# ctpeterson/qex

Hardware: AMD Instinct MI355X
Metric: staggered Dslash GFLOP/s + CG iters/s, 32^4 SU(3) fp64, 1/2/4/8 MI355X (higher is better)
Workload: dtype f64

## Files before the change

### include/qexhip.h

```cpp
#ifndef QEXHIP_H
#define QEXHIP_H

#include <stddef.h>

#ifdef __cplusplus
extern "C" {
#endif

typedef struct qexhip_ctx *qexhip_handle;

#define QEXHIP_OK 0
#define QEXHIP_ERR_ARG (-1)
#define QEXHIP_ERR_HIP (-2)
#define QEXHIP_ERR_STATE (-3)
#define QEXHIP_ERR_COMM (-4)
#define QEXHIP_ERR_IO (-5)

#define QEXHIP_EVEN 0
#define QEXHIP_ODD 1
#define QEXHIP_ALL 2

int qexhip_init(qexhip_handle *h, int device, const int latLocal[4],
                const int rankGeom[4], const int rankCoord[4]);
int qexhip_finalize(qexhip_handle h);
int qexhip_device_count(int *n);
const char *qexhip_last_error(void);
int qexhip_sync(qexhip_handle h);
int qexhip_device_info(qexhip_handle h, char *buf, int buflen);

#define QEXHIP_UNIQUE_ID_BYTES 128
int qexhip_comm_unique_id(char id[QEXHIP_UNIQUE_ID_BYTES]);
int qexhip_comm_init(qexhip_handle h, const char id[QEXHIP_UNIQUE_ID_BYTES], int nranks, int rank);
int qexhip_comm_info(qexhip_handle h, int *nranks, int *rank, int *device, char *busid, int buslen);
int qexhip_comm_transport(qexhip_handle h, char *name, int len, long stats[4]);
int qexhip_comm_count(qexhip_handle h, int *ncomms);
int qexhip_stag_sweep_info(qexhip_handle h, int out[8]);
int qexhip_stag_sweep_tuning(qexhip_handle h, double out[8]);
int qexhip_comm_force_halo(qexhip_handle h, int on);

int qexhip_layout_default_inner(const int localGeom[4], int V, int innerGeom[4]);
int qexhip_layout_simd_map(const int localGeom[4], const int innerGeom[4], int *v1_of_simd);
int qexhip_layout_vec_simd_to_v1(const int localGeom[4], const int innerGeom[4], const double *simd, double *v1);
int qexhip_layout_vec_v1_to_simd(const int localGeom[4], const int innerGeom[4], const double *v1, double *simd);
int qexhip_layout_gauge_simd_to_v1(const int localGeom[4], const int innerGeom[4], const double *const g[4], double *v1);
int qexhip_layout_gauge_v1_to_simd(const int localGeom[4], const int innerGeom[4], const double *v1, double *const g[4]);

int qexhip_stag_set_links(qexhip_handle h, const double *fat, const double *lng);

int qexhip_stag_dslash(qexhip_handle h, double *r, const double *x, int parity, double a, double b);

int qexhip_stag_D(qexhip_handle h, double *r, const double *x, double m, double sc);

int qexhip_stag_stagD(qexhip_handle h, double *r, const double *x, int parity, double m, double sc, double a);

int qexhip_stag_D_acc(qexhip_handle h, double *r, const double *x, double m, double sc, double a);

int qexhip_stag_op_xx(qexhip_handle h, double *r, const double *x, double m2, int par_even);

int qexhip_stag_eo_reconstruct(qexhip_handle h, double *r, const double *b, double m);

int qexhip_stag_eo_reduce(qexhip_handle h, double *r, const double *b, double m);

int qexhip_stag_outer(qexhip_handle h, double *f, const double *x, double scale_even, double scale_odd,
                      int accumulate);

int qexhip_stag_solve_xx(qexhip_handle h, double *x, const double *b, double mass, double r2req,
                         int maxits, int par_even, int *iters, double *r2_over_b2,
                         double *hist, int histcap);

int qexhip_stag_solve(qexhip_handle h, double *x, const double *b, double mass, double r2req,
                      int maxits, int *iters, double *r2_final);

int qexhip_stag_solve_prev(qexhip_handle h, double *x, const double *b, double mass, double r2req,
                           int maxits, int use_prev, int *iters, double *r2_final);

int qexhip_stag_solve_xx_sloppy(qexhip_handle h, double *x, const double *b, double mass, double r2req, int maxits,
                                int par_even, int sloppy, int *iters, double *r2_over_b2, int *nupdates);
int qexhip_stag_solve_sloppy(qexhip_handle h, double *x, const double *b, double mass, double r2req, int maxits,
                             int use_prev, int sloppy, int *iters, double *r2_final, int *nupdates);

int qexhip_stag_solve_xx_multi(qexhip_handle h, double *const *xs, const double *b,
                               const double *shifts, int nmass, double r2req, int maxits,
                               int par_even, int *iters, double *hist, int histcap);
int qexhip_stag_solve_multi(qexhip_handle h, double *const *xs, const double *b,
                            const double *masses, int nmass, double r2req, int maxits,
                            int *iters, double *r2_final);

int qexhip_norm2(qexhip_handle h, const double *x, int parity, double *out);
int qexhip_redot(qexhip_handle h, const double *x, const double *y, int parity, double *out);
int qexhip_dot(qexhip_handle h, const double *x, const double *y, int parity, double out[2]);
int qexhip_axpy(qexhip_handle h, double a, const double *x, double *y, int parity);
int qexhip_xpay(qexhip_handle h, const double *x, double a, double *y, int parity);

int qexhip_field_new(qexhip_handle h, int *id);
int qexhip_field_free(qexhip_handle h, int id);
int qexhip_field_upload(qexhip_handle h, int id, const double *host);
int qexhip_field_download(qexhip_handle h, int id, double *host);
int qexhip_field_zero(qexhip_handle h, int id);
int qexhip_dev_dslash(qexhip_handle h, int r_id, int x_id, int parity, double a, double b);
int qexhip_dev_op_xx(qexhip_handle h, int r_id, int x_id, double m2, int par_even);
int qexhip_dev_solve_xx(qexhip_handle h, int x_id, int b_id, double mass, double r2req,
                        int maxits, int par_even, int *iters, double *r2_over_b2,
                        double *hist, int histcap);
int qexhip_dev_solve_xx_sloppy(qexhip_handle h, int x_id, int b_id, double mass, double r2req, int maxits, int par_even,
                               int sloppy, int *iters, double *r2_over_b2, int *nupdates);
int qexhip_dev_op_xx_sloppy(qexhip_handle h, int r_id, int x_id, double m2, int par_even);
int qexhip_stag_links_info_f32(qexhip_handle h, int *format, double *max_dev);
int qexhip_dev_solve_xx_continue(qexhip_handle h, int x_id, double r2req, int maxits, int *iters, double *r2_over_b2,
                                 double *hist, int histcap);
int qexhip_dev_solve_xx_multi(qexhip_handle h, const int *x_ids, int b_id, const double *shifts, int nmass,
                              double r2req, int maxits, int par_even, int *iters, double *hist, int histcap);

int qexhip_release_workspace(qexhip_handle h);
int qexhip_dev_norm2(qexhip_handle h, int x_id, int parity, double *out);
int qexhip_dev_redot(qexhip_handle h, int x_id, int y_id, int parity, double *out);
int qexhip_dev_dot(qexhip_handle h, int x_id, int y_id, int parity, double out[2]);
int qexhip_dev_D(qexhip_handle h, int r_id, int x_id, double m, double sc);
int qexhip_dev_zero(qexhip_handle h, int id, int parity);
int qexhip_dev_solve_batch(qexhip_handle h, int n, const int *x_ids, const int *b_ids, const double *mass,
                           const double *r2req, int maxits, int *iters, double *r2);
int qexhip_dev_solve_batch_sloppy(qexhip_handle h, int n, const int *x_ids, const int *b_ids, const double *mass,
                                  const double *r2req, int maxits, int sloppy, int *iters, double *r2_final, int *nupdates);

int qexhip_dev_meson_corners(qexhip_handle h, int n, const int *x_ids, const int *y_ids, int t0, double *out);
int qexhip_dev_sym_shift(qexhip_handle h, int r_id, int x_id, int mu);
int qexhip_dev_norm2slice(qexhip_handle h, int id, int dir, double *out);

int qexhip_gauge_set(qexhip_handle h, const double *g);
int qexhip_gauge_get(qexhip_handle h, double *g);
int qexhip_plaq(qexhip_handle h, double out[6]);
int qexhip_gauge_force(qexhip_handle h, double *f, double cplaq);
int qexhip_wflow(qexhip_handle h, int nsteps, double eps);
int qexhip_gauge_force_general(qexhip_handle h, double *f, double cplaq, double c2, int kind);
int qexhip_wflow_general(qexhip_handle h, int nsteps, double eps, double cplaq, double c2, int kind);
int qexhip_flow_EQ(qexhip_handle h, int loop, double out[3]);
int qexhip_flow_measure(qexhip_handle h, double plaq[6], double EQ[3]);
int qexhip_gauge_action(qexhip_handle h, double cplaq, double crect, double cadjplaq, double *out);
int qexhip_gauge_update(qexhip_handle h, const double *p, double t);
int qexhip_gauge_reunit(qexhip_handle h);
int qexhip_wline(qexhip_handle h, const int *path, int n, double out[2]);
int qexhip_polyakov_loops(qexhip_handle h, double out[8]);
int qexhip_plaq_s4(qexhip_handle h, double out[8]);

int qexhip_fat7(qexhip_handle h, const double *g, const double coef[5], double *fl, double *ll, double naik);
int qexhip_hisq_smear(qexhip_handle h, const double *g, double *fl, double *ll);
int qexhip_nhyp_smear(qexhip_handle h, const double *g, double *fl, double alpha1, double alpha2, double alpha3);
int qexhip_fat7_deriv(qexhip_handle h, const double *g, const double *dfl, const double coef[5], const double *dll, double naik, double *d);
int qexhip_hisq_force(qexhip_handle h, const double *g, const double *dsdsu, const double *dsdsul, double *f);
int qexhip_hisq_prepare(qexhip_handle h, const double *g, double *fl, double *ll);
int qexhip_hisq_closure_force(qexhip_handle h, const double *dsdsu, const double *dsdsul, double *f);
int qexhip_hisq_release(qexhip_handle h);
int qexhip_hisq_fermion_force(qexhip_handle h, double *f, const double *const *psi, const double *scale, int n);

int qexhip_stag_solve_xx_batch(qexhip_handle h, int n, double *const *x, const double *const *b, const double *mass,
                               const double *r2req, int maxits, int par_even, int *iters, double *r2_over_b2);
int qexhip_stag_solve_batch(qexhip_handle h, int n, double *const *x, const double *const *b, const double *mass,
                            const double *r2req, int maxits, int *iters, double *r2_over_b2);

int qexhip_stag_solve_xx_batch_sloppy(qexhip_handle h, int n, double *const *x, const double *const *b, const double *mass,
                                      const double *r2req, int maxits, int par_even, int sloppy, int *iters, double *r2_over_b2,
                                      int *nupdates);
int qexhip_stag_solve_batch_sloppy(qexhip_handle h, int n, double *const *x, const double *const *b, const double *mass,
                                   const double *r2req, int maxits, int sloppy, int *iters, double *r2_final, int *nupdates);

int qexhip_stag_links_info(qexhip_handle h, int *nlinks, int *compressed, double *max_dev);
int qexhip_stag_links_storage(qexhip_handle h, int *bytes_per_link, long long *escaped);
int qexhip_link_residual_host(const double *links, int n, unsigned char *escaped, double *row2);
int qexhip_set_option(qexhip_handle h, const char *name, int value);

int qexhip_stag_set_links_hisq(qexhip_handle h, const double *g);
int qexhip_stag_set_links_nhyp(qexhip_handle h, const double *g, double alpha1, double alpha2, double alpha3,
                               const int antiperiodic[4], const int phases[4]);

int qexhip_nhyp_prepare(qexhip_handle h, const double *g, double alpha1, double alpha2, double alpha3, double *fl);
int qexhip_nhyp_force(qexhip_handle h, double *f, const double *chain);
int qexhip_nhyp_release(qexhip_handle h);
int qexhip_nhyp_gauge_force(qexhip_handle h, double *f, double cplaq, double crect, double cadjplaq);
int qexhip_nhyp_fforce(qexhip_handle h, double *f, int n, const double *const *phi, const double *mass, const double *scale,
                       const double *r2req, int maxits, const int antiperiodic[4], const int phases[4], int *iters);
int qexhip_nhyp_fermion_force(qexhip_handle h, double *f, const double *const *psi, const double *scale, int n,
                              const int antiperiodic[4], const int phases[4]);
int qexhip_nhyp_fforce_dev(qexhip_handle h, double *f, int n, const int *phi_ids, const double *mass, const double *scale,
                           const double *r2req, int maxits, const int antiperiodic[4], const int phases[4], int *iters);

typedef struct qexhip_rng qexhip_rng;
int qexhip_rng_new(qexhip_rng **rng, int kind, unsigned long long seed, const int lat[4], const int glat[4], int t_offset);
int qexhip_rng_free(qexhip_rng *rng);
int qexhip_rng_uniform(qexhip_rng *rng, int ncomp, double *v);
int qexhip_rng_gaussian_vector(qexhip_rng *rng, double *v);
int qexhip_rng_u1_vector(qexhip_rng *rng, double *v);
int qexhip_rng_random_tah(qexhip_rng *rng, double *p);
int qexhip_rng_gauge_random(qexhip_rng *rng, double *g);
int qexhip_rng_gauge_warm(qexhip_rng *rng, double s, double *g);
int qexhip_rng_state_words(qexhip_rng *rng);
int qexhip_rng_get_state(qexhip_rng *rng, unsigned *out);
int qexhip_rng_set_state(qexhip_rng *rng, const unsigned *in);

int qexhip_rng_dev_gaussian_vector(qexhip_handle h, qexhip_rng *rng, int field_id);
int qexhip_rng_dev_u1_vector(qexhip_handle h, qexhip_rng *rng, int field_id);
int qexhip_md_refresh_momenta(qexhip_handle h, qexhip_rng *rng);

int qexhip_md_begin(qexhip_handle h, const double *g, const double *p);
int qexhip_md_end(qexhip_handle h, double *g, double *p);
int qexhip_md_momentum_norm2(qexhip_handle h, double *p2);
int qexhip_md_update_links(qexhip_handle h, double t);
int qexhip_md_gauge_force(qexhip_handle h, double cplaq, double crect, double cadj);
int qexhip_md_kick(qexhip_handle h, int source, double t);
int qexhip_md_shift_links(qexhip_handle h, int source, double t);
int qexhip_md_save_links(qexhip_handle h);
int qexhip_md_restore_links(qexhip_handle h);

int qexhip_io_gauge_info(const char *path, int lat[4], char *precision, int *checksums_present);
int qexhip_io_read_gauge(const char *path, const int lat[4], double *g, unsigned *suma, unsigned *sumb);
int qexhip_io_read_gauge_slab(const char *path, const int lat[4], int t0, int nt, double *g);
int qexhip_io_write_gauge(const char *path, const int lat[4], const double *g, char precision, const char *file_md,
                          const char *record_md);
int qexhip_io_write_field(const char *path, const int lat[4], const void *data, int site_bytes, int word_bytes, const char *datatype,
                          char precision, int colors, int datacount, const char *file_md, const char *record_md);
int qexhip_io_read_field(const char *path, const int lat[4], void *data, int site_bytes, int word_bytes, char datatype[64]);
int qexhip_io_metadata(const char *path, char *file_md, int file_cap, char *record_md, int record_cap, int *file_len,
                       int *record_len);
int qexhip_io_crc32(const void *data, size_t nbytes, unsigned *crc);

int qexhip_timers_enable(qexhip_handle h, int on);
int qexhip_timers_reset(qexhip_handle h);
int qexhip_timers_get(qexhip_handle h, const char *name, long *count, double *total_ms);

int qexhip_debug_geom(const int latLocal[4], int depth, int halo, int out[8]);
int qexhip_debug_nbr_pos(const int latLocal[4], int depth, int halo, int c, int parity, int mu, int hop);
int qexhip_debug_site_coord(const int latLocal[4], int c, int parity, int x[4]);
int qexhip_debug_tile_order(const int latLocal[4], int mu, int nu, int *out, int cap);

#ifdef __cplusplus
}
#endif
#endif
```

### qex_amd/__init__.py

```python
from ._lib import QexHipError, LIB_PATH, lib
from .layout import Layout
from .gauge import setBC, stagPhase, rephase, unit, synthetic_random_su3, synthetic_gaussian_vector
from .staggered import (
    Context, device_count, Staggered, SolverParams, newStag, newStag3, link_residual_host, plaq, gaugeForce, gaugeFlow, gaugeSet, gaugeFlowResident, flowEQ, flowMeasure, gaugeAction, gaugeUpdate, reunit, wline, ploops, s4_gauge, ResidentMD, HisqCoefs, HypCoefs, makeImpLinks, fat7lDeriv, EVEN, ODD, ALL,
    SloppyNone, SloppySingle, SloppyHalf,
)
from .io import loadGauge, loadGaugeSlab, saveGauge, getFileLattice, gaugeFileInfo, writeField, readField, fileMetadata
from .rng import RngField, RngMilc6, MRG32k3a
from .mesons import stagLocalMesons, stagMesons, norm2slice, sft, printLocalMesons, pointSource, wallSource, localMesonTables
```

### qex_amd/_lib.py

```python
import ctypes as C
import os

_HERE = os.path.dirname(os.path.abspath(__file__))
LIB_PATH = os.environ.get("QEXHIP_LIB", os.path.join(_HERE, "libqexhip.so"))
_lib = None

_vp, _ci, _cd = C.c_void_p, C.c_int, C.c_double
_pi, _pd = C.POINTER(C.c_int), C.POINTER(C.c_double)
SYMBOLS = [
    ("qexhip_init", _ci, [C.POINTER(_vp), _ci, _pi, _pi, _pi]),
    ("qexhip_finalize", _ci, [_vp]),
    ("qexhip_device_count", _ci, [_pi]),
    ("qexhip_last_error", C.c_char_p, []),
    ("qexhip_sync", _ci, [_vp]),
    ("qexhip_device_info", _ci, [_vp, C.c_char_p, _ci]),
    ("qexhip_layout_default_inner", _ci, [_pi, _ci, _pi]),
    ("qexhip_layout_simd_map", _ci, [_pi, _pi, _pi]),
    ("qexhip_layout_vec_simd_to_v1", _ci, [_pi, _pi, _vp, _vp]),
    ("qexhip_layout_vec_v1_to_simd", _ci, [_pi, _pi, _vp, _vp]),
    ("qexhip_layout_gauge_simd_to_v1", _ci, [_pi, _pi, C.POINTER(C.c_void_p), _vp]),
    ("qexhip_layout_gauge_v1_to_simd", _ci, [_pi, _pi, _vp, C.POINTER(C.c_void_p)]),
    ("qexhip_comm_unique_id", _ci, [C.c_char_p]),
    ("qexhip_comm_init", _ci, [_vp, C.c_char_p, _ci, _ci]),
    ("qexhip_comm_force_halo", _ci, [_vp, _ci]),
    ("qexhip_comm_info", _ci, [_vp, _pi, _pi, _pi, C.c_char_p, _ci]),
    ("qexhip_comm_count", _ci, [_vp, _pi]),
    ("qexhip_comm_transport", _ci, [_vp, C.c_char_p, _ci, C.POINTER(C.c_long)]),
    ("qexhip_stag_sweep_info", _ci, [_vp, _pi]),
    ("qexhip_stag_sweep_tuning", _ci, [_vp, _pd]),
    ("qexhip_dot", _ci, [_vp, _vp, _vp, _ci, _pd]),
    ("qexhip_dev_dot", _ci, [_vp, _ci, _ci, _ci, _pd]),
    ("qexhip_stag_set_links", _ci, [_vp, _vp, _vp]),
    ("qexhip_stag_dslash", _ci, [_vp, _vp, _vp, _ci, _cd, _cd]),
    ("qexhip_stag_D", _ci, [_vp, _vp, _vp, _cd, _cd]),
    ("qexhip_stag_D_acc", _ci, [_vp, _vp, _vp, _cd, _cd, _cd]),
    ("qexhip_stag_op_xx", _ci, [_vp, _vp, _vp, _cd, _ci]),
    ("qexhip_stag_eo_reconstruct", _ci, [_vp, _vp, _vp, _cd]),
    ("qexhip_stag_eo_reduce", _ci, [_vp, _vp, _vp, _cd]),
    ("qexhip_stag_stagD", _ci, [_vp, _vp, _vp, _ci, _cd, _cd, _cd]),
    ("qexhip_stag_outer", _ci, [_vp, _vp, _vp, _cd, _cd, _ci]),
    ("qexhip_stag_solve_xx", _ci, [_vp, _vp, _vp, _cd, _cd, _ci, _ci, _pi, _pd, _vp, _ci]),
    ("qexhip_stag_solve", _ci, [_vp, _vp, _vp, _cd, _cd, _ci, _pi, _pd]),
    ("qexhip_stag_solve_xx_sloppy", _ci, [_vp, _vp, _vp, _cd, _cd, _ci, _ci, _ci, _pi, _pd, _pi]),
    ("qexhip_stag_solve_sloppy", _ci, [_vp, _vp, _vp, _cd, _cd, _ci, _ci, _ci, _pi, _pd, _pi]),
    ("qexhip_dev_solve_xx_sloppy", _ci, [_vp, _ci, _ci, _cd, _cd, _ci, _ci, _ci, _pi, _pd, _pi]),
    ("qexhip_dev_op_xx_sloppy", _ci, [_vp, _ci, _ci, _cd, _ci]),
    ("qexhip_stag_links_info_f32", _ci, [_vp, _pi, _pd]),
    ("qexhip_stag_solve_prev", _ci, [_vp, _vp, _vp, _cd, _cd, _ci, _ci, _pi, _pd]),
    ("qexhip_stag_solve_xx_multi", _ci, [_vp, _vp, _vp, _vp, _ci, _cd, _ci, _ci, _pi, _vp, _ci]),
    ("qexhip_stag_solve_multi", _ci, [_vp, _vp, _vp, _vp, _ci, _cd, _ci, _pi, _pd]),
    ("qexhip_norm2", _ci, [_vp, _vp, _ci, _pd]),
    ("qexhip_redot", _ci, [_vp, _vp, _vp, _ci, _pd]),
    ("qexhip_axpy", _ci, [_vp, _cd, _vp, _vp, _ci]),
    ("qexhip_xpay", _ci, [_vp, _vp, _cd, _vp, _ci]),
    ("qexhip_field_new", _ci, [_vp, _pi]),
    ("qexhip_field_free", _ci, [_vp, _ci]),
    ("qexhip_field_upload", _ci, [_vp, _ci, _vp]),
    ("qexhip_field_download", _ci, [_vp, _ci, _vp]),
    ("qexhip_field_zero", _ci, [_vp, _ci]),
    ("qexhip_dev_dslash", _ci, [_vp, _ci, _ci, _ci, _cd, _cd]),
    ("qexhip_dev_op_xx", _ci, [_vp, _ci, _ci, _cd, _ci]),
    ("qexhip_dev_solve_xx", _ci, [_vp, _ci, _ci, _cd, _cd, _ci, _ci, _pi, _pd, _vp, _ci]),
    ("qexhip_dev_solve_xx_continue", _ci, [_vp, _ci, _cd, _ci, _pi, _pd, _vp, _ci]),
    ("qexhip_dev_solve_xx_multi", _ci, [_vp, _pi, _ci, _pd, _ci, _cd, _ci, _ci, _pi, _vp, _ci]),
    ("qexhip_release_workspace", _ci, [_vp]),
    ("qexhip_dev_norm2", _ci, [_vp, _ci, _ci, _pd]),
    ("qexhip_dev_redot", _ci, [_vp, _ci, _ci, _ci, _pd]),
    ("qexhip_dev_D", _ci, [_vp, _ci, _ci, _cd, _cd]),
    ("qexhip_gauge_set", _ci, [_vp, _vp]),
    ("qexhip_gauge_get", _ci, [_vp, _vp]),
    ("qexhip_plaq", _ci, [_vp, _vp]),
    ("qexhip_gauge_force", _ci, [_vp, _vp, _cd]),
    ("qexhip_wflow", _ci, [_vp, _ci, _cd]),
    ("qexhip_flow_EQ", _ci, [_vp, _ci, _vp]),
    ("qexhip_flow_measure", _ci, [_vp, _vp, _vp]),
    ("qexhip_gauge_force_general", _ci, [_vp, _vp, _cd, _cd, _ci]),
    ("qexhip_wflow_general", _ci, [_vp, _ci, _cd, _cd, _cd, _ci]),
    ("qexhip_fat7", _ci, [_vp, _vp, _pd, _vp, _vp, _cd]),
    ("qexhip_hisq_smear", _ci, [_vp, _vp, _vp, _vp]),
    ("qexhip_nhyp_smear", _ci, [_vp, _vp, _vp, _cd, _cd, _cd]),
    ("qexhip_stag_solve_xx_batch", _ci, [_vp, _ci, _vp, _vp, _vp, _vp, _ci, _ci, _pi, _vp]),
    ("qexhip_stag_solve_batch", _ci, [_vp, _ci, _vp, _vp, _vp, _vp, _ci, _pi, _vp]),
    ("qexhip_stag_solve_xx_batch_sloppy", _ci, [_vp, _ci, _vp, _vp, _vp, _vp, _ci, _ci, _ci, _pi, _vp, _pi]),
    ("qexhip_stag_solve_batch_sloppy", _ci, [_vp, _ci, _vp, _vp, _vp, _vp, _ci, _ci, _pi, _vp, _pi]),
    ("qexhip_stag_links_info", _ci, [_vp, _pi, _pi, _vp]),
    ("qexhip_stag_links_storage", _ci, [_vp, _pi, C.POINTER(C.c_longlong)]),
    ("qexhip_link_residual_host", _ci, [_vp, _ci, _vp, _vp]),
    ("qexhip_set_option", _ci, [_vp, C.c_char_p, _ci]),
    ("qexhip_fat7_deriv", _ci, [_vp, _vp, _vp, _vp, _vp, _cd, _vp]),
    ("qexhip_hisq_force", _ci, [_vp, _vp, _vp, _vp, _vp]),
    ("qexhip_hisq_prepare", _ci, [_vp, _vp, _vp, _vp]),
    ("qexhip_hisq_closure_force", _ci, [_vp, _vp, _vp, _vp]),
    ("qexhip_hisq_release", _ci, [_vp]),
    ("qexhip_hisq_fermion_force", _ci, [_vp, _vp, _vp, _vp, _ci]),
    ("qexhip_stag_set_links_hisq", _ci, [_vp, _vp]),
    ("qexhip_stag_set_links_nhyp", _ci, [_vp, _vp, _cd, _cd, _cd, _pi, _pi]),
    ("qexhip_nhyp_prepare", _ci, [_vp, _vp, _cd, _cd, _cd, _vp]),
    ("qexhip_nhyp_force", _ci, [_vp, _vp, _vp]),
    ("qexhip_nhyp_release", _ci, [_vp]),
    ("qexhip_nhyp_fforce", _ci, [_vp, _vp, _ci, _vp, _vp, _vp, _vp, _ci, _pi, _pi, _pi]),
    ("qexhip_nhyp_gauge_force", _ci, [_vp, _vp, _cd, _cd, _cd]),
    ("qexhip_nhyp_fermion_force", _ci, [_vp, _vp, _vp, _vp, _ci, _pi, _pi]),
    ("qexhip_gauge_action", _ci, [_vp, _cd, _cd, _cd, _vp]),
    ("qexhip_gauge_update", _ci, [_vp, _vp, _cd]),
    ("qexhip_gauge_reunit", _ci, [_vp]),
    ("qexhip_wline", _ci, [_vp, _pi, _ci, _vp]),
    ("qexhip_polyakov_loops", _ci, [_vp, _vp]),
    ("qexhip_plaq_s4", _ci, [_vp, _vp]),
    ("qexhip_rng_new", _ci, [_vp, _ci, C.c_ulonglong, _pi, _pi, _ci]),
    ("qexhip_rng_free", _ci, [_vp]),
    ("qexhip_rng_uniform", _ci, [_vp, _ci, _vp]),
    ("qexhip_rng_gaussian_vector", _ci, [_vp, _vp]),
    ("qexhip_rng_u1_vector", _ci, [_vp, _vp]),
    ("qexhip_rng_random_tah", _ci, [_vp, _vp]),
    ("qexhip_rng_gauge_random", _ci, [_vp, _vp]),
    ("qexhip_rng_gauge_warm", _ci, [_vp, _cd, _vp]),
    ("qexhip_rng_dev_gaussian_vector", _ci, [_vp, _vp, _ci]),
    ("qexhip_rng_dev_u1_vector", _ci, [_vp, _vp, _ci]),
    ("qexhip_md_refresh_momenta", _ci, [_vp, _vp]),
    ("qexhip_dev_zero", _ci, [_vp, _ci, _ci]),
    ("qexhip_dev_solve_batch", _ci, [_vp, _ci, _pi, _pi, _pd, _pd, _ci, _pi, _pd]),
    ("qexhip_dev_solve_batch_sloppy", _ci, [_vp, _ci, _pi, _pi, _pd, _pd, _ci, _ci, _pi, _pd, _pi]),
    ("qexhip_dev_meson_corners", _ci, [_vp, _ci, _pi, _pi, _ci, _vp]),
    ("qexhip_dev_sym_shift", _ci, [_vp, _ci, _ci, _ci]),
    ("qexhip_dev_norm2slice", _ci, [_vp, _ci, _ci, _vp]),
    ("qexhip_nhyp_fforce_dev", _ci, [_vp, _vp, _ci, _pi, _pd, _pd, _pd, _ci, _pi, _pi, _pi]),
    ("qexhip_rng_state_words", _ci, [_vp]),
    ("qexhip_rng_get_state", _ci, [_vp, _vp]),
    ("qexhip_rng_set_state", _ci, [_vp, _vp]),
    ("qexhip_io_write_field", _ci, [C.c_char_p, _pi, _vp, _ci, _ci, C.c_char_p, C.c_char, _ci, _ci, C.c_char_p, C.c_char_p]),
    ("qexhip_io_read_field", _ci, [C.c_char_p, _pi, _vp, _ci, _ci, C.c_char_p]),
    ("qexhip_md_begin", _ci, [_vp, _vp, _vp]),
    ("qexhip_md_end", _ci, [_vp, _vp, _vp]),
    ("qexhip_md_momentum_norm2", _ci, [_vp, _pd]),
    ("qexhip_md_update_links", _ci, [_vp, _cd]),
    ("qexhip_md_gauge_force", _ci, [_vp, _cd, _cd, _cd]),
    ("qexhip_md_kick", _ci, [_vp, _ci, _cd]),
    ("qexhip_md_shift_links", _ci, [_vp, _ci, _cd]),
    ("qexhip_md_save_links", _ci, [_vp]),
    ("qexhip_md_restore_links", _ci, [_vp]),
    ("qexhip_io_metadata", _ci, [C.c_char_p, C.c_char_p, _ci, C.c_char_p, _ci, _pi, _pi]),
    ("qexhip_io_crc32", _ci, [C.c_char_p, C.c_size_t, C.POINTER(C.c_uint)]),
    ("qexhip_io_gauge_info", _ci, [C.c_char_p, _pi, C.c_char_p, _pi]),
    ("qexhip_io_read_gauge", _ci, [C.c_char_p, _pi, _vp, _vp, _vp]),
    ("qexhip_io_read_gauge_slab", _ci, [C.c_char_p, _pi, _ci, _ci, _vp]),
    ("qexhip_io_write_gauge", _ci, [C.c_char_p, _pi, _vp, C.c_char, C.c_char_p, C.c_char_p]),
    ("qexhip_timers_enable", _ci, [_vp, _ci]),
    ("qexhip_timers_reset", _ci, [_vp]),
    ("qexhip_timers_get", _ci, [_vp, C.c_char_p, C.POINTER(C.c_long), _pd]),
    ("qexhip_debug_geom", _ci, [_pi, _ci, _ci, _pi]),
    ("qexhip_debug_nbr_pos", _ci, [_pi, _ci, _ci, _ci, _ci, _ci, _ci]),
    ("qexhip_debug_site_coord", _ci, [_pi, _ci, _ci, _pi]),
    ("qexhip_debug_tile_order", _ci, [_pi, _ci, _ci, _pi, _ci]),
]


class QexHipError(RuntimeError):
    pass


def lib():
    global _lib
    if _lib is None:
        if not os.path.exists(LIB_PATH):
            raise QexHipError(
                f"{LIB_PATH} not found: build it with `make -C {_HERE}` "
                "(__graft_entry__.build()).  qex_amd has no CPU fallback."
            )
        L = C.CDLL(LIB_PATH, mode=C.RTLD_LOCAL | getattr(os, "RTLD_DEEPBIND", 0))
        for name, res, args in SYMBOLS:
            f = getattr(L, name)
            f.restype = res
            f.argtypes = args
        _lib = L
    return _lib


_tune = None


def tune_lib():
    global _tune
    if _tune is None:
        lib()
        path = os.path.join(os.path.dirname(LIB_PATH), "libqexhip_tune.so")
        if not os.path.exists(path):
            raise QexHipError(f"{path} not found: build it with `make -C {_HERE} libqexhip_tune.so`")
        T = C.CDLL(path, mode=C.RTLD_LOCAL | getattr(os, "RTLD_DEEPBIND", 0))
        pd = C.POINTER(C.c_double)
        T.qexhip_tune_dslash.argtypes = [_vp, _ci, _ci, _ci, pd]
        T.qexhip_tune_dslash_norm2.argtypes = [_vp, pd]
        T.qexhip_tune_stream.argtypes = [_vp, _ci, C.c_size_t, _ci, _ci, pd]
        T.qexhip_tune_fma64.argtypes = [_vp, _ci, _ci, _ci, _ci, pd]
        T.qexhip_tune_gather.argtypes = [_vp, _ci, _ci, _ci, _ci, pd]
        T.qexhip_tune_gather_rows.argtypes = [_vp, _ci, _ci, _ci, _ci, _ci, pd]
        _tune = T
    return _tune


def check(rc):
    if rc != 0:
        msg = lib().qexhip_last_error()
        raise QexHipError(f"libqexhip error {rc}: {msg.decode() if msg else ''}")
```

### qex_amd/csrc/api.cpp

```cpp
#include "qexhip_internal.h"
#include <string>
#include "../../include/qexhip.h"
#include <algorithm>
#include <cstdarg>
#include <cstdlib>
#include <cstring>
#include <vector>

static thread_local char g_err[1024] = "";

void qexhip_set_error(const char *fmt, ...) {
  va_list ap;
  va_start(ap, fmt);
  vsnprintf(g_err, sizeof(g_err), fmt, ap);
  va_end(ap);
}
extern "C" const char *qexhip_last_error(void) { return g_err; }

static bool timer_class_on(const qexhip_ctx *c, const char *name) {
  if (!c->timers_on) return false;
  if (c->timers_on == 2) return strncmp(name, "dslash", 6) == 0;
  if (c->timers_on == 3) return strncmp(name, "dslash", 6) == 0 || strcmp(name, "exchange") == 0 || strcmp(name, "allreduce") == 0;
  return true;
}
// ... 581 lines not shown
  if (!c) return QEXHIP_ERR_ARG;
  CHK(sloppy_check(c, 1));
  HIPCHK(hipSetDevice(c->device));
  DevField *fr, *fx;
  CHK(find_field(c, r_id, &fr));
  CHK(find_field(c, x_id, &fx));
  DevFieldF *xi, *ro;
  CHK(f32_field(c, F32_IN, &xi));
  CHK(f32_field(c, F32_AP, &ro));
  const int px = par_even ? 0 : 1;
  CHK(f32_from_f64(c, *xi, *fx, px, 1.0));
  CHK(f32_op_xx(c, *ro, *xi, m2, par_even, 0, nullptr, nullptr));
  return f32_to_f64(c, *fr, *ro, px, 1.0, 0);
}
extern "C" int qexhip_stag_links_info_f32(qexhip_handle c, int *format, double *max_dev) {
  if (!c) return QEXHIP_ERR_ARG;
  HIPCHK(hipSetDevice(c->device));
  return f32_links(c, format, max_dev);
}

extern "C" int qexhip_dev_solve_xx_continue(qexhip_handle c, int x_id, double r2req, int maxits, int *iters, double *r2_over_b2,
                                            double *hist, int histcap) {
  if (!c) return QEXHIP_ERR_ARG;
  HIPCHK(hipSetDevice(c->device));
  DevField *fx;
  CHK(find_field(c, x_id, &fx));
  return solve_xx_continue_dev(c, *fx, r2req, maxits, iters, r2_over_b2, hist, histcap);
}

extern "C" int qexhip_dev_solve_xx_multi(qexhip_handle c, const int *x_ids, int b_id, const double *shifts, int nmass,
                                         double r2req, int maxits, int par_even, int *iters, double *hist, int histcap) {
  if (!c || !x_ids || !shifts || nmass < 1 || nmass > 32) return QEXHIP_ERR_ARG;
  DevField *fb;
  CHK(find_field(c, b_id, &fb));
  std::vector<DevField *> xp(nmass);
  for (int k = 0; k < nmass; k++) {
    CHK(find_field(c, x_ids[k], &xp[k]));
    if (x_ids[k] == b_id) { qexhip_set_error("dev_solve_xx_multi: x_ids[%d] is the source field", k); return QEXHIP_ERR_ARG; }
    for (int j = 0; j < k; j++)
      if (x_ids[j] == x_ids[k]) { qexhip_set_error("dev_solve_xx_multi: x_ids[%d] == x_ids[%d]", j, k); return QEXHIP_ERR_ARG; }
  }
  return solve_xx_multi_dev(c, xp, *fb, shifts, nmass, r2req, maxits, par_even, iters, hist, histcap);
}

extern "C" int qexhip_release_workspace(qexhip_handle c) {
  if (!c) return QEXHIP_ERR_ARG;
  HIPCHK(hipSetDevice(c->device));
  HIPCHK(hipStreamSynchronize(c->stream));
  for (auto it = c->fields.begin(); it != c->fields.end();) {
    if (it->first <= -1000) {
      HIPCHK(hipFree(it->second.d));
      it = c->fields.erase(it);
    } else {
      ++it;
    }
  }
  gauge_release_scratch(c);
  f32_state_free(c);
  batch_f32_state_free(c);
  return 0;
}

extern "C" int qexhip_dev_norm2(qexhip_handle c, int x_id, int parity, double *out) {
  if (!c || !out || parity < 0 || parity > 2) return QEXHIP_ERR_ARG;
  HIPCHK(hipSetDevice(c->device));
  DevField *fx;
  CHK(find_field(c, x_id, &fx));
  CHK(blas_norm2(c, *fx, parity, &c->dscal[8]));
  return read_scalars(c, &c->dscal[8], 1, out);
}
extern "C" int qexhip_dev_redot(qexhip_handle c, int x_id, int y_id, int parity, double *out) {
  if (!c || !out || parity < 0 || parity > 2) return QEXHIP_ERR_ARG;
  HIPCHK(hipSetDevice(c->device));
  DevField *fx, *fy;
  CHK(find_field(c, x_id, &fx));
  CHK(find_field(c, y_id, &fy));
  CHK(blas_redot(c, *fx, *fy, parity, &c->dscal[8]));
  return read_scalars(c, &c->dscal[8], 1, out);
}
extern "C" int qexhip_dev_dot(qexhip_handle c, int x_id, int y_id, int parity, double out[2]) {
  if (!c || !out || parity < 0 || parity > 2) return QEXHIP_ERR_ARG;
  HIPCHK(hipSetDevice(c->device));
  DevField *fx, *fy;
  CHK(find_field(c, x_id, &fx));
  CHK(find_field(c, y_id, &fy));
  CHK(blas_cdot(c, *fx, *fy, parity, &c->dscal[8]));
  return read_scalars(c, &c->dscal[8], 2, out);
}
extern "C" int qexhip_dev_D(qexhip_handle c, int r_id, int x_id, double m, double sc) {
  if (!c || r_id == x_id) return QEXHIP_ERR_ARG;
  HIPCHK(hipSetDevice(c->device));
  DevField *fr, *fx;
  CHK(find_field(c, r_id, &fr));
  CHK(find_field(c, x_id, &fx));
  return op_D(c, *fr, *fx, m, sc);
}

extern "C" int qexhip_dev_meson_corners(qexhip_handle c, int n, const int *x_ids, const int *y_ids, int t0, double *out) {
  if (!c) return QEXHIP_ERR_ARG;
  if (!x_ids || !y_ids || !out) { qexhip_set_error("dev_meson_corners: null argument"); return QEXHIP_ERR_ARG; }
  if (n < 1 || n > 4) { qexhip_set_error("dev_meson_corners: n = %d, must be 1..4", n); return QEXHIP_ERR_ARG; }
  const int ntg = c->g.X[3] * c->rankGeom[3];
  if (t0 < 0 || t0 >= ntg) { qexhip_set_error("dev_meson_corners: t0 = %d outside [0, %d)", t0, ntg); return QEXHIP_ERR_ARG; }
  HIPCHK(hipSetDevice(c->device));
  DevField *xs[4], *ys[4];
  for (int k = 0; k < n; k++) {
    CHK(find_field(c, x_ids[k], &xs[k]));
    CHK(find_field(c, y_ids[k], &ys[k]));
  }
  return meson_corners(c, n, xs, ys, t0, out);
}
extern "C" int qexhip_dev_sym_shift(qexhip_handle c, int r_id, int x_id, int mu) {
  if (!c) return QEXHIP_ERR_ARG;
  if (mu < 0 || mu > 2) { qexhip_set_error("dev_sym_shift: mu = %d, only the spatial directions 0..2 are shifted", mu); return QEXHIP_ERR_ARG; }
  if (r_id == x_id) { qexhip_set_error("dev_sym_shift: r_id == x_id"); return QEXHIP_ERR_ARG; }
  if (!c->W) { qexhip_set_error("dev_sym_shift: no links set (qexhip_stag_set_links first)"); return QEXHIP_ERR_ARG; }
  HIPCHK(hipSetDevice(c->device));
  DevField *fr, *fx;
  CHK(find_field(c, r_id, &fr));
  CHK(find_field(c, x_id, &fx));
  return sym_shift(c, *fr, *fx, mu);
}
extern "C" int qexhip_dev_norm2slice(qexhip_handle c, int id, int dir, double *out) {
  if (!c) return QEXHIP_ERR_ARG;
  if (!out) { qexhip_set_error("dev_norm2slice: null argument"); return QEXHIP_ERR_ARG; }
  if (dir < 0 || dir > 3) { qexhip_set_error("dev_norm2slice: dir = %d, must be 0..3", dir); return QEXHIP_ERR_ARG; }
  HIPCHK(hipSetDevice(c->device));
  DevField *f;
  CHK(find_field(c, id, &f));
  return norm2slice(c, *f, dir, out);
}

extern "C" int qexhip_fat7(qexhip_handle c, const double *g, const double coef[5], double *fl, double *ll, double naik) {
  if (!c || !g || !coef || !fl) return QEXHIP_ERR_ARG;
  HIPCHK(hipSetDevice(c->device));
  return smear_fat7_host(c, g, coef, fl, ll, naik);
}
extern "C" int qexhip_hisq_smear(qexhip_handle c, const double *g, double *fl, double *ll) {
  if (!c || !g || !fl || !ll) return QEXHIP_ERR_ARG;
  HIPCHK(hipSetDevice(c->device));
  return smear_hisq_host(c, g, fl, ll);
}
extern "C" int qexhip_nhyp_smear(qexhip_handle c, const double *g, double *fl, double a1, double a2, double a3) {
  if (!c || !g || !fl) return QEXHIP_ERR_ARG;
  HIPCHK(hipSetDevice(c->device));
  return smear_nhyp_host(c, g, fl, a1, a2, a3);
}

extern "C" int qexhip_set_option(qexhip_handle c, const char *name, int value) {
  if (!c || !name) return QEXHIP_ERR_ARG;
  const std::string n(name);
  if (n == "recon") c->opt_recon = value;
  else if (n == "lossless") c->opt_lossless = value;
  else if (n == "overlap") c->opt_overlap = value;
  else if (n == "transport") {
    if (comm_ready(c)) { qexhip_set_error("option transport must be set before qexhip_comm_init"); return QEXHIP_ERR_STATE; }
    if (value < 0 || value > 3) { qexhip_set_error("option transport: 0 auto, 1 rccl, 2 peer, 3 rccl + mailbox sums"); return QEXHIP_ERR_ARG; }
    c->opt_transport = value;
  }
  else if (n == "batch_multi") c->opt_batch_multi = value;
  else if (n == "multi_reduce") c->opt_multi_reduce = value;
  else if (n == "flow_exp") c->opt_flow_exp = value;
  else if (n == "smear_ca") c->opt_smear_ca = value;
  else if (n == "chain_overlap") c->opt_chain_overlap = value;
  else if (n == "hop_split") {
    if (value != -1 && value != 0 && value != 2) { qexhip_set_error("option hop_split: -1 measured, 0 split by sites, 2 fused (the two-launch form 1 left the library in round 6)"); return QEXHIP_ERR_ARG; }
    c->opt_hop_split = value;
  }
  else if (n == "fused_spin_us") c->opt_fused_spin_us = value;
  else if (n == "emu_exchange_us") c->emu_exchange_us = value;
  else if (n == "emu_allreduce_us") c->emu_allreduce_us = value;
  else if (n == "emu_link_gbs") c->emu_link_gbs = value;
  else if (n == "obs_clover") c->opt_obs_clover = value;
  else if (n == "force_pair") c->opt_force_pair = value;
  else if (n == "sloppy_check") {
    if (value < 1) { qexhip_set_error("option sloppy_check: >= 1 fp32 iterations"); return QEXHIP_ERR_ARG; }
    c->opt_sloppy_check = value;
  }
  else { qexhip_set_error("unknown option"); return QEXHIP_ERR_ARG; }
  return 0;
}
extern "C" int qexhip_stag_solve_xx_batch(qexhip_handle c, int n, double *const *x, const double *const *b, const double *mass,
                                          const double *r2req, int maxits, int par_even, int *iters, double *r2_over_b2) {
  if (!c || !x || !b || !mass || !r2req) return QEXHIP_ERR_ARG;
  HIPCHK(hipSetDevice(c->device));
  return solve_batch_host(c, n, x, b, mass, r2req, maxits, par_even ? 1 : 0, iters, r2_over_b2);
}
extern "C" int qexhip_stag_solve_batch(qexhip_handle c, int n, double *const *x, const double *const *b, const double *mass,
                                       const double *r2req, int maxits, int *iters, double *r2_over_b2) {
  if (!c || !x || !b || !mass || !r2req) return QEXHIP_ERR_ARG;
  HIPCHK(hipSetDevice(c->device));
  return solve_batch_host(c, n, x, b, mass, r2req, maxits, -1, iters, r2_over_b2);
}
extern "C" int qexhip_stag_solve_xx_batch_sloppy(qexhip_handle c, int n, double *const *x, const double *const *b, const double *mass,
                                                 const double *r2req, int maxits, int par_even, int sloppy, int *iters,
                                                 double *r2_over_b2, int *nupdates) {
  if (!c || !x || !b || !mass || !r2req) return QEXHIP_ERR_ARG;
  CHK(sloppy_check(c, sloppy));
  if (n < 1 || n > 4) { qexhip_set_error("batch solve: 1 <= n <= 4"); return QEXHIP_ERR_ARG; }
  if (nupdates) for (int j = 0; j < n; j++) nupdates[j] = 0;
  if (!sloppy) return qexhip_stag_solve_xx_batch(c, n, x, b, mass, r2req, maxits, par_even, iters, r2_over_b2);
  HIPCHK(hipSetDevice(c->device));
  return solve_batch_sloppy_host(c, n, x, b, mass, r2req, maxits, par_even ? 1 : 0, sloppy, iters, r2_over_b2, nupdates);
}
extern "C" int qexhip_stag_solve_batch_sloppy(qexhip_handle c, int n, double *const *x, const double *const *b, const double *mass,
                                              const double *r2req, int maxits, int sloppy, int *iters, double *r2_final, int *nupdates) {
  if (!c || !x || !b || !mass || !r2req) return QEXHIP_ERR_ARG;
  CHK(sloppy_check(c, sloppy));
  if (n < 1 || n > 4) { qexhip_set_error("batch solve: 1 <= n <= 4"); return QEXHIP_ERR_ARG; }
  if (nupdates) for (int j = 0; j < n; j++) nupdates[j] = 0;
  if (!sloppy) return qexhip_stag_solve_batch(c, n, x, b, mass, r2req, maxits, iters, r2_final);
  HIPCHK(hipSetDevice(c->device));
  return solve_batch_sloppy_host(c, n, x, b, mass, r2req, maxits, -1, sloppy, iters, r2_final, nupdates);
}
extern "C" int qexhip_stag_links_info(qexhip_handle c, int *nlinks, int *compressed, double *max_dev) {
  if (!c) return QEXHIP_ERR_ARG;
  if (nlinks) *nlinks = c->W ? c->ndir : 0;
  if (compressed) *compressed = c->recon;
  if (max_dev) *max_dev = c->recon_dev;
  return 0;
}
extern "C" int qexhip_stag_links_storage(qexhip_handle c, int *bytes_per_link, long long *escaped) {
  if (!c) return QEXHIP_ERR_ARG;
  if (bytes_per_link) *bytes_per_link = !c->W ? 0 : (c->lres ? 108 : (c->recon == 1 ? 96 : (c->recon == 2 ? 112 : 144)));
  if (escaped) *escaped = c->lres_esc;
  return 0;
}
extern "C" int qexhip_link_residual_host(const double *links, int n, unsigned char *escaped, double *row2) {
  if (!links || n < 0) return QEXHIP_ERR_ARG;
  return link_residual_host((const double2 *)links, n, escaped, (double2 *)row2);
}
extern "C" int qexhip_hisq_prepare(qexhip_handle c, const double *g, double *fl, double *ll) {
  if (!c || !g) return QEXHIP_ERR_ARG;
  HIPCHK(hipSetDevice(c->device));
  return hisq_prepare(c, g, fl, ll);
}
extern "C" int qexhip_hisq_closure_force(qexhip_handle c, const double *dsdsu, const double *dsdsul, double *f) {
  if (!c || !dsdsu || !dsdsul || !f) return QEXHIP_ERR_ARG;
  HIPCHK(hipSetDevice(c->device));
  return hisq_closure_force(c, dsdsu, dsdsul, f);
}
extern "C" int qexhip_hisq_fermion_force(qexhip_handle c, double *f, const double *const *psi, const double *scale, int n) {
  if (!c || !f || !psi || !scale) return QEXHIP_ERR_ARG;
  HIPCHK(hipSetDevice(c->device));
  return hisq_fermion_force(c, f, psi, scale, n);
}
extern "C" int qexhip_hisq_release(qexhip_handle c) {
  if (!c) return QEXHIP_ERR_ARG;
  HIPCHK(hipSetDevice(c->device));
  hisq_state_free(c);
  return 0;
}
extern "C" int qexhip_hisq_force(qexhip_handle c, const double *g, const double *dsdsu, const double *dsdsul, double *f) {
  if (!c || !g || !dsdsu || !dsdsul || !f) return QEXHIP_ERR_ARG;
  HIPCHK(hipSetDevice(c->device));
  return smear_hisq_force_host(c, g, dsdsu, dsdsul, f);
}
extern "C" int qexhip_fat7_deriv(qexhip_handle c, const double *g, const double *dfl, const double coef[5], const double *dll,
                                 double naik, double *d) {
  if (!c || !g || !dfl || !coef || !d) return QEXHIP_ERR_ARG;
  HIPCHK(hipSetDevice(c->device));
  return smear_fat7_deriv_host(c, g, dfl, coef, dll, naik, d);
}
extern "C" int qexhip_stag_set_links_hisq(qexhip_handle c, const double *g) {
  if (!c) return QEXHIP_ERR_ARG;
  HIPCHK(hipSetDevice(c->device));
  return smear_set_links_hisq(c, g);
}
extern "C" int qexhip_stag_set_links_nhyp(qexhip_handle c, const double *g, double a1, double a2, double a3,
                                          const int antiperiodic[4], const int phases[4]) {
  if (!c) return QEXHIP_ERR_ARG;
  HIPCHK(hipSetDevice(c->device));
  static const int defph[4] = {8, 9, 11, 0};
  int mask = 0;
  for (int mu = 0; mu < 4; mu++) if (antiperiodic ? antiperiodic[mu] : (mu == 3)) mask |= 1 << mu;
  return smear_set_links_nhyp(c, g, a1, a2, a3, mask, phases ? phases : defph);
}

extern "C" int qexhip_nhyp_prepare(qexhip_handle c, const double *g, double a1, double a2, double a3, double *fl) {
  if (!c) return QEXHIP_ERR_ARG;
  HIPCHK(hipSetDevice(c->device));
  return nhyp_prepare(c, g, a1, a2, a3, fl);
}
extern "C" int qexhip_nhyp_force(qexhip_handle c, double *f, const double *chain) {
  if (!c || !f || !chain) return QEXHIP_ERR_ARG;
  HIPCHK(hipSetDevice(c->device));
  return nhyp_force_host(c, f, chain);
}
extern "C" int qexhip_nhyp_gauge_force(qexhip_handle c, double *f, double cplaq, double crect, double cadj) {
  if (!c) return QEXHIP_ERR_ARG;
  if (crect != 0.0 && cadj != 0.0) { qexhip_set_error("rect and adjplaq together are not a QEX action"); return QEXHIP_ERR_ARG; }
  HIPCHK(hipSetDevice(c->device));
  return nhyp_gauge_force(c, f, cplaq, cadj != 0.0 ? cadj : crect, cadj != 0.0 ? 1 : 0);
}
extern "C" int qexhip_nhyp_fermion_force(qexhip_handle c, double *f, const double *const *psi, const double *scale, int n,
                                         const int antiperiodic[4], const int phases[4]) {
  if (!c || !psi || !scale) return QEXHIP_ERR_ARG;
  HIPCHK(hipSetDevice(c->device));
  static const int defph[4] = {8, 9, 11, 0};
  int mask = 0;
  for (int mu = 0; mu < 4; mu++) if (antiperiodic ? antiperiodic[mu] : (mu == 3)) mask |= 1 << mu;
  return nhyp_fermion_force(c, f, psi, scale, n, mask, phases ? phases : defph);
}
extern "C" int qexhip_nhyp_fforce(qexhip_handle c, double *f, int n, const double *const *phi, const double *mass,
                                  const double *scale, const double *r2req, int maxits, const int antiperiodic[4],
                                  const int phases[4], int *iters) {
  if (!c || !phi || !mass || !scale || !r2req) return QEXHIP_ERR_ARG;
  HIPCHK(hipSetDevice(c->device));
  static const int defph[4] = {8, 9, 11, 0};
  int mask = 0;
  for (int mu = 0; mu < 4; mu++) if (antiperiodic ? antiperiodic[mu] : (mu == 3)) mask |= 1 << mu;
  return nhyp_fforce(c, f, n, phi, mass, scale, r2req, maxits, mask, phases ? phases : defph, iters);
}
extern "C" int qexhip_nhyp_fforce_dev(qexhip_handle c, double *f, int n, const int *phi_ids, const double *mass,
                                      const double *scale, const double *r2req, int maxits, const int antiperiodic[4],
                                      const int phases[4], int *iters) {
  if (!c || !phi_ids || !mass || !scale || !r2req || n < 1 || n > 64) return QEXHIP_ERR_ARG;
  HIPCHK(hipSetDevice(c->device));
  static const int defph[4] = {8, 9, 11, 0};
  int mask = 0;
  for (int mu = 0; mu < 4; mu++) if (antiperiodic ? antiperiodic[mu] : (mu == 3)) mask |= 1 << mu;
  std::vector<DevField *> pf(n);
  for (int k = 0; k < n; k++) CHK(find_field(c, phi_ids[k], &pf[k]));
  return nhyp_fforce(c, f, n, nullptr, mass, scale, r2req, maxits, mask, phases ? phases : defph, iters, pf.data());
}
struct qexhip_rng;
extern "C" int qexhip_rng_dev_gaussian_vector(qexhip_handle c, qexhip_rng *rng, int field_id) {
  if (!c || !rng) return QEXHIP_ERR_ARG;
  DevField *f;
  CHK(find_field(c, field_id, &f));
  return rng_dev_generate(c, rng, 0, f, nullptr);
}
extern "C" int qexhip_rng_dev_u1_vector(qexhip_handle c, qexhip_rng *rng, int field_id) {
  if (!c || !rng) return QEXHIP_ERR_ARG;
  DevField *f;
  CHK(find_field(c, field_id, &f));
  return rng_dev_generate(c, rng, 1, f, nullptr);
}
extern "C" int qexhip_md_refresh_momenta(qexhip_handle c, qexhip_rng *rng) {
  if (!c || !rng) return QEXHIP_ERR_ARG;
  HIPCHK(hipSetDevice(c->device));
  double2 *M = nullptr;
  CHK(md_momenta_dev(c, &M));
  return rng_dev_generate(c, rng, 2, nullptr, M);
}
extern "C" int qexhip_dev_zero(qexhip_handle c, int id, int parity) {
  if (!c || parity < 0 || parity > 2) return QEXHIP_ERR_ARG;
  HIPCHK(hipSetDevice(c->device));
  DevField *f;
  CHK(find_field(c, id, &f));
  return blas_zero(c, *f, parity);
}
static int batch_alias_check(int n, const int *x_ids, const int *b_ids) {
  for (int i = 0; i < n; i++)
    for (int j = 0; j < n; j++)
      if (x_ids[i] == b_ids[j] || (i != j && x_ids[i] == x_ids[j])) {
        qexhip_set_error("dev_solve_batch: solution field %d (system %d) aliases %s of system %d", x_ids[i], i,
                         x_ids[i] == b_ids[j] ? "the source" : "the solution", j);
        return QEXHIP_ERR_ARG;
      }
  return 0;
}
extern "C" int qexhip_dev_solve_batch(qexhip_handle c, int n, const int *x_ids, const int *b_ids, const double *mass,
                                      const double *r2req, int maxits, int *iters, double *r2) {
  if (!c || !x_ids || !b_ids || !mass || !r2req || n < 1 || n > 64) return QEXHIP_ERR_ARG;
  HIPCHK(hipSetDevice(c->device));
  CHK(batch_alias_check(n, x_ids, b_ids));
  for (int k0 = 0; k0 < n; k0 += 4) {
    const int k = std::min(4, n - k0);
    DevField *xs[4], *bs[4];
    for (int j = 0; j < k; j++) {
      CHK(find_field(c, x_ids[k0 + j], &xs[j]));
      CHK(find_field(c, b_ids[k0 + j], &bs[j]));
    }
    CHK(solve_full_batch_dev(c, k, xs, bs, mass + k0, r2req + k0, maxits, iters ? iters + k0 : nullptr, r2 ? r2 + k0 : nullptr));
  }
  return 0;
}
extern "C" int qexhip_dev_solve_batch_sloppy(qexhip_handle c, int n, const int *x_ids, const int *b_ids, const double *mass,
                                             const double *r2req, int maxits, int sloppy, int *iters, double *r2, int *nupdates) {
  if (!c || !x_ids || !b_ids || !mass || !r2req) return QEXHIP_ERR_ARG;
  CHK(sloppy_check(c, sloppy));
  if (n < 1 || n > 4) { qexhip_set_error("batch solve: 1 <= n <= 4"); return QEXHIP_ERR_ARG; }
  if (nupdates) for (int j = 0; j < n; j++) nupdates[j] = 0;
// ... 91 lines not shown
```

### qex_amd/csrc/blas.hip

```cpp
#include "qexhip_internal.h"
#include "reduce.h"
#include "cg_device.h"
#include <cstring>
#include "peer_device.h"

static inline int grid_for(size_t n2) {
  size_t nb = (n2 + 255) / 256;
  if (nb > 2048) nb = 2048;
  if (nb < 1) nb = 1;
  return (int)nb;
}
static inline size_t body2(const qexhip_ctx *c) { return (size_t)c->g.ntile * 192; }

#define FOR_PAR(par, p) for (int p = ((par) == 2 ? 0 : (par)); p <= ((par) == 2 ? 1 : (par)); p++)

__global__ void __launch_bounds__(256) k_zero(double2 *y, size_t n) {
  for (size_t i = blockIdx.x * 256 + threadIdx.x; i < n; i += (size_t)gridDim.x * 256) y[i] = make_double2(0, 0);
}
__global__ void __launch_bounds__(256) k_copy(double2 *y, const double2 *x, size_t n) {
  for (size_t i = blockIdx.x * 256 + threadIdx.x; i < n; i += (size_t)gridDim.x * 256) y[i] = x[i];
}
__global__ void __launch_bounds__(256) k_axpy(double a, const double2 *x, double2 *y, size_t n) {
  for (size_t i = blockIdx.x * 256 + threadIdx.x; i < n; i += (size_t)gridDim.x * 256) {
    double2 xv = x[i], yv = y[i];
// ... 17 lines not shown
}
__global__ void __launch_bounds__(256) k_axpby(double a, const double2 *x, double b, const double2 *y, double2 *z, size_t n) {
  for (size_t i = blockIdx.x * 256 + threadIdx.x; i < n; i += (size_t)gridDim.x * 256) {
    double2 xv = x[i], yv = y[i];
    z[i] = make_double2(a * xv.x + b * yv.x, a * xv.y + b * yv.y);
  }
}
__global__ void __launch_bounds__(256) k_redot(const double2 *x, const double2 *y, size_t n, double *partials) {
  double acc = 0;
  for (size_t i = blockIdx.x * 256 + threadIdx.x; i < n; i += (size_t)gridDim.x * 256) {
    double2 xv = x[i], yv = y[i];
    acc = fma(xv.x, yv.x, fma(xv.y, yv.y, acc));
  }
  double r = block_sum_256(acc);
  if (threadIdx.x == 0) partials[blockIdx.x] = r;
}
__global__ void __launch_bounds__(256) k_reduce_final(const double *partials, int n, double *out, const int *done) {
  if (done && *done) return;
  double acc = 0;
  for (int i = threadIdx.x; i < n; i += 256) acc += partials[i];
  double r = block_sum_256(acc);
  if (threadIdx.x == 0) *out = r;
}

__global__ void k_delay(long long ticks) {
  const long long t0 = wall_clock64();
  for (int i = 0; i < (1 << 22); i++) {
    if (wall_clock64() - t0 >= ticks) break;
    __builtin_amdgcn_s_sleep(32);
  }
}
int blas_delay(hipStream_t st, int us) {
  if (us <= 0) return 0;
  k_delay<<<1, 1, 0, st>>>((long long)us * 100);
  HIPCHK(hipGetLastError());
  return 0;
}

int blas_grid(const qexhip_ctx *c, int) { return grid_for(body2(c)); }

int blas_zero(qexhip_ctx *c, DevField &f, int parity) {
  size_t n = body2(c);
  FOR_PAR(parity, p) k_zero<<<grid_for(n), 256, 0, c->stream>>>(f.par(p), n);
  HIPCHK(hipGetLastError());
  return 0;
}
int blas_copy(qexhip_ctx *c, DevField &dst, const DevField &src, int parity) {
  size_t n = body2(c);
  FOR_PAR(parity, p) k_copy<<<grid_for(n), 256, 0, c->stream>>>(dst.par(p), src.par(p), n);
  HIPCHK(hipGetLastError());
  return 0;
}
int blas_axpy(qexhip_ctx *c, double a, const DevField &x, DevField &y, int parity) {
  size_t n = body2(c);
  ScopedTimer tm(c, "blas", c->stream);
  FOR_PAR(parity, p) k_axpy<<<grid_for(n), 256, 0, c->stream>>>(a, x.par(p), y.par(p), n);
  HIPCHK(hipGetLastError());
  return 0;
}
int blas_xpay(qexhip_ctx *c, const DevField &x, double a, DevField &y, int parity) {
  size_t n = body2(c);
  ScopedTimer tm(c, "blas", c->stream);
  FOR_PAR(parity, p) k_xpay<<<grid_for(n), 256, 0, c->stream>>>(x.par(p), a, y.par(p), n);
  HIPCHK(hipGetLastError());
  return 0;
}
int blas_scale(qexhip_ctx *c, double a, DevField &y, int parity) {
  size_t n = body2(c);
  FOR_PAR(parity, p) k_scale<<<grid_for(n), 256, 0, c->stream>>>(a, y.par(p), n);
  HIPCHK(hipGetLastError());
  return 0;
}
int blas_axpby(qexhip_ctx *c, double a, const DevField &x, double b, const DevField &y, DevField &z, int parity) {
  size_t n = body2(c);
  FOR_PAR(parity, p) k_axpby<<<grid_for(n), 256, 0, c->stream>>>(a, x.par(p), b, y.par(p), z.par(p), n);
  HIPCHK(hipGetLastError());
  return 0;
}

int reduce_partials(qexhip_ctx *c, int n, double *dev_out) {
  {
    ScopedTimer tm(c, "reduce", c->stream);
    k_reduce_final<<<1, 256, 0, c->stream>>>(c->partials, n, dev_out, nullptr);
    HIPCHK(hipGetLastError());
  }
  if (multi_rank(c)) CHK(comm_allreduce(c, dev_out, 1));
  return 0;
}

int blas_redot(qexhip_ctx *c, const DevField &x, const DevField &y, int parity, double *dev_out) {
  size_t n = body2(c);
  int nb = grid_for(n);
  int tot = 0;
  {
    ScopedTimer tm(c, "blas", c->stream);
    FOR_PAR(parity, p) {
      k_redot<<<nb, 256, 0, c->stream>>>(x.par(p), y.par(p), n, c->partials + tot);
      tot += nb;
    }
    HIPCHK(hipGetLastError());
  }
  return reduce_partials(c, tot, dev_out);
}
__global__ void __launch_bounds__(256) k_cdot(const double2 *x, const double2 *y, size_t n, double *pre, double *pim) {
  double ar = 0, ai = 0;
  for (size_t i = blockIdx.x * 256 + threadIdx.x; i < n; i += (size_t)gridDim.x * 256) {
    const double2 xv = x[i], yv = y[i];
    ar = fma(xv.x, yv.x, fma(xv.y, yv.y, ar));
    ai = fma(xv.x, yv.y, fma(-xv.y, yv.x, ai));
  }
  double r = block_sum_256(ar);
  if (threadIdx.x == 0) pre[blockIdx.x] = r;
  r = block_sum_256(ai);
  if (threadIdx.x == 0) pim[blockIdx.x] = r;
}
__global__ void __launch_bounds__(256) k_reduce_final2(const double *pre, const double *pim, int n, double *out) {
  const double *p = blockIdx.x ? pim : pre;
  double acc = 0;
  for (int i = threadIdx.x; i < n; i += 256) acc += p[i];
  double r = block_sum_256(acc);
  if (threadIdx.x == 0) out[blockIdx.x] = r;
}
int blas_cdot(qexhip_ctx *c, const DevField &x, const DevField &y, int parity, double *dev_out) {
  size_t n = body2(c);
  const int nb = grid_for(n);
  int tot = 0;
  double *pre = c->partials, *pim = c->partials + 2 * nb;
  if (4 * nb > c->part2_off + 2048) { qexhip_set_error("internal: partial buffer too small for cdot"); return -3; }
  {
    ScopedTimer tm(c, "blas", c->stream);
    FOR_PAR(parity, p) {
      k_cdot<<<nb, 256, 0, c->stream>>>(x.par(p), y.par(p), n, pre + tot, pim + tot);
      tot += nb;
    }
    k_reduce_final2<<<2, 256, 0, c->stream>>>(pre, pim, tot, dev_out);
    HIPCHK(hipGetLastError());
  }
  if (multi_rank(c)) CHK(comm_allreduce(c, dev_out, 2));
  return 0;
}

int blas_norm2(qexhip_ctx *c, const DevField &x, int parity, double *dev_out) {
  return blas_redot(c, x, x, parity, dev_out);
}

int read_scalars(qexhip_ctx *c, const double *dev, int n, double *host) {
  HIPCHK(hipMemcpyAsync(c->pinned, dev, sizeof(double) * n, hipMemcpyDeviceToHost, c->stream));
  HIPCHK(hipStreamSynchronize(c->stream));
  CHK(peer_check(c));
  for (int i = 0; i < n; i++) host[i] = ((double *)c->pinned)[i];
  return 0;
}

__global__ void __launch_bounds__(256) k_cg_xpay(double2 *p, const double2 *r, size_t n, CgScal *s, int k, int rolled,
                                                const double *r2parts, int nparts, double *hist, int histcap) {
  const int cur = k & 1, prv = cur ^ 1;
  double r2k;
  if (rolled) {
    if (s->dones[cur]) return;
    r2k = s->r2s[cur];
  } else {
    if (s->dones[prv]) {
      if (blockIdx.x == 0 && threadIdx.x == 0) cg_carry(s, k);
      return;
    }
    r2k = cg_sum_parts(r2parts, nparts);
    if (blockIdx.x == 0 && threadIdx.x == 0) cg_roll(s, k, r2k, hist, histcap);
    if (!(k < s->maxits && r2k > s->r2stop)) return;
  }
  const bool first = (k == 0);
  const double beta = r2k / s->r2s[prv];
  for (size_t i = blockIdx.x * 256 + threadIdx.x; i < n; i += (size_t)gridDim.x * 256) {
    double2 rv = r[i];
    if (first) p[i] = rv;
    else {
      double2 pv = p[i];
      p[i] = make_double2(fma(beta, pv.x, rv.x), fma(beta, pv.y, rv.y));
    }
  }
}
__global__ void __launch_bounds__(256) k_cg_update(double2 *x, double2 *r, const double2 *p, const double2 *Ap,
                                                  size_t n, const CgScal *s, int k, double *partials,
                                                  const double *dotp, int ndot) {
  if (s->dones[k & 1]) return;
  const double pAp = (ndot > 0) ? cg_sum_parts(dotp, ndot) : s->pAp;
  const double alpha = s->r2s[k & 1] / pAp;
  double acc = 0;
  for (size_t i = blockIdx.x * 256 + threadIdx.x; i < n; i += (size_t)gridDim.x * 256) {
    double2 pv = p[i], xv = x[i], rv = r[i], av = Ap[i];
    xv.x += alpha * pv.x; xv.y += alpha * pv.y;
    rv.x -= alpha * av.x; rv.y -= alpha * av.y;
    x[i] = xv; r[i] = rv;
    acc = fma(rv.x, rv.x, fma(rv.y, rv.y, acc));
  }
  double t = block_sum_256(acc);
  if (threadIdx.x == 0) partials[blockIdx.x] = t;
}
__global__ void k_cg_init(CgScal *s, const double *dscal, double r2req, int maxits, double *hist, int histcap) {
  s->b2 = dscal[0];
  s->r2 = dscal[1];
  s->rzo = 1.0;
  s->pAp = 0.0;
  s->r2stop = r2req * s->b2;
  s->itn = 0;
  s->maxits = maxits;
  s->done = !(0 < maxits && s->r2 > s->r2stop);
  s->r2s[0] = s->r2; s->itns[0] = 0; s->dones[0] = s->done;
  s->r2s[1] = 1.0; s->itns[1] = 0; s->dones[1] = s->done;
  if (histcap > 0) hist[0] = (s->b2 != 0.0) ? s->r2 / s->b2 : 0.0;
}
__global__ void __launch_bounds__(256) k_cg_close(CgScal *s, int k, const double *r2parts, int nparts, double *hist, int histcap) {
  if (s->dones[(k & 1) ^ 1]) {
    if (threadIdx.x == 0) cg_carry(s, k);
    return;
  }
  const double r2k = cg_sum_parts(r2parts, nparts);
  if (threadIdx.x == 0) cg_roll(s, k, r2k, hist, histcap);
}

int cg_xpay(qexhip_ctx *c, DevField &p, const DevField &r, int parity, int k, int rolled) {
  size_t n = body2(c);
  ScopedTimer tm(c, "blas", c->stream);
  k_cg_xpay<<<grid_for(n), 256, 0, c->stream>>>(p.par(parity), r.par(parity), n, c->cg, k, rolled,
                                               c->partials + c->part2_off, rolled ? grid_for(n) : c->cg_r2parts, c->hist, c->histcap);
  HIPCHK(hipGetLastError());
  return 0;
}
int cg_update(qexhip_ctx *c, DevField &x, DevField &r, const DevField &p, const DevField &Ap, int parity, int k, int ndot) {
  size_t n = body2(c);
  int nb = grid_for(n);
  double *r2p = c->partials + c->part2_off;
  if (ndot > 0) CHK(comm_allreduce_parts(c, c->partials, ndot, &ndot));
  CHK(devjoin_flush(c));
  {
    ScopedTimer tm(c, "blas", c->stream);
    k_cg_update<<<nb, 256, 0, c->stream>>>(x.par(parity), r.par(parity), p.par(parity), Ap.par(parity), n, c->cg, k, r2p,
                                           c->partials, ndot);
    HIPCHK(hipGetLastError());
  }
  CHK(comm_allreduce_parts(c, r2p, nb, &c->cg_r2parts));
  return 0;
}
int cg_close(qexhip_ctx *c, int k) {
  k_cg_close<<<1, 256, 0, c->stream>>>(c->cg, k, c->partials + c->part2_off, c->cg_r2parts, c->hist, c->histcap);
  HIPCHK(hipGetLastError());
  return comm_agree_post(c);
}
__global__ void k_cg_resume(CgScal *s, int k, double r2req, int maxits) {
  const int cur = k & 1;
  s->r2stop = r2req * s->b2;
  s->maxits = maxits;
  s->r2s[cur] = s->r2; s->r2s[cur ^ 1] = s->rzo; s->itns[cur] = k;
  s->dones[cur] = !(k < maxits && s->r2s[cur] > s->r2stop);
  s->done = s->dones[cur];
  s->agree[0] = s->r2s[cur]; s->agree[1] = -s->r2s[cur]; s->agree[2] = (double)k; s->agree[3] = -(double)k;
}
int cg_resume(qexhip_ctx *c, int k, double r2req, int maxits) {
  k_cg_resume<<<1, 1, 0, c->stream>>>(c->cg, k, r2req, maxits);
  HIPCHK(hipGetLastError());
  return 0;
}
int cg_init(qexhip_ctx *c, double r2req, int maxits) {
  c->cg_resume.valid = 0;
  k_cg_init<<<1, 1, 0, c->stream>>>(c->cg, c->dscal, r2req, maxits, c->hist, c->histcap);
  HIPCHK(hipGetLastError());
  return 0;
}
```

### qex_amd/csrc/dslash.hip

```cpp
#include "qexhip_internal.h"
#include "site_index.h"
#include "reduce.h"
#include "fused_sweep.h"
#include <hip/hip_ext.h>
#include <cstring>
#include <algorithm>
#include <chrono>

static double now_us() { return std::chrono::duration<double, std::micro>(std::chrono::steady_clock::now().time_since_epoch()).count(); }

struct DslashArgs {
  Geom g;
  const double2 *W;
  const unsigned long long *S;
  const double2 *in;
  double2 *out;
  const double2 *rin;
  const double2 *xs;
  double ca, cb;
  double sgn;
  double post;
  int parity;
  SweepRanges r;
  const double2 *gh_hi, *gh_lo;
  double *partials;
  const int *done;
  int swz;
  int ntstore;
  FusedSweep fs;
};

#include "dslash_core.h"

template <int NDIR, bool HALO, bool INIT, bool DOT, int RECON, bool FUSED>
__device__ __forceinline__ void dslash_body(const DslashArgs &A) {
  const bool skip = A.done && *A.done;
  if (skip && !FUSED) return;
  if (FUSED && fused_push(A.fs, skip)) return;
  FusedRole R;
  R.bid = blockIdx.x; R.cleanup = false; R.bnd = false; R.parked = false;
  if (FUSED) fused_enter(A.fs, A.r.nb1, R);
  const bool cleanup = FUSED && R.cleanup;
  for (;;) {
    int lb = R.bid;
    if (FUSED && !fused_next_block(A.fs, R, lb)) break;
    const bool bnd = FUSED && R.bnd;
    if (A.swz && !bnd) {
      int per = A.swz >> 3;
      lb = (lb & 7) * per + (lb >> 3);
    }
    int c, clim;
    if (FUSED) c = fused_site(A.fs, R, lb, A.r, clim);
    else sweep_site(A.r, lb, c, clim);
    double dotv = 0;
    const bool active = c < clim && !skip;
    const Geom &g = A.g;
    const SiteXYZT s = site_coord(g, c, A.parity);
    const int tu = FUSED ? __builtin_amdgcn_readfirstlane(s.t) : 0;
    double2 acc[3];
    double2 xsv[3];
    const LinkCursor<NDIR, RECON> L(A.W, A.S, c);
    const double2 *in_f1 = A.in, *in_b1 = A.in, *in_f3 = A.in, *in_b3 = A.in;
    if (FUSED) {
      in_f1 = tu + 1 >= g.X[3] ? A.gh_hi : A.in;
      in_b1 = tu - 1 < 0 ? A.gh_lo : A.in;
      in_f3 = tu + 3 >= g.X[3] ? A.gh_hi : A.in;
      in_b3 = tu - 3 < 0 ? A.gh_lo : A.in;
    }
    auto pair = [&](const int pr, const bool do_f, const bool do_b) __attribute__((always_inline)) {
      const int mu = pr & 3;
      const int hop = pr >= 4 ? 3 : 1;
      const int pf = nbr_pos<HALO>(g, c, s, mu, hop);
      const int pb = nbr_pos<HALO>(g, c, s, mu, -hop);
      double2 U[9], W[9], vf[3], vb[3];
      constexpr int NLOAD = LinkFormat<RECON>::NLOAD, LROW = LinkFormat<RECON>::LROW;
      const double2 *wp = L.w + (size_t)pr * (2 * LROW);
      if (do_f) {
#pragma unroll
        for (int k = 0; k < NLOAD; k++) {
          d2v t = __builtin_nontemporal_load((const d2v *)&wp[k * 64]);
          U[k] = make_double2(t.x, t.y);
        }
      }
      if (do_b) {
#pragma unroll
        for (int k = 0; k < NLOAD; k++) {
          d2v t = __builtin_nontemporal_load((const d2v *)&wp[LROW + k * 64]);
          W[k] = make_double2(t.x, t.y);
        }
      }
      if (RECON == 1) {
        if (do_f) recon_row2<1>(U, (L.sm[2 * pr] >> L.lane) & 1ull);
        if (do_b) recon_row2<1>(W, (L.sm[2 * pr + 1] >> L.lane) & 1ull);
      } else if (RECON == 3) {
        const size_t fr = ((size_t)L.tile * NDIR + 2 * pr) * 576 + L.lane;
        if (do_f) recon_row2_res(U, wp - L.lane, L.sm + 4 * pr, L.hdr, fr, L.lane);
        if (do_b) recon_row2_res(W, wp - L.lane + LROW, L.sm + 4 * pr + 2, L.hdr, fr + 576, L.lane);
      } else if (RECON == 2) {
        if (do_f) recon_row2<2>(U, false);
        if (do_b) recon_row2<2>(W, false);
      }
      const double2 *srcf = (FUSED && mu == 3) ? (hop == 3 ? in_f3 : in_f1) : A.in;
      const double2 *srcb = (FUSED && mu == 3) ? (hop == 3 ? in_b3 : in_b1) : A.in;
      if (do_f) {
#pragma unroll
        for (int k = 0; k < 3; k++) vf[k] = srcf[vec_off(pf, k)];
      }
      if (do_b) {
#pragma unroll
        for (int k = 0; k < 3; k++) vb[k] = srcb[vec_off(pb, k)];
      }
      if (do_f) mv3<false>(acc, U, vf);
      if (do_b) mv3<true>(acc, W, vb);
    };
    auto edge_pairs = [&](const bool crossing) __attribute__((always_inline)) {
      if (!crossing) {
        constexpr int NSP = NDIR / 2 - NDIR / 8;
        constexpr int UNS = NDIR == 8 ? 1 : 2;
#pragma unroll UNS
        for (int q = 0; q < NSP; q++) pair(q + q / 3, true, true);
      }
#pragma unroll 1
      for (int pr = 3; pr < NDIR / 2; pr += 4) {
        const int hop = pr >= 4 ? 3 : 1;
        const bool xf = tu + hop >= g.X[3], xb = tu - hop < 0;
        pair(pr, crossing ? xf : !xf, crossing ? xb : !xb);
      }
    };
    const bool edge = FUSED && bnd;
    if (active) {
      if ((INIT && !cleanup) || DOT) {
#pragma unroll
        for (int k = 0; k < 3; k++) xsv[k] = A.xs[vec_off(c, k)];
      }
      if (FUSED && cleanup) {
#pragma unroll
        for (int k = 0; k < 3; k++) acc[k] = A.out[vec_off(c, k)];
      } else if (INIT) {
#pragma unroll
        for (int k = 0; k < 3; k++) {
          acc[k].x = (A.sgn * A.cb) * xsv[k].x;
          acc[k].y = (A.sgn * A.cb) * xsv[k].y;
        }
        if (A.ca != 0.0) {
#pragma unroll
          for (int k = 0; k < 3; k++) {
            double2 r = A.rin[vec_off(c, k)];
            acc[k].x += (A.sgn * A.ca) * r.x;
            acc[k].y += (A.sgn * A.ca) * r.y;
          }
        }
      } else {
#pragma unroll
        for (int k = 0; k < 3; k++) acc[k] = make_double2(0.0, 0.0);
      }
      constexpr int UNR = (NDIR == 8) ? (RECON == 3 ? (FUSED ? 1 : 2) : (RECON ? 1 : 4)) : 2;
      if (!edge) {
#pragma unroll UNR
        for (int pr = 0; pr < NDIR / 2; pr++) pair(pr, true, true);
      } else if (!cleanup) {
        edge_pairs(false);
      }
    }
    if (edge && !skip) {
      fused_wait_faces(A.fs, R);
      if (active && !R.parked) edge_pairs(true);
    }
    const bool parked = FUSED && R.parked;
    if (active) {
      if (parked) {
#pragma unroll
        for (int k = 0; k < 3; k++) A.out[vec_off(c, k)] = acc[k];
      } else {
#pragma unroll
        for (int k = 0; k < 3; k++) {
          acc[k].x *= (A.sgn * A.post); acc[k].y *= (A.sgn * A.post);
          if (A.ntstore) {
            d2v t; t.x = acc[k].x; t.y = acc[k].y;
            __builtin_nontemporal_store(t, (d2v *)&A.out[vec_off(c, k)]);
          } else {
            A.out[vec_off(c, k)] = acc[k];
          }
        }
        if (DOT) {
#pragma unroll
          for (int k = 0; k < 3; k++) dotv = fma(xsv[k].x, acc[k].x, fma(xsv[k].y, acc[k].y, dotv));
        }
      }
    }
    if (DOT && !skip && !parked) {
      const int pidx = !FUSED ? (RECON == 3 ? lb : (int)blockIdx.x) : fused_partial_slot(A.fs, R, lb);
      double r = block_sum_256(dotv);
      if (threadIdx.x == 0) A.partials[pidx] = r;
    }
    if (!cleanup) break;
  }
  if (FUSED) fused_finish(A.fs, R);
}

template <int NDIR, bool HALO, bool INIT, bool DOT, int RECON>
__global__ void __launch_bounds__(256) k_dslash(DslashArgs A) { dslash_body<NDIR, HALO, INIT, DOT, RECON, false>(A); }
template <int NDIR, bool INIT, bool DOT, int RECON>
__global__ void __launch_bounds__(256) k_dslash_fused(DslashArgs A) { dslash_body<NDIR, true, INIT, DOT, RECON, true>(A); }

template <class K>
static void launch_timed(qexhip_ctx *c, const char *tname, K kernel, dim3 grid, dim3 block, DslashArgs &A, hipStream_t st) {
  hipEvent_t e0 = nullptr, e1 = nullptr;
  if (timer_event_pair(c, tname, &e0, &e1)) hipExtLaunchKernelGGL(kernel, grid, block, 0, st, e0, e1, 0, A);
  else hipLaunchKernelGGL(kernel, grid, block, 0, st, A);
}

template <int NDIR, bool HALO>
static int launch(qexhip_ctx *c, DslashArgs &A, int c0, int c1, bool init, bool dot, int part_off,
                  int d0 = 0, int d1 = 0, const char *tname = "dslash", hipStream_t st = nullptr, int fused_grid = 0) {
  if (!st) st = c->stream;
  const bool fused = fused_grid > 0;
  const int nb = sweep_ranges(A.r, c0, c1, d0, d1);
  if (!nb) return 0;
  const int nsw = fused ? A.r.nb1 : nb;
  A.swz = ((c->recon != 0 || (c->lres && !fused)) && nsw >= 64 && (nsw & 7) == 0) ? nsw : 0;
  A.ntstore = 1;
  double *psave = A.partials;
  A.partials = psave ? psave + part_off : nullptr;
  dim3 grid(fused ? fused_grid : nb), block(256);
#define QX_LAUNCH(R) \
  do { \
    if (HALO && fused) { \
      if (init && dot) launch_timed(c, tname, k_dslash_fused<NDIR, true, true, R>, grid, block, A, st); \
      else if (init) launch_timed(c, tname, k_dslash_fused<NDIR, true, false, R>, grid, block, A, st); \
      else if (dot) launch_timed(c, tname, k_dslash_fused<NDIR, false, true, R>, grid, block, A, st); \
      else launch_timed(c, tname, k_dslash_fused<NDIR, false, false, R>, grid, block, A, st); \
    } else if (init && dot) launch_timed(c, tname, k_dslash<NDIR, HALO, true, true, R>, grid, block, A, st); \
    else if (init) launch_timed(c, tname, k_dslash<NDIR, HALO, true, false, R>, grid, block, A, st); \
    else if (dot) launch_timed(c, tname, k_dslash<NDIR, HALO, false, true, R>, grid, block, A, st); \
    else launch_timed(c, tname, k_dslash<NDIR, HALO, false, false, R>, grid, block, A, st); \
  } while (0)
  if (c->recon == 1) QX_LAUNCH(1);
  else if (c->recon == 2) QX_LAUNCH(2);
  else if constexpr (NDIR == 8) {
    if (c->lres) QX_LAUNCH(3);
    else QX_LAUNCH(0);
  } else QX_LAUNCH(0);
#undef QX_LAUNCH
  A.partials = psave;
  HIPCHK(hipGetLastError());
  return 0;
}

void sweep_plan(const qexhip_ctx *c, int *lo_end_out, int *hi_beg_out, int *overlap_out) {
  const Geom &g = c->g;
  int lo_end = g.depth * g.F; if (lo_end > g.Vh) lo_end = g.Vh;
  int hi_beg = g.Vh - g.depth * g.F; if (hi_beg < lo_end) hi_beg = lo_end;
  const size_t face_bytes = (size_t)g.depth * g.F * 48;
  *lo_end_out = lo_end; *hi_beg_out = hi_beg;
  const int tuned = c->overlap_auto[c->ndir == 16];
  *overlap_out = !g.halo || hi_beg <= lo_end ? 0
                 : (c->opt_overlap >= 0 ? (c->opt_overlap != 0)
                    : (tuned >= 0 ? tuned : ((hi_beg - lo_end) >= 131072 && face_bytes >= ((size_t)1 << 20))));
}

int sweep_form(const qexhip_ctx *c, int overlap) {
  if (!overlap || !peer_faces(c)) return 0;
  if (c->opt_hop_split >= 0) return c->opt_hop_split ? 2 : 0;
  const int m = c->form_auto[c->ndir == 16];
  return m >= 0 ? m : 2;
}

static double exchange_estimate_us(const qexhip_ctx *c) {
  const double meas = c->xchg_us[c->ndir == 16];
  if (meas > 0) return meas;
  const double link = (c->emu_link_gbs > 0 ? c->emu_link_gbs : 45.0) * 1e3;
  return 3.0 + (double)c->g.depth * c->g.F * 48.0 / link;
}
double sweep_push_fraction(const qexhip_ctx *c, int interior_sites, int nrhs) {
  const double bsite = c->ndir * (c->recon == 1 ? 96.0 : (c->recon == 2 ? 112.0 : (c->lres ? 108.0 : 144.0))) + 120.0 * nrhs;
  const double t_int = (double)interior_sites * bsite / 5.5e6;
  return t_int > 0 ? std::min(1.0, std::max(0.65, nrhs * exchange_estimate_us(c) / t_int)) : 1.0;
}

static int sweep_fused_ctl(qexhip_ctx *c, int nbnd, FusedCtl *F, int nrhs) {
  if (c->fz_cap < nbnd) {
    HIPCHK(hipStreamSynchronize(c->stream));
    if (c->fz_buf) HIPCHK(hipFree(c->fz_buf));
    c->fz_buf = nullptr; c->fz_cap = 0;
    const int cap = std::max(2 * nbnd, 4096);
    HIPCHK(hipMalloc((void **)&c->fz_buf, (size_t)(256 + cap) * sizeof(unsigned int)));
    HIPCHK(hipMemsetAsync(c->fz_buf, 0, (size_t)(256 + cap) * sizeof(unsigned int), c->stream));
    c->fz_cap = cap;
  }
  F->dec = c->fz_buf; F->ndef = c->fz_buf + 32; F->cl_done = c->fz_buf + 64; F->late = c->fz_buf + 96;
  F->list = c->fz_buf + 256;
  F->ncl = std::max(std::min(nbnd, 4), std::min(nbnd / 8, 32));
  const double tick_per_us = (double)c->dj.ticks / (c->dj.timeout_s * 1e6);
  if (c->opt_fused_spin_us == -2) F->spin_ticks = -1;
  else {
    const double us = c->opt_fused_spin_us >= 0 ? (double)c->opt_fused_spin_us : std::max(25.0, nrhs * exchange_estimate_us(c));
    F->spin_ticks = (long long)(us * tick_per_us);
  }
  return 0;
}

int fused_sweep_setup(qexhip_ctx *c, int nrhs, DevField *const *f, int parity, int lo_end, int hi_beg, FusedSweep *F,
                      const double2 **gh_hi, const double2 **gh_lo, int *grid, int *nparts) {
  const int nb_int = (hi_beg - lo_end + 255) / 256, nb_lo = (lo_end + 255) / 256, nb_hi = (c->g.Vh - hi_beg + 255) / 256;
  CHK(comm_halo_push_only_multi(c, nrhs, f, parity, gh_hi, gh_lo, &F->push));
  CHK(peer_ghost_args(c, &F->pg));
  CHK(sweep_fused_ctl(c, nb_lo + nb_hi, &F->fz, nrhs));
  F->e0 = hi_beg; F->e1 = c->g.Vh; F->nb2 = nb_int + nb_lo;
  F->nbA = (int)(sweep_push_fraction(c, hi_beg - lo_end, nrhs) * nb_int);
  *grid = F->push.nblocks + nb_int + nb_lo + nb_hi + F->fz.ncl;
  *nparts = nb_int + nb_lo + nb_hi;
  return 0;
}

int sweep_autotune(qexhip_ctx *c) {
  const Geom &g = c->g;
  const int slot = c->ndir == 16;
  if (!g.halo || !c->W) return 0;
  const bool multi = c->nranks > 1 && comm_ready(c);
  if (multi) {
    const double code = 64.0 * c->opt_overlap + 1024.0 * (c->opt_hop_split + 1) + 65536.0 * (c->opt_fused_spin_us + 2);
    double v[2] = {code, -code};
    CHK(comm_allreduce_max(c, v, 2));
    if (v[0] != -v[1]) {
      qexhip_set_error("options overlap (QEXHIP_OVERLAP) / hop_split / fused_spin_us differ between the ranks (65536 (fused_spin_us + 2) + 1024 (hop_split + 1) "
                       "+ 64 overlap = %g .. %g): they must be the same everywhere", -v[1], v[0]);
      return -3;
    }
  }
  if (c->form_auto[slot] >= 0) return 0;
  const bool measure = c->opt_overlap == -2 || multi;
  if (!measure) return 0;
  int lo_end, hi_beg, dummy;
  sweep_plan(c, &lo_end, &hi_beg, &dummy);
  if (hi_beg <= lo_end) { c->overlap_auto[slot] = 0; c->form_auto[slot] = 0; return 0; }
  DevField f[3];
  int rc = 0;
  for (int k = 0; k < 3 && !rc; k++) rc = field_alloc(c, f[k]);
  const int saved = c->opt_overlap, saved_form = c->opt_hop_split, saved_timers = c->timers_on;
  c->timers_on = 0;
  double tx = 0;
  for (int k = 0; k < 10 && !rc; k++) {
    if (k == 2) { rc = hipStreamSynchronize(c->stream) != hipSuccess ? -2 : 0; tx = -now_us(); }
    if (!rc) rc = comm_halo_exchange(c, f[0], 0, 0);
  }
  if (!rc && hipStreamSynchronize(c->stream) != hipSuccess) rc = -2;
  tx = (tx + now_us()) / 8.0;
  if (!rc && multi) {
    double v[2] = {tx, 0};
    rc = comm_allreduce_max(c, v, 1);
    tx = v[0];
  }
  if (!rc) c->xchg_us[slot] = tx;
  const bool try_fused = peer_faces(c) && (c->opt_hop_split < 0 || c->opt_hop_split == 2);
  const bool try_sites = !(peer_faces(c) && c->opt_hop_split == 2);
  double t[3] = {0, 0, 0};
  for (int mode = 0; mode < 3 && !rc; mode++) {
    if ((mode == 1 && !try_sites) || (mode == 2 && !try_fused)) continue;
    if ((mode && saved == 0) || (!mode && saved == 1)) continue;
    c->opt_overlap = mode ? 1 : 0;
    c->opt_hop_split = mode == 2 ? 2 : 0;
    for (int k = 0; k < 6 && !rc; k++) {
      if (k == 1) { rc = hipStreamSynchronize(c->stream) != hipSuccess ? -2 : 0; t[mode] = -now_us(); }
      DslashOpts o1, o2;
      DevField &in0 = f[(k & 1) ? 2 : 0], &out2 = f[(k & 1) ? 0 : 2];
      if (!rc) rc = dslash_sweep(c, f[1], in0, 1, o1);
      if (!rc) rc = dslash_sweep(c, out2, f[1], 0, o2);
    }
    if (!rc && hipStreamSynchronize(c->stream) != hipSuccess) rc = -2;
    t[mode] += now_us();
  }
  c->opt_overlap = saved;
  c->opt_hop_split = saved_form;
  c->timers_on = saved_timers;
  for (int k = 0; k < 3; k++) if (f[k].d) (void)hipFree(f[k].d);
  double v[4] = {t[0], t[1], t[2], rc ? 1.0 : 0.0};
  if (multi) {
    const int e = comm_allreduce_max(c, v, 4);
    if (e && !rc) rc = e;
  }
  if (rc) return rc;
  if (v[3] != 0.0) { qexhip_set_error("sweep_autotune: another rank failed while measuring"); return -4; }
  const bool have1 = v[1] > 0, have2 = v[2] > 0;
  const int form = have2 && !(have1 && v[1] < 0.97 * v[2]) ? 2 : 0;
  const double best = form == 2 ? v[2] : v[1];
  c->form_auto[slot] = form;
  if (saved < 0) c->overlap_auto[slot] = (best > 0 && v[0] > 0 && best < 0.95 * v[0]) ? 1 : 0;
  for (int k = 0; k < 3; k++) c->overlap_tune_us[slot][k] = v[k] / 10.0;
  return 0;
}

void stag_link_bases(const qexhip_ctx *c, int parity, bool lossless, const double2 **W, const unsigned long long **S) {
  const size_t rows = (size_t)parity * c->g.ntile * c->ndir;
  if (c->recon) {
    *W = c->Wc + rows * (c->recon == 1 ? LinkFormat<1>::LROW : LinkFormat<2>::LROW);
    *S = c->Ws + rows;
  } else if (lossless) {
    *W = c->Wc + rows * LinkFormat<3>::LROW;
    *S = c->Wm + (size_t)parity * (2 + c->g.ntile * c->ndir * 2) + 2;
  } else {
    *W = c->W + rows * LinkFormat<0>::LROW;
    *S = nullptr;
  }
}

int dslash_sweep(qexhip_ctx *c, DevField &out, DevField &in, int parity, const DslashOpts &o) {
  const Geom &g = c->g;
  if (!c->W) { qexhip_set_error("staggered links not set (qexhip_stag_set_links)"); return -3; }
  DslashArgs A;
  memset(&A, 0, sizeof A);
  A.g = g;
  stag_link_bases(c, parity, c->lres != 0, &A.W, &A.S);
  A.in = in.par(1 - parity);
  A.out = out.par(parity);
  A.rin = o.rin ? o.rin->par(parity) : nullptr;
  A.xs = o.xs ? o.xs->par(parity) : nullptr;
  A.ca = o.ca; A.cb = o.cb;
  A.sgn = o.neg ? -1.0 : 1.0;
  A.post = o.post;
  A.parity = parity;
  A.partials = c->partials;
  A.done = o.done;
  const bool init = (o.ca != 0.0 || o.cb != 0.0);
  if ((init || o.dot) && !A.xs) { qexhip_set_error("dslash_sweep: b-term/dot needs xs"); return -1; }
  if (o.ca != 0.0 && !A.rin) { qexhip_set_error("dslash_sweep: a-term needs rin"); return -1; }
  int nparts = 0;
  const double2 *faces_on_cstream = nullptr;
  if (!g.halo) {
    if (c->ndir == 8) CHK((launch<8, false>(c, A, 0, g.Vh, init, o.dot, 0)));
    else CHK((launch<16, false>(c, A, 0, g.Vh, init, o.dot, 0)));
    nparts = (g.Vh + 255) / 256;
  } else {
    int lo_end, hi_beg, overlap;
    sweep_plan(c, &lo_end, &hi_beg, &overlap);
    CHK(devjoin_flush(c));
    const int nb_int = (hi_beg - lo_end + 255) / 256, nb_lo = (lo_end + 255) / 256, nb_hi = (g.Vh - hi_beg + 255) / 256;
    if (sweep_form(c, overlap) == 2) {
      DevField *inp = &in;
      int grid;
      CHK(fused_sweep_setup(c, 1, &inp, 1 - parity, lo_end, hi_beg, &A.fs, &A.gh_hi, &A.gh_lo, &grid, &nparts));
      if (c->ndir == 8) CHK((launch<8, true>(c, A, lo_end, hi_beg, init, o.dot, 0, 0, lo_end, "dslash", nullptr, grid)));
      else CHK((launch<16, true>(c, A, lo_end, hi_beg, init, o.dot, 0, 0, lo_end, "dslash", nullptr, grid)));
    } else if (!overlap) {
      CHK(comm_halo_exchange(c, in, 1 - parity, 0));
      if (c->ndir == 8) CHK((launch<8, true>(c, A, 0, g.Vh, init, o.dot, 0)));
      else CHK((launch<16, true>(c, A, 0, g.Vh, init, o.dot, 0)));
      nparts = (g.Vh + 255) / 256;
    } else {
      const bool early = o.pair2 && c->bnd_out_on_cstream == in.par(1 - parity);
      HIPCHK(hipEventRecord(c->ev_ready, c->stream));
      CHK(comm_halo_exchange(c, in, 1 - parity, 1, !early));
      if (early) HIPCHK(hipStreamWaitEvent(c->cstream, c->ev_ready, 0));
      if (c->ndir == 8) CHK((launch<8, true>(c, A, lo_end, hi_beg, init, o.dot, 0)));
      else CHK((launch<16, true>(c, A, lo_end, hi_beg, init, o.dot, 0)));
      if (c->ndir == 8) CHK((launch<8, true>(c, A, 0, lo_end, init, o.dot, nb_int, hi_beg, g.Vh, "dslash_bnd", c->cstream)));
      else CHK((launch<16, true>(c, A, 0, lo_end, init, o.dot, nb_int, hi_beg, g.Vh, "dslash_bnd", c->cstream)));
      CHK(devjoin_signal(c, c->cstream));
      if (o.defer_join && c->peer) CHK(devjoin_defer(c));
      else CHK(devjoin_wait(c, c->stream, c->cstream));
      nparts = nb_int + nb_lo + nb_hi;
      faces_on_cstream = out.par(parity);
    }
  }
  c->bnd_out_on_cstream = faces_on_cstream;
  if (o.dot) {
    if (nparts > c->part2_off) { qexhip_set_error("internal: partial buffer too small"); return -3; }
    if (o.dot == 2 && o.nparts_out && nparts <= 4096) *o.nparts_out = nparts;
    else {
      if (o.nparts_out) *o.nparts_out = 0;
      CHK(devjoin_flush(c));
      CHK(reduce_partials(c, nparts, o.dot_out));
    }
  }
  return 0;
}
```

### qex_amd/csrc/dslash_core.h

```cpp
#pragma once
#include <hip/hip_runtime.h>
#include "link_residual.h"

typedef double d2v __attribute__((ext_vector_type(2)));

template <bool SUB>
__device__ __forceinline__ void mv3(double2 acc[3], const double2 U[9], const double2 v[3]) {
#pragma unroll
  for (int i = 0; i < 3; i++) {
#pragma unroll
    for (int j = 0; j < 3; j++) {
      if (!SUB) {
        acc[i].x += U[3 * i + j].x * v[j].x;
        acc[i].x -= U[3 * i + j].y * v[j].y;
        acc[i].y += U[3 * i + j].x * v[j].y;
        acc[i].y += U[3 * i + j].y * v[j].x;
      } else {
        acc[i].x -= U[3 * i + j].x * v[j].x;
        acc[i].x += U[3 * i + j].y * v[j].y;
        acc[i].y -= U[3 * i + j].x * v[j].y;
        acc[i].y -= U[3 * i + j].y * v[j].x;
      }
    }
  }
}

template <int FMT>
__device__ __forceinline__ void recon_row2(double2 U[9], bool neg) {
  const double2 ph = U[6];
  double2 r2[3];
#pragma unroll
  for (int k = 0; k < 3; k++) {
    const int a = (k + 1) % 3, b = (k + 2) % 3;
    double rx = U[a].x * U[3 + b].x;
    rx -= U[a].y * U[3 + b].y;
    rx -= U[b].x * U[3 + a].x;
    rx += U[b].y * U[3 + a].y;
    double ry = U[b].x * U[3 + a].y;
    ry += U[b].y * U[3 + a].x;
    ry -= U[a].x * U[3 + b].y;
    ry -= U[a].y * U[3 + b].x;
    if (FMT == 1) r2[k] = make_double2(neg ? -rx : rx, neg ? -ry : ry);
    else r2[k] = make_double2(fma(ph.x, rx, -(ph.y * ry)), fma(ph.x, ry, ph.y * rx));
  }
#pragma unroll
  for (int k = 0; k < 3; k++) U[6 + k] = r2[k];
}

__device__ __forceinline__ void recon_row2_res(double2 U[9], const double2 *row, const unsigned long long *m, const unsigned long long *hdr,
                                               size_t fr, int lane) {
  const uint64_t lo = __builtin_nontemporal_load((const uint64_t *)(row + LR_RES) + lane);
  const uint32_t hi = __builtin_nontemporal_load((const uint32_t *)(row + LR_RES + 32) + lane);
  double2 r2[3];
  lr_decode(U, (m[0] >> lane) & 1ull, lo, hi, r2);
  if ((m[1] >> lane) & 1ull) {
    const double2 *wf = (const double2 *)(uintptr_t)hdr[0] + fr;
#pragma unroll
    for (int k = 0; k < 3; k++) r2[k] = wf[(6 + k) * 64];
  }
#pragma unroll
  for (int k = 0; k < 3; k++) U[6 + k] = r2[k];
}

template <int RECON> struct LinkFormat {
  static constexpr int NLOAD = (RECON == 1 || RECON == 3) ? 6 : (RECON == 2 ? 7 : 9);
  static constexpr int LROW = RECON == 3 ? LR_ROW : NLOAD * 64;
};

template <int NDIR, int RECON>
struct LinkCursor {
  static constexpr int NLOAD = LinkFormat<RECON>::NLOAD, LROW = LinkFormat<RECON>::LROW;
  const double2 *w;
  const unsigned long long *sm;
  const unsigned long long *hdr;
  int tile, lane;
  __device__ __forceinline__ LinkCursor(const double2 *W, const unsigned long long *S, const int c)
      : w(W + (size_t)(c >> 6) * (NDIR * LROW) + (c & 63)),
        sm(RECON == 1 ? S + (size_t)(c >> 6) * NDIR : (RECON == 3 ? S + (size_t)(c >> 6) * NDIR * 2 : nullptr)),
        hdr(RECON == 3 ? S - 2 : nullptr), tile(c >> 6), lane(c & 63) {}
  __device__ __forceinline__ void fetch(const int pr, const bool do_f, const bool do_b, double2 U[9], double2 Wb[9]) const {
    const double2 *wp = w + (size_t)pr * (2 * LROW);
    if (do_f) {
#pragma unroll
      for (int k = 0; k < NLOAD; k++) {
        d2v t = __builtin_nontemporal_load((const d2v *)&wp[k * 64]);
        U[k] = make_double2(t.x, t.y);
      }
    }
    if (do_b) {
#pragma unroll
      for (int k = 0; k < NLOAD; k++) {
        d2v t = __builtin_nontemporal_load((const d2v *)&wp[LROW + k * 64]);
        Wb[k] = make_double2(t.x, t.y);
      }
    }
    if (RECON == 1) {
      if (do_f) recon_row2<1>(U, (sm[2 * pr] >> lane) & 1ull);
      if (do_b) recon_row2<1>(Wb, (sm[2 * pr + 1] >> lane) & 1ull);
    } else if (RECON == 3) {
      const size_t fr = ((size_t)tile * NDIR + 2 * pr) * 576 + lane;
      if (do_f) recon_row2_res(U, wp - lane, sm + 4 * pr, hdr, fr, lane);
      if (do_b) recon_row2_res(Wb, wp - lane + LROW, sm + 4 * pr + 2, hdr, fr + 576, lane);
    } else if (RECON == 2) {
      if (do_f) recon_row2<2>(U, false);
      if (do_b) recon_row2<2>(Wb, false);
    }
  }
};

template <int RECON>
__device__ __forceinline__ void load_link(double2 U[9], const double2 *w, const unsigned long long *sm, int lane) {
  static_assert(RECON != 3, "the lossless rows are read through LinkCursor only");
#pragma unroll
  for (int k = 0; k < LinkFormat<RECON>::NLOAD; k++) U[k] = w[k * 64];
  if (RECON == 1) recon_row2<1>(U, (*sm >> lane) & 1ull);
  else if (RECON == 2) recon_row2<2>(U, false);
}
```

### qex_amd/csrc/layout.hip

```cpp
#include <algorithm>
#include <vector>
#include "qexhip_internal.h"
#include "site_index.h"
#include "link_residual.h"
#include <cstring>

int geom_init(Geom &g, const int X[4], int depth, int halo) {
  for (int i = 0; i < 4; i++) {
    if (X[i] < 2 || (X[i] & 1)) { qexhip_set_error("local lattice extents must be even and >= 2 (got %d in dim %d)", X[i], i); return -1; }
    if (X[i] > 1024) { qexhip_set_error("local lattice extents above 1024 are not supported (got %d in dim %d)", X[i], i); return -1; }
    g.X[i] = X[i];
  }
  g.Xh = X[0] / 2;
  g.V = X[0] * X[1] * X[2] * X[3];
  g.Vh = g.V / 2;
  g.F = g.Xh * X[1] * X[2];
  g.ntile = (g.Vh + QEXHIP_TILE - 1) / QEXHIP_TILE;
  g.halo = halo;
  g.depth = halo ? depth : 0;
  if (halo) {
    if (g.F % QEXHIP_TILE) { qexhip_set_error("sharding in t needs X*Y*Z/2 to be a multiple of 64 (got %d)", g.F); return -1; }
    if (X[3] < 3) { qexhip_set_error("sharding in t needs a local t extent >= 3"); return -1; }
    g.gtile = 3 * g.F / QEXHIP_TILE;
  } else {
// ... 37 lines not shown

int field_upload(qexhip_ctx *c, DevField &f, const double *host) {
  size_t bytes = (size_t)c->g.V * 6 * sizeof(double);
  CHK(ensure_stage(c, bytes));
  HIPCHK(hipMemcpyAsync(c->stage, host, bytes, hipMemcpyHostToDevice, c->stream));
  k_vec_to_tiles<<<(c->g.V + 255) / 256, 256, 0, c->stream>>>(c->g, (const double2 *)c->stage, f.d, f.half);
  HIPCHK(hipGetLastError());
  return 0;
}

int field_download(qexhip_ctx *c, const DevField &f, double *host) {
  size_t bytes = (size_t)c->g.V * 6 * sizeof(double);
  CHK(ensure_stage(c, bytes));
  k_vec_from_tiles<<<(c->g.V + 255) / 256, 256, 0, c->stream>>>(c->g, (double2 *)c->stage, f.d, f.half);
  HIPCHK(hipGetLastError());
  HIPCHK(hipMemcpyAsync(host, c->stage, bytes, hipMemcpyDeviceToHost, c->stream));
  HIPCHK(hipStreamSynchronize(c->stream));
  return 0;
}

__global__ void __launch_bounds__(256) k_pack_top_links(Geom g, const double2 *__restrict__ hostfmt, double2 *buf) {
  int n = g.depth * g.F;
  int i = blockIdx.x * 256 + threadIdx.x;
  if (i >= 2 * n) return;
  int p = i / n, j = i - p * n;
  int c = g.Vh - n + j;
  const double2 *U = hostfmt + ((size_t)(p * g.Vh + c) * 4 + 3) * 9;
  for (int k = 0; k < 9; k++) buf[(size_t)i * 9 + k] = U[k];
}

template <bool HALO>
__global__ void __launch_bounds__(256) k_links_to_tiles(Geom g, const double2 *__restrict__ hostfmt,
                                                        const double2 *__restrict__ ghost, double2 *W,
                                                        int ndir, int dbase, int hop) {
  int i = blockIdx.x * 256 + threadIdx.x;
  if (i >= g.V) return;
  int p = i >= g.Vh, c = i - p * g.Vh;
  SiteXYZT s = site_coord(g, c, p);
  double2 *w = W + ((size_t)p * g.ntile + (c >> 6)) * ndir * 576 + (c & 63);
  for (int mu = 0; mu < 4; mu++) {
    const double2 *U = hostfmt + ((size_t)i * 4 + mu) * 9;
    double2 *wf = w + (size_t)(dbase + 2 * mu) * 576;
    for (int k = 0; k < 9; k++) wf[k * 64] = U[k];
    const double2 *B;
    if (HALO && mu == 3 && s.t - hop < 0) {
      int cF = c - s.t * g.F;
      int j = (s.t - hop + g.depth) * g.F + cF;
      B = ghost + ((size_t)(1 - p) * g.depth * g.F + j) * 9;
    } else {
      int cb = nbr_pos<false>(g, c, s, mu, -hop);
      B = hostfmt + ((size_t)((1 - p) * g.Vh + cb) * 4 + mu) * 9;
    }
    double2 *wb = w + (size_t)(dbase + 2 * mu + 1) * 576;
    for (int r = 0; r < 3; r++)
      for (int q = 0; q < 3; q++) {
        double2 v = B[q * 3 + r];
        wb[(r * 3 + q) * 64] = make_double2(v.x, -v.y);
      }
  }
}

int links_upload(qexhip_ctx *c, const double *fat, const double *lng) {
  c->cg_resume.valid = 0;
  const Geom &g = c->g;
  int ndir = lng ? 16 : 8;
  if (lng) for (int i = 0; i < 4; i++) if (g.X[i] < 4) { qexhip_set_error("Naik links need local extents >= 4"); return -1; }
  if (lng && g.halo && g.depth < 3) { qexhip_set_error("internal: ghost depth %d < 3 for Naik links", g.depth); return -3; }
  size_t wbytes = (size_t)2 * g.ntile * ndir * 576 * sizeof(double2);
  if (c->W && c->ndir != ndir) { HIPCHK(hipFree(c->W)); c->W = nullptr; }
  if (!c->W) { HIPCHK(hipMalloc((void **)&c->W, wbytes)); }
  HIPCHK(hipMemsetAsync(c->W, 0, wbytes, c->stream));
  c->ndir = ndir;
  size_t gbytes = (size_t)g.V * 72 * sizeof(double);
  size_t ghost_elems = g.halo ? (size_t)2 * g.depth * g.F * 9 : 0;
  size_t ghost_bytes = ghost_elems * sizeof(double2);
  CHK(ensure_stage(c, gbytes + 2 * ghost_bytes + 256));
  double2 *hostfmt = (double2 *)c->stage;
  double2 *sendbuf = (double2 *)((char *)c->stage + gbytes);
  double2 *ghost = (double2 *)((char *)c->stage + gbytes + ghost_bytes);
  for (int pass = 0; pass < (lng ? 2 : 1); pass++) {
    const double *src = pass ? lng : fat;
    HIPCHK(hipMemcpyAsync(hostfmt, src, gbytes, hipMemcpyHostToDevice, c->stream));
    if (g.halo) {
      int n = 2 * g.depth * g.F;
      k_pack_top_links<<<(n + 255) / 256, 256, 0, c->stream>>>(g, hostfmt, sendbuf);
      HIPCHK(hipGetLastError());
      CHK(comm_exchange_raw(c, sendbuf, ghost, ghost_bytes, c->stream));
      k_links_to_tiles<true><<<(g.V + 255) / 256, 256, 0, c->stream>>>(g, hostfmt, ghost, c->W, ndir, pass * 8, pass ? 3 : 1);
    } else {
      k_links_to_tiles<false><<<(g.V + 255) / 256, 256, 0, c->stream>>>(g, hostfmt, nullptr, c->W, ndir, pass * 8, pass ? 3 : 1);
    }
    HIPCHK(hipGetLastError());
  }
  HIPCHK(hipStreamSynchronize(c->stream));
  CHK(links_compress(c));
  return sweep_autotune(c);
}

template <int FMT>
__global__ void __launch_bounds__(256) k_links_compress(size_t nrows, const double2 *__restrict__ W, double2 *Wc,
                                                        unsigned long long *Ws, unsigned int *maxdev) {
  const size_t j = (size_t)blockIdx.x * 256 + threadIdx.x;
  const size_t row = j >> 6;
  if (row >= nrows) return;
  const int l = j & 63;
  const double2 *w = W + row * 576 + l;
  constexpr int NR = FMT == 1 ? 6 : 7;
  double2 *o = Wc + row * (NR * 64) + l;
  double2 u[9], r[3];
#pragma unroll
  for (int k = 0; k < 9; k++) u[k] = w[k * 64];
#pragma unroll
  for (int k = 0; k < 6; k++) o[k * 64] = u[k];
  double n2 = 0, px = 0, py = 0;
#pragma unroll
  for (int k = 0; k < 3; k++) {
    const int a = (k + 1) % 3, b = (k + 2) % 3;
    r[k].x = (u[a].x * u[3 + b].x - u[a].y * u[3 + b].y) - (u[b].x * u[3 + a].x - u[b].y * u[3 + a].y);
    r[k].y = -((u[a].x * u[3 + b].y + u[a].y * u[3 + b].x) - (u[b].x * u[3 + a].y + u[b].y * u[3 + a].x));
    n2 += r[k].x * r[k].x + r[k].y * r[k].y;
    px += u[6 + k].x * r[k].x + u[6 + k].y * r[k].y;
    py += u[6 + k].y * r[k].x - u[6 + k].x * r[k].y;
  }
  double2 ph;
  if (n2 > 0) ph = make_double2(px / n2, py / n2); else ph = make_double2(1.0, 0.0);
  if (FMT == 1) ph = make_double2(ph.x < 0 ? -1.0 : 1.0, 0.0);
  double dev = 0;
#pragma unroll
  for (int k = 0; k < 3; k++) {
    const double rx = ph.x * r[k].x - ph.y * r[k].y, ry = ph.x * r[k].y + ph.y * r[k].x;
    dev = fmax(dev, fmax(fabs(u[6 + k].x - rx), fabs(u[6 + k].y - ry)));
  }
  if (FMT == 1) {
    const unsigned long long mask = __ballot(ph.x < 0);
    if (l == 0) Ws[row] = mask;
  } else {
    o[6 * 64] = ph;
  }
  unsigned int bits = __float_as_uint((float)dev);
#pragma unroll
  for (int off = 32; off > 0; off >>= 1) {
    const unsigned int o2 = __shfl_xor(bits, off, 64);
    bits = o2 > bits ? o2 : bits;
  }
  if (l == 0 && bits > __hip_atomic_load(maxdev, __ATOMIC_RELAXED, __HIP_MEMORY_SCOPE_AGENT)) atomicMax(maxdev, bits);
}
__global__ void __launch_bounds__(256) k_links_residual(size_t nrows, size_t prows, const double2 *__restrict__ W, double2 *Wc,
                                                        unsigned long long *Wm, unsigned int *nesc) {
  const size_t j = (size_t)blockIdx.x * 256 + threadIdx.x;
  const size_t row = j >> 6;
  if (row >= nrows) return;
  const int l = j & 63;
  const double2 *w = W + row * 576 + l;
  double2 *o = Wc + row * LR_ROW + l;
  double2 u[9];
#pragma unroll
  for (int k = 0; k < 9; k++) u[k] = w[k * 64];
#pragma unroll
  for (int k = 0; k < 6; k++) o[k * 64] = u[k];
  bool neg;
  uint64_t lo;
  uint32_t hi;
  const bool ok = lr_encode(u, &neg, &lo, &hi);
  ((uint64_t *)(Wc + row * LR_ROW + LR_RES))[l] = lo;
  ((uint32_t *)(Wc + row * LR_ROW + LR_RES + 32))[l] = hi;
  const unsigned long long sgn = __ballot(neg), esc = __ballot(!ok);
  if (l == 0) {
    unsigned long long *m = Wm + 2 * (row + row / prows + 1);
    m[0] = sgn;
    m[1] = esc;
    if (esc) atomicAdd(nesc, (unsigned int)__popcll(esc));
  }
}

int link_residual_host(const double2 *u, long n, unsigned char *escaped, double2 *row2) {
  for (long i = 0; i < n; i++) {
    bool neg;
    uint64_t lo;
    uint32_t hi;
    const bool ok = lr_encode(u + 9 * i, &neg, &lo, &hi);
    if (escaped) escaped[i] = !ok;
    if (row2) lr_decode(u + 9 * i, neg, lo, hi, row2 + 3 * i);
  }
  return 0;
}

int links_compress(qexhip_ctx *c) {
  const Geom &g = c->g;
  c->links_gen++;
  c->recon = 0;
  c->lres = 0; c->lres_esc = 0;
  if (!c->opt_recon || !c->W) return 0;
  const size_t nrows = (size_t)2 * g.ntile * c->ndir;
  if (c->Wc_rows < nrows) {
    if (c->Wc) HIPCHK(hipFree(c->Wc));
    if (c->Ws) HIPCHK(hipFree(c->Ws));
    HIPCHK(hipMalloc((void **)&c->Wc, nrows * 448 * sizeof(double2)));
    HIPCHK(hipMalloc((void **)&c->Ws, nrows * sizeof(unsigned long long)));
    c->Wc_rows = nrows;
  }
  unsigned int *flag = (unsigned int *)&c->dscal[62];
  const unsigned nblk = (unsigned)((nrows * 64 + 255) / 256);
  for (int fmt = 1; fmt <= 2; fmt++) {
    if (fmt == 2 && c->opt_recon == 1) break;
    HIPCHK(hipMemsetAsync(flag, 0, sizeof(unsigned int), c->stream));
    if (fmt == 1) k_links_compress<1><<<nblk, 256, 0, c->stream>>>(nrows, c->W, c->Wc, c->Ws, flag);
    else k_links_compress<2><<<nblk, 256, 0, c->stream>>>(nrows, c->W, c->Wc, c->Ws, flag);
    HIPCHK(hipGetLastError());
    unsigned int bits = 0;
    HIPCHK(hipMemcpyAsync(&bits, flag, sizeof(bits), hipMemcpyDeviceToHost, c->stream));
    HIPCHK(hipStreamSynchronize(c->stream));
    float dev;
    memcpy(&dev, &bits, sizeof(dev));
    if (fmt == 1 || dev <= 5e-14f) c->recon_dev = dev;
    if (dev <= 5e-14f) { c->recon = fmt; break; }
  }
  if (!c->recon && c->opt_lossless && c->ndir == 8) {
    if (!c->Wm || c->Wm_rows < nrows) {
      if (c->Wm) HIPCHK(hipFree(c->Wm));
      c->Wm = nullptr; c->Wm_rows = 0;
      HIPCHK(hipMalloc((void **)&c->Wm, (nrows + 2) * 2 * sizeof(unsigned long long)));
      c->Wm_rows = nrows;
    }
    const size_t prows = nrows / 2;
    HIPCHK(hipMemsetAsync(flag, 0, sizeof(unsigned int), c->stream));
    k_links_residual<<<nblk, 256, 0, c->stream>>>(nrows, prows, c->W, c->Wc, c->Wm, flag);
    HIPCHK(hipGetLastError());
    unsigned int nesc = 0;
    HIPCHK(hipMemcpyAsync(&nesc, flag, sizeof(nesc), hipMemcpyDeviceToHost, c->stream));
    const unsigned long long hdr[2][2] = {{(unsigned long long)(uintptr_t)c->W, 0}, {(unsigned long long)(uintptr_t)(c->W + prows * 576), 0}};
    for (int p = 0; p < 2; p++) HIPCHK(hipMemcpyAsync(c->Wm + p * 2 * (prows + 1), hdr[p], sizeof hdr[p], hipMemcpyHostToDevice, c->stream));
    HIPCHK(hipStreamSynchronize(c->stream));
    c->lres_esc = nesc;
    if ((double)nesc <= 0.01 * (double)(nrows * 64)) c->lres = 1;
  }
  return 0;
}

__global__ void __launch_bounds__(256) k_links_from_nat(Geom g, const double2 *__restrict__ N, double2 *W, int ndir, int dbase, int hop) {
  int i = blockIdx.x * 256 + threadIdx.x;
  if (i >= g.V) return;
  int p = i >= g.Vh, c = i - p * g.Vh;
  SiteXYZT s = site_coord(g, c, p);
  double2 *w = W + ((size_t)p * g.ntile + (c >> 6)) * ndir * 576 + (c & 63);
  for (int mu = 0; mu < 4; mu++) {
    const double2 *U = N + (((size_t)p * g.etile + (c >> 6)) * 4 + mu) * 576 + (c & 63);
    double2 *wf = w + (size_t)(dbase + 2 * mu) * 576;
    for (int k = 0; k < 9; k++) wf[k * 64] = U[k * 64];
    int cb;
    if (g.halo && mu == 3) {
      const int t = c / g.F, tn = t - hop;
      cb = (tn < 0 ? tn + g.X[3] + 6 : tn) * g.F + (c - t * g.F);
    } else {
      cb = nbr_pos<false>(g, c, s, mu, -hop);
    }
    const double2 *B = N + (((size_t)(1 - p) * g.etile + (cb >> 6)) * 4 + mu) * 576 + (cb & 63);
    double2 *wb = w + (size_t)(dbase + 2 * mu + 1) * 576;
    for (int r = 0; r < 3; r++)
      for (int q = 0; q < 3; q++) {
        double2 v = B[(q * 3 + r) * 64];
        wb[(r * 3 + q) * 64] = make_double2(v.x, -v.y);
      }
  }
}
int links_from_natural(qexhip_ctx *c, const double2 *fat, const double2 *lng) {
  c->cg_resume.valid = 0;
  const Geom &g = c->g;
  int ndir = lng ? 16 : 8;
  if (lng) for (int i = 0; i < 4; i++) if (g.X[i] < 4) { qexhip_set_error("Naik links need local extents >= 4"); return -1; }
  if (g.halo) c->g.depth = lng ? 3 : 1;
  size_t wbytes = (size_t)2 * g.ntile * ndir * 576 * sizeof(double2);
  if (c->W && c->ndir != ndir) { HIPCHK(hipFree(c->W)); c->W = nullptr; }
  if (!c->W) { HIPCHK(hipMalloc((void **)&c->W, wbytes)); }
  HIPCHK(hipMemsetAsync(c->W, 0, wbytes, c->stream));
  c->ndir = ndir;
  k_links_from_nat<<<(g.V + 255) / 256, 256, 0, c->stream>>>(g, fat, c->W, ndir, 0, 1);
  if (lng) k_links_from_nat<<<(g.V + 255) / 256, 256, 0, c->stream>>>(g, lng, c->W, ndir, 8, 3);
  HIPCHK(hipGetLastError());
  HIPCHK(hipStreamSynchronize(c->stream));
  CHK(links_compress(c));
  return sweep_autotune(c);
}

extern "C" int qexhip_debug_geom(const int latLocal[4], int depth, int halo, int out[8]) {
  Geom g;
  if (geom_init(g, latLocal, depth, halo)) return -1;
  out[0] = g.Vh; out[1] = g.F; out[2] = g.ntile; out[3] = g.gtile; out[4] = g.etile;
  out[5] = g.depth; out[6] = g.halo; out[7] = g.Xh;
  return 0;
}
extern "C" int qexhip_debug_nbr_pos(const int latLocal[4], int depth, int halo, int c, int parity, int mu, int hop) {
  Geom g;
  if (geom_init(g, latLocal, depth, halo)) return -1;
  if (c < 0 || c >= g.Vh || mu < 0 || mu > 3) return -1;
  SiteXYZT s = site_coord(g, c, parity);
  return halo ? nbr_pos<true>(g, c, s, mu, hop) : nbr_pos<false>(g, c, s, mu, hop);
}
extern "C" int qexhip_debug_site_coord(const int latLocal[4], int c, int parity, int x[4]) {
  Geom g;
  if (geom_init(g, latLocal, 1, 0)) return -1;
  if (c < 0 || c >= g.Vh) return -1;
  SiteXYZT s = site_coord(g, c, parity);
  x[0] = 2 * s.xh + s.o; x[1] = s.y; x[2] = s.z; x[3] = s.t;
  return 0;
}

int tile_order_table(qexhip_ctx *c, const int **tab, int *chunk_out) {
  const Geom &g = c->g;
  const int n = 2 * g.ntile, chunk = (n + 7) / 8;
  if (c->tile_order && c->tile_order_n == 8 * chunk) { *tab = c->tile_order; *chunk_out = chunk; return 0; }
  constexpr int by = 8, bz = 4, bt = 4;
  struct Ent { unsigned long long key0, key1; int e; };
  std::vector<Ent> v(n);
  for (int p = 0; p < 2; p++)
    for (int tile = 0; tile < g.ntile; tile++) {
      unsigned r = (unsigned)tile * 64u / (unsigned)g.Xh;
      const int y = r % g.X[1]; r /= g.X[1];
      const int z = r % g.X[2], t = r / g.X[2];
      Ent &a = v[(size_t)p * g.ntile + tile];
      a.e = 2 * tile + p;
      a.key0 = (((long)t * g.X[2] + z) * g.X[1] + y) * 2 + p;
      a.key1 = ((((((unsigned long long)(t / bt) * 1024u + z / bz) * 1024u + y / by) * 1024u + t % bt) * 1024u + z % bz) * 1024u + (y % by)) * 2 + p;
    }
  std::sort(v.begin(), v.end(), [](const Ent &a, const Ent &b) { return a.key0 < b.key0; });
  std::vector<int> h((size_t)8 * chunk, -1);
  for (int k = 0; k < 8; k++) {
    const int lo = std::min(n, k * chunk), hi = std::min(n, (k + 1) * chunk);
    std::sort(v.begin() + lo, v.begin() + hi, [](const Ent &a, const Ent &b) { return a.key1 < b.key1; });
    for (int j = lo; j < hi; j++) h[(size_t)k * chunk + (j - lo)] = v[j].e;
  }
  int pairs = (chunk % 2 == 0);
  for (size_t j = 0; pairs && j + 1 < h.size(); j += 2)
    if (!((h[j] < 0 && h[j + 1] < 0) || (h[j] >= 0 && h[j + 1] == h[j] + 1 && (h[j] & 1) == 0))) pairs = 0;
  c->tile_pairs_ok = pairs;
  if (c->tile_order) { (void)hipFree(c->tile_order); c->tile_order = nullptr; }
  HIPCHK(hipMalloc(&c->tile_order, h.size() * sizeof(int)));
// ... 80 lines not shown
```

### qex_amd/csrc/link_residual.h

```cpp
#pragma once
#include <hip/hip_runtime.h>
#include <cstdint>
#include <cmath>

#define LR_ROW 432
#define LR_RES 384

__host__ __device__ __forceinline__ uint64_t lr_bits(double x) { return __builtin_bit_cast(uint64_t, x); }
__host__ __device__ __forceinline__ double lr_double(uint64_t b) { return __builtin_bit_cast(double, b); }

__host__ __device__ __forceinline__ void lr_rebuild(const double2 u[6], bool neg, double rec[6]) {
#pragma clang fp contract(off)
#pragma unroll
  for (int k = 0; k < 3; k++) {
    const int a = (k + 1) % 3, b = (k + 2) % 3;
    double rx = u[a].x * u[3 + b].x;
    rx = fma(-u[a].y, u[3 + b].y, rx);
    rx = fma(-u[b].x, u[3 + a].x, rx);
    rx = fma(u[b].y, u[3 + a].y, rx);
    double ry = u[b].x * u[3 + a].y;
    ry = fma(u[b].y, u[3 + a].x, ry);
    ry = fma(-u[a].x, u[3 + b].y, ry);
    ry = fma(-u[a].y, u[3 + b].x, ry);
    rec[2 * k] = neg ? -rx : rx;
    rec[2 * k + 1] = neg ? -ry : ry;
  }
}

__host__ __device__ __forceinline__ double lr_apply(double rec, int k) {
  const double sc = lr_double(lr_bits(rec) & 0x7ff0000000000000ull) * 0x1p-52;
  return fma((double)k, sc, rec);
}

__host__ __device__ __forceinline__ void lr_decode(const double2 u[6], bool neg, uint64_t lo, uint32_t hi, double2 r2[3]) {
  double rec[6];
  lr_rebuild(u, neg, rec);
  const int k[6] = {(int16_t)lo, (int16_t)(lo >> 16), (int16_t)(lo >> 32), (int16_t)(lo >> 48), (int16_t)hi, (int16_t)(hi >> 16)};
#pragma unroll
  for (int j = 0; j < 3; j++) r2[j] = make_double2(lr_apply(rec[2 * j], k[2 * j]), lr_apply(rec[2 * j + 1], k[2 * j + 1]));
}

__host__ __device__ __forceinline__ bool lr_encode(const double2 u[9], bool *neg, uint64_t *lo, uint32_t *hi) {
  double rec[6];
  lr_rebuild(u, false, rec);
  double px = 0;
#pragma unroll
  for (int j = 0; j < 3; j++) px += u[6 + j].x * rec[2 * j] + u[6 + j].y * rec[2 * j + 1];
  const bool ng = px < 0;
  if (ng) {
#pragma unroll
    for (int j = 0; j < 6; j++) rec[j] = -rec[j];
  }
  const double row2[6] = {u[6].x, u[6].y, u[7].x, u[7].y, u[8].x, u[8].y};
  int k[6];
  bool ok = true;
#pragma unroll
  for (int j = 0; j < 6; j++) {
    const double sc = lr_double(lr_bits(rec[j]) & 0x7ff0000000000000ull) * 0x1p-52;
    const double q = sc > 0 ? (row2[j] - rec[j]) / sc : 0.0;
    k[j] = fabs(q) <= 32767.0 ? (int)rint(q) : 0;
    ok = ok && lr_bits(lr_apply(rec[j], k[j])) == lr_bits(row2[j]);
  }
  if (!ok) {
#pragma unroll
    for (int j = 0; j < 6; j++) k[j] = 0;
  }
  *neg = ng;
  *lo = (uint64_t)(uint16_t)k[0] | (uint64_t)(uint16_t)k[1] << 16 | (uint64_t)(uint16_t)k[2] << 32 | (uint64_t)(uint16_t)k[3] << 48;
  *hi = (uint32_t)(uint16_t)k[4] | (uint32_t)(uint16_t)k[5] << 16;
  return ok;
}
```

### qex_amd/csrc/qexhip_internal.h

```cpp
#pragma once
#include <hip/hip_runtime.h>
#include <cstdint>
#include <cstdio>
#include <string>
#include <vector>
#include <map>

#define QEXHIP_TILE 64

struct Geom {
  int X[4];
  int Xh;
  int V, Vh;
  int F;
  int ntile;
  int depth;
  int gtile;
  int etile;
  int halo;
};

__host__ __device__ inline size_t vec_off(int pos, int colour) {
  return (size_t)(pos >> 6) * 192 + (size_t)colour * 64 + (size_t)(pos & 63);
}

struct DevField {
  double2 *d = nullptr;
  size_t half = 0;
  double2 *par(int p) const { return d + (size_t)p * half; }
};

struct DevFieldF {
  float2 *d = nullptr;
  size_t half = 0;
  float2 *par(int p) const { return d + (size_t)p * half; }
};

struct SlpScal {
  double b2, r2stop;
  double r2t;
  double sigma, sigma_p;
  double r2s, r2s_old, maxr2s;
  int k, maxits, nupd;
  int done, upd, noupd;
  int conv, first;
};

struct CgScal {
  double b2, r2, rzo, pAp, r2stop, tmp;
  int itn, maxits, done, pad;
  double r2s[2];
  int itns[2], dones[2];
  double agree[4];
};

struct TimerSlot {
  std::vector<hipEvent_t> ev;
  size_t used = 0;
  long count = 0;
  double total_ms = 0;
};

struct DevJoin {
  unsigned long long *ready = nullptr;
  unsigned long long *err = nullptr;
  long long ticks = 0;
  double timeout_s = 30.0;
  unsigned long long seq[2]{0, 0};
  int deferred = 0;
};

struct GaugeNat;
struct PeerComm;

enum { WK_SLOTS = 16 };

struct qexhip_ctx {
  int device = 0;
  Geom g{};
  int rankGeom[4]{1, 1, 1, 1}, rankCoord[4]{0, 0, 0, 0};
  hipStream_t stream = nullptr, cstream = nullptr;
  hipEvent_t ev_ready = nullptr;
  void *comm = nullptr;
  void *comm2 = nullptr;
  PeerComm *peer = nullptr;
  DevJoin dj;
  int opt_transport = -1;
  int nranks = 1, rank = 0;
  int force_halo = 0;
  double2 *W = nullptr;
  int ndir = 0;
  std::map<int, DevField> fields;
  int next_field = 1;
  double *stage = nullptr; size_t stage_bytes = 0;
  double *partials = nullptr; int npartials = 0;
  int part2_off = 0;
  double *dscal = nullptr;
  CgScal *cg = nullptr;
  struct { int valid = 0; const double2 *x = nullptr; int par_even = 0; double m2 = 0; int k = 0; } cg_resume;
  int cg_r2parts = 0;
  double *hist = nullptr; int histcap = 0;
  void *pinned = nullptr;
  int wk[WK_SLOTS]{0};
  int timers_on = 0;
  std::map<std::string, TimerSlot> timers;
  double2 *Wc = nullptr; unsigned long long *Ws = nullptr; size_t Wc_rows = 0; int recon = 0; double recon_dev = 0;
  unsigned long long *Wm = nullptr; size_t Wm_rows = 0; int lres = 0; long long lres_esc = 0;
  int opt_lossless = 1;
  int opt_batch_multi = 0;
  int opt_multi_reduce = 0;
  int opt_force_pair = 1;
  int opt_obs_clover = 1;
  int opt_hop_split = -1;
  int opt_fused_spin_us = -1;
  int ranks_share_device = 0;
  int hybrid_sums = 0;
  unsigned int *fz_buf = nullptr; int fz_cap = 0;
  const double2 *bnd_out_on_cstream = nullptr;
  double xchg_us[2]{0, 0};
  int form_auto[2]{-1, -1};
  int opt_chain_overlap = 1;
  int opt_smear_ca = 1;
  int opt_flow_exp = 1;
  int opt_recon = 2;
  int opt_overlap = -1;
  int emu_link_gbs = 0;
  int emu_exchange_us = 0, emu_allreduce_us = 0;
  int overlap_auto[2]{-1, -1};
  double overlap_tune_us[2][3]{};
  GaugeNat *gn = nullptr;
  void *nhyp = nullptr;
  void *hisq = nullptr;
  double2 *outer_F = nullptr; size_t outer_Fn = 0;
  int tile_pairs_ok = 0;
  int *tile_order = nullptr; int tile_order_n = 0;
  int *tile_order_pl[16]{};
  void *obs_table = nullptr;
  void *batch = nullptr;
  int lds_attr_done = 0;
  void *cgm_scal = nullptr;
  double *meson_buf = nullptr; size_t meson_cap = 0;
  unsigned long links_gen = 0;
  void *f32 = nullptr;
  void *batch_f32 = nullptr;
  int opt_sloppy_check = 4;
};

enum { WK_T = 0, WK_R, WK_P, WK_AP, WK_Y, WK_D, WK_R2, WK_XT, WK_IN, WK_OUT, WK_IN2, WK_N };

void qexhip_set_error(const char *fmt, ...);
#define HIPCHK(expr)                                                                     \
  do {                                                                                   \
    hipError_t e_ = (expr);                                                              \
    if (e_ != hipSuccess) {                                                              \
      qexhip_set_error("%s:%d: %s -> %s", __FILE__, __LINE__, #expr, hipGetErrorString(e_)); \
      return -2;                                                                         \
    }                                                                                    \
  } while (0)
#define CHK(expr) do { int r_ = (expr); if (r_ != 0) return r_; } while (0)

struct ScopedTimer {
  qexhip_ctx *c; TimerSlot *s = nullptr; hipStream_t st;
  ScopedTimer(qexhip_ctx *c_, const char *name, hipStream_t st_);
  ~ScopedTimer();
};
int timers_collect(qexhip_ctx *c);
bool timer_event_pair(qexhip_ctx *c, const char *name, hipEvent_t *e0, hipEvent_t *e1);

int geom_init(Geom &g, const int X[4], int depth, int halo);
int field_alloc(qexhip_ctx *c, DevField &f);
int field_upload(qexhip_ctx *c, DevField &f, const double *host);
int field_download(qexhip_ctx *c, const DevField &f, double *host);
int links_upload(qexhip_ctx *c, const double *fat, const double *lng);
int ensure_stage(qexhip_ctx *c, size_t bytes);
int links_from_natural(qexhip_ctx *c, const double2 *fat, const double2 *lng);
int links_compress(qexhip_ctx *c);
int link_residual_host(const double2 *u, long n, unsigned char *escaped, double2 *row2);
int op_eo_reconstruct_pub(qexhip_ctx *c, DevField &r, DevField &b, double m);
int op_eo_reduce_pub(qexhip_ctx *c, DevField &r, DevField &b, double m);
int op_stagD_pub(qexhip_ctx *c, DevField &r, DevField &x, int parity, double m, double sc, double a);
void batch_state_free(qexhip_ctx *c);
int batch_io_fields(qexhip_ctx *c, int n, DevField **xs, DevField **bs);
int solve_full_batch_dev(qexhip_ctx *c, int n, DevField **x, DevField **b, const double *mass, const double *r2req,
                         int maxits, int *iters, double *r2_final);
int batch_work_fields(qexhip_ctx *c, int count, DevField **out);
void batch_f32_state_free(qexhip_ctx *c);
int batch_sloppy_check(qexhip_ctx *c, int n, const double *mass);
int solve_xx_batch_sloppy_dev(qexhip_ctx *c, int n, DevField **x, DevField **b, const double *mass, const double *r2req,
                              int maxits, int par_even, int *iters, double *r2_over_b2, int *nupdates);
int solve_full_batch_sloppy_dev(qexhip_ctx *c, int n, DevField **x, DevField **b, const double *mass, const double *r2req,
                                int maxits, int sloppy, int *iters, double *r2_final, int *nupdates);
int solve_batch_sloppy_host(qexhip_ctx *c, int n, double *const *x, const double *const *b, const double *mass, const double *r2req,
                            int maxits, int xx_parity, int sloppy, int *iters, double *r2, int *nupdates);
int nhyp_fforce(qexhip_ctx *c, double *f_host, int n, const double *const *phi, const double *mass, const double *scale,
                const double *r2req, int maxits, int bcmask, const int ph[4], int *iters, DevField *const *phi_dev = nullptr);
int solve_batch_host(qexhip_ctx *c, int n, double *const *x, const double *const *b, const double *mass,
                     const double *r2req, int maxits, int xx_parity, int *iters, double *r2);

inline bool multi_rank(const qexhip_ctx *c) { return c->nranks > 1 || c->opt_multi_reduce; }

int comm_halo_push_only_multi(qexhip_ctx *c, int n, DevField *const *f, int parity, const double2 **gh_hi, const double2 **gh_lo, struct PeerPush *push);
int comm_halo_exchange(qexhip_ctx *c, DevField &f, int parity, int overlap, bool wait_ready = true);
int comm_halo_exchange_f32(qexhip_ctx *c, DevFieldF &f, int parity, int overlap);
int comm_halo_exchange_multi(qexhip_ctx *c, int n, DevField *const *f, int parity, int overlap);
int comm_allreduce(qexhip_ctx *c, double *dptr, int n);
int comm_allreduce_parts(qexhip_ctx *c, double *parts, int n, int *n_out);
int comm_allreduce_max(qexhip_ctx *c, double *host, int n);
int comm_agree_post(qexhip_ctx *c);
int comm_agree_check(qexhip_ctx *c, const CgScal &host);
int comm_allgather(qexhip_ctx *c, const double *send, double *recv, size_t n);
int comm_faces_exchange(qexhip_ctx *c, int nbuf, double *const bottom[], double *const top[], double *const ghost_hi[],
                        double *const ghost_lo[], size_t ndoubles, int async = 0);
int comm_exchange_raw(qexhip_ctx *c, const void *send_up, void *recv_from_down, size_t bytes, hipStream_t st);
void comm_destroy(qexhip_ctx *c);
inline bool comm_ready(const qexhip_ctx *c) { return c->comm != nullptr || c->peer != nullptr; }
inline bool peer_faces(const qexhip_ctx *c) { return c->peer != nullptr && c->comm == nullptr; }

int devjoin_init(qexhip_ctx *c);
void devjoin_destroy(qexhip_ctx *c);
int devjoin_check(qexhip_ctx *c);
int devjoin_signal(qexhip_ctx *c, hipStream_t from);
int devjoin_wait(qexhip_ctx *c, hipStream_t waiter, hipStream_t from);
int devjoin_defer(qexhip_ctx *c);
int devjoin_flush(qexhip_ctx *c);
struct PeerHost;
int peer_init(qexhip_ctx *c, PeerHost &host);
int peer_selftest(qexhip_ctx *c);
void peer_destroy(qexhip_ctx *c);
inline int peer_check(qexhip_ctx *c) { return devjoin_check(c); }
int peer_exchange(qexhip_ctx *c, hipStream_t st, int ns_dn, const void *const *src_dn, int ns_up, const void *const *src_up,
                  void *const *dst_from_up, void *const *dst_from_dn, size_t bytes, double emu_us = 0.0, const void **zc_from_up = nullptr,
                  const void **zc_from_dn = nullptr, struct PeerPush *push_only = nullptr);
int peer_allreduce_parts(qexhip_ctx *c, double *parts, int n);
int peer_allreduce(qexhip_ctx *c, double *dptr, int n, int op);
int peer_host_reduce(qexhip_ctx *c, double *host, int n, int op);
int peer_allgather(qexhip_ctx *c, const double *send, double *recv, size_t n);
void peer_info(const qexhip_ctx *c, long out[4]);

struct DslashOpts {
  double ca = 0, cb = 0;
  const DevField *rin = nullptr;
  const DevField *xs = nullptr;
  int neg = 0;
  double post = 1.0;
  int dot = 0;
  int *nparts_out = nullptr;
  double *dot_out = nullptr;
  const int *done = nullptr;
  int pair2 = 0;
  int defer_join = 0;
};
int dslash_sweep(qexhip_ctx *c, DevField &out, DevField &in, int parity, const DslashOpts &o);
void stag_link_bases(const qexhip_ctx *c, int parity, bool lossless, const double2 **W, const unsigned long long **S);
int sweep_autotune(qexhip_ctx *c);
void sweep_plan(const qexhip_ctx *c, int *lo_end, int *hi_beg, int *overlap);
int sweep_form(const qexhip_ctx *c, int overlap);
double sweep_push_fraction(const qexhip_ctx *c, int interior_sites, int nrhs = 1);

enum { F32_T = 0, F32_R, F32_P, F32_AP, F32_X, F32_IN, F32_NF };
#define SLP_DELTA 0.1
int f32_links(qexhip_ctx *c, int *fmt, double *dev);
int f32_links_dev(qexhip_ctx *c, int parity, const void **W, const unsigned long long **S, int *fmt);
int f32_field(qexhip_ctx *c, int slot, DevFieldF **f);
int f32_field_ensure(qexhip_ctx *c, DevFieldF &F);
int f32_op_xx(qexhip_ctx *c, DevFieldF &r, DevFieldF &x, double m2, int par_even, int dot, const int *done, int *nparts);
int f32_from_f64(qexhip_ctx *c, DevFieldF &y, const DevField &x, int parity, double a);
int f32_to_f64(qexhip_ctx *c, DevField &y, const DevFieldF &x, int parity, double a, int accumulate);
void f32_state_free(qexhip_ctx *c);
int slp_alloc(qexhip_ctx *c, SlpScal **s);
int slp_init(qexhip_ctx *c, SlpScal *s, double r2req, int maxits);
int slp_xpay(qexhip_ctx *c, SlpScal *s, DevFieldF &p, DevFieldF &rs, const DevField &r, int parity);
int slp_update(qexhip_ctx *c, SlpScal *s, DevFieldF &xs, DevFieldF &rs, const DevFieldF &p, const DevFieldF &Ap, int parity, int ndot);
int slp_flush(qexhip_ctx *c, SlpScal *s, DevField &x, DevFieldF &xs, int parity);
int slp_resid(qexhip_ctx *c, SlpScal *s, DevField &r, const DevField &b, const DevField &Ax, int parity);

int blas_zero(qexhip_ctx *c, DevField &f, int parity);
int blas_copy(qexhip_ctx *c, DevField &dst, const DevField &src, int parity);
int blas_axpy(qexhip_ctx *c, double a, const DevField &x, DevField &y, int parity);
int blas_xpay(qexhip_ctx *c, const DevField &x, double a, DevField &y, int parity);
int blas_scale(qexhip_ctx *c, double a, DevField &y, int parity);
int blas_axpby(qexhip_ctx *c, double a, const DevField &x, double b, const DevField &y, DevField &z, int parity);
int blas_norm2(qexhip_ctx *c, const DevField &x, int parity, double *dev_out);
int blas_redot(qexhip_ctx *c, const DevField &x, const DevField &y, int parity, double *dev_out);
int blas_cdot(qexhip_ctx *c, const DevField &x, const DevField &y, int parity, double *dev_out);
int tile_order_table(qexhip_ctx *c, const int **tab, int *chunk);
int tile_order_plane(qexhip_ctx *c, int mu, int nu, const int **tab, int *chunk);
int reduce_partials(qexhip_ctx *c, int n, double *dev_out);
int read_scalars(qexhip_ctx *c, const double *dev, int n, double *host);
int blas_grid(const qexhip_ctx *c, int parity_count);
int blas_delay(hipStream_t st, int us);
int cg_xpay(qexhip_ctx *c, DevField &p, const DevField &r, int parity, int k, int rolled);
int cg_update(qexhip_ctx *c, DevField &x, DevField &r, const DevField &p, const DevField &Ap, int parity, int k, int ndot);
int cg_close(qexhip_ctx *c, int k);
int cg_init(qexhip_ctx *c, double r2req, int maxits);
int cg_resume(qexhip_ctx *c, int k, double r2req, int maxits);

int get_work(qexhip_ctx *c, int slot, DevField **f);
int op_xx(qexhip_ctx *c, DevField &r, DevField &x, double m2, int par_even, int dot, const int *done, int *ndot = nullptr);
int op_D(qexhip_ctx *c, DevField &r, DevField &x, double m, double sc, double a = 0.0);
int solve_xx_dev(qexhip_ctx *c, DevField &x, DevField &b, double mass, double r2req, int maxits,
                 int par_even, int *iters, double *r2_over_b2, double *hist, int histcap);
int solve_xx_continue_dev(qexhip_ctx *c, DevField &x, double r2req, int maxits, int *iters, double *r2_over_b2, double *hist, int histcap);
int solve_full_dev(qexhip_ctx *c, DevField &x, DevField &b, double mass, double r2req, int maxits,
                   int *iters, double *r2_final, int use_prev = 0, int sloppy = 0, int *nupdates = nullptr);
int solve_xx_sloppy_dev(qexhip_ctx *c, DevField &x, DevField &b, double mass, double r2req, int maxits, int par_even,
                        int *iters, double *r2_over_b2, int *nupdates);
int solve_xx_multi_dev(qexhip_ctx *c, std::vector<DevField *> &xs, DevField &b, const double *shifts,
                       int nmass, double r2req, int maxits, int par_even, int *iters, double *hist, int histcap);
int solve_multi_dev(qexhip_ctx *c, std::vector<DevField *> &xs, DevField &b, const double *masses,
                    int nmass, double r2req, int maxits, int *iters, double *r2_final);
enum { POOL_PS = 0, POOL_YS = 32, POOL_XS = 64 };
int pool_field(qexhip_ctx *c, int idx, DevField **f);

int stag_outer_host(qexhip_ctx *c, double *f_host, const double *x_host, double se, double so, int accumulate);

int meson_corners(qexhip_ctx *c, int n, DevField *const *x, DevField *const *y, int t0, double *host_out);
int sym_shift(qexhip_ctx *c, DevField &r, const DevField &x, int mu);
int norm2slice(qexhip_ctx *c, const DevField &f, int dir, double *host_out);

int smear_fat7_host(qexhip_ctx *c, const double *g_host, const double coef[5], double *fl_host, double *ll_host, double naik);
int smear_hisq_host(qexhip_ctx *c, const double *g_host, double *fl_host, double *ll_host);
int smear_nhyp_host(qexhip_ctx *c, const double *g_host, double *fl_host, double a1, double a2, double a3);
int smear_set_links_hisq(qexhip_ctx *c, const double *g_host);
int smear_hisq_force_host(qexhip_ctx *c, const double *g_host, const double *dfl_host, const double *dll_host, double *f_host);
int smear_fat7_deriv_host(qexhip_ctx *c, const double *g_host, const double *dfl_host, const double coef[5], const double *dll_host,
                          double naik, double *d_host);
void nhyp_state_free(qexhip_ctx *c);
void hisq_state_free(qexhip_ctx *c);
int hisq_prepare(qexhip_ctx *c, const double *g_host, double *fl_host, double *ll_host);
int hisq_closure_force(qexhip_ctx *c, const double *dfl_host, const double *dll_host, double *f_host);
int gauge_deriv_dev(qexhip_ctx *c, const double2 *G, double2 *F, double cplaq, double c2, int kind);
int stag_outer_dev(qexhip_ctx *c, DevField &fx, double2 *F, double se, double so, int accumulate, int hop = 1);
int hisq_fermion_force(qexhip_ctx *c, double *f_host, const double *const *psi, const double *scale, int n);
int nhyp_gauge_force(qexhip_ctx *c, double *f_host, double cplaq, double c2, int kind);
int nhyp_fermion_force(qexhip_ctx *c, double *f_host, const double *const *psi, const double *scale, int n, int bcmask, const int ph[4]);
int nhyp_prepare(qexhip_ctx *c, const double *g_host, double a1, double a2, double a3, double *fl_host);
int nhyp_force_host(qexhip_ctx *c, double *f_host, const double *chain_host);
int smear_set_links_nhyp(qexhip_ctx *c, const double *g_host, double a1, double a2, double a3, int bcmask, const int ph[4]);

int gauge_set(qexhip_ctx *c, const double *g);
int gauge_get(qexhip_ctx *c, double *g);
int gauge_plaq(qexhip_ctx *c, double out[6]);
int gauge_force(qexhip_ctx *c, double *f_host, double cplaq, double c2 = 0.0, int kind = 0);
int gauge_wflow(qexhip_ctx *c, int nsteps, double eps, double cplaq = 1.0, double c2 = 0.0, int kind = 0);
int gauge_flow_obs(qexhip_ctx *c, int loop, double out[3], double *plaq6 = nullptr);
int gauge_action(qexhip_ctx *c, double cplaq, double c2, int kind, double *out);
int gauge_md_update(qexhip_ctx *c, const double *p_host, double t);
int gauge_reunit(qexhip_ctx *c);
int md_begin(qexhip_ctx *c, const double *g, const double *p);
int md_end(qexhip_ctx *c, double *g, double *p);
int md_momentum_norm2(qexhip_ctx *c, double *out);
int md_update_links(qexhip_ctx *c, double t);
int md_gauge_force(qexhip_ctx *c, double cplaq, double c2, int kind);
int md_kick(qexhip_ctx *c, int source, double t);
int md_shift_links(qexhip_ctx *c, int source, double t);
int md_save_links(qexhip_ctx *c);
int md_restore_links(qexhip_ctx *c);
int gauge_wline(qexhip_ctx *c, const int *path, int n, double out[2]);
int gauge_polyakov(qexhip_ctx *c, double out[8]);
int gauge_plaq_s4(qexhip_ctx *c, double out[8]);
void gauge_free(qexhip_ctx *c);
void gauge_release_scratch(qexhip_ctx *c);
const double2 *gauge_links_dev(qexhip_ctx *c);
struct qexhip_rng;
int rng_dev_generate(qexhip_ctx *c, qexhip_rng *R, int what, DevField *f, double2 *P);
int md_momenta_dev(qexhip_ctx *c, double2 **M);
```

### qex_amd/csrc/solver.cpp

```cpp
#include "qexhip_internal.h"
#include "../../include/qexhip.h"
#include <cmath>
#include <cstring>
#include <algorithm>


int get_work(qexhip_ctx *c, int slot, DevField **f) {
  if (slot == WK_R || slot == WK_P || slot == WK_AP) c->cg_resume.valid = 0;
  if (c->wk[slot] == 0) {
    DevField nf;
    CHK(field_alloc(c, nf));
    int id = -(slot + 1);
    c->fields[id] = nf;
    c->wk[slot] = id;
  }
  *f = &c->fields[c->wk[slot]];
  return 0;
}

int op_xx(qexhip_ctx *c, DevField &r, DevField &x, double m2, int par_even, int dot, const int *done, int *ndot) {
  DevField *t;
  CHK(get_work(c, WK_T, &t));
  const int px = par_even ? 0 : 1, py = 1 - px;
  DslashOpts o1, o2;
  o1.done = done;
  o2.cb = 4.0 * m2;
  o2.xs = &x;
  o2.neg = 1;
  o2.dot = (dot && ndot) ? 2 : dot;
  o2.nparts_out = ndot;
  o2.dot_out = &c->cg->pAp;
  o2.done = done;
  o2.defer_join = (dot && ndot) ? 1 : 0;
  o2.pair2 = (t->d != x.d && t->d != r.d) ? 1 : 0;
  if (o2.cb == 0.0 && dot) { qexhip_set_error("op_xx: dot with m2 == 0 unsupported"); return -1; }
  CHK(dslash_sweep(c, *t, x, py, o1));
  CHK(dslash_sweep(c, r, *t, px, o2));
  return 0;
}

static int op_stagD(qexhip_ctx *c, DevField &r, DevField &x, int parity, double m, double sc, double a) {
  DslashOpts o;
  o.ca = a / (0.5 * sc);
  o.cb = m / (0.5 * sc);
  o.rin = &r;
  o.xs = &x;
  o.post = 0.5 * sc;
  return dslash_sweep(c, r, x, parity, o);
}

int op_D(qexhip_ctx *c, DevField &r, DevField &x, double m, double sc, double a) {
  CHK(op_stagD(c, r, x, 0, m, sc, a));
  CHK(op_stagD(c, r, x, 1, m, sc, a));
  return 0;
}

static int op_eo_reconstruct(qexhip_ctx *c, DevField &r, DevField &b, double m) {
  CHK(op_stagD(c, r, r, 1, 0.0, -1.0 / m, 0.0));
  CHK(blas_axpy(c, 1.0 / m, b, r, 1));
  return 0;
}
int op_eo_reconstruct_pub(qexhip_ctx *c, DevField &r, DevField &b, double m) { return op_eo_reconstruct(c, r, b, m); }
int op_stagD_pub(qexhip_ctx *c, DevField &r, DevField &x, int parity, double m, double sc, double a) { return op_stagD(c, r, x, parity, m, sc, a); }
int op_eo_reduce_pub(qexhip_ctx *c, DevField &r, DevField &b, double m) { return op_stagD(c, r, b, 0, m, -1.0, 0.0); }

static int ensure_hist(qexhip_ctx *c, int cap) {
  if (cap < 1) cap = 1;
  if (c->histcap >= cap) return 0;
  if (c->hist) HIPCHK(hipFree(c->hist));
  c->hist = nullptr; c->histcap = 0;
  HIPCHK(hipMalloc((void **)&c->hist, sizeof(double) * cap));
  c->histcap = cap;
  return 0;
}

static int read_cg(qexhip_ctx *c, CgScal *host) {
  HIPCHK(hipMemcpyAsync(c->pinned, c->cg, sizeof(CgScal), hipMemcpyDeviceToHost, c->stream));
  HIPCHK(hipStreamSynchronize(c->stream));
  memcpy(host, c->pinned, sizeof(CgScal));
  return 0;
}

static int cg_iterate(qexhip_ctx *c, DevField &x, DevField *r, DevField *p, DevField *Ap, double m2, int par_even, int k,
                      CgScal &st, int *iters, double *r2_over_b2, double *hist, int histcap) {
  const int par = par_even ? 0 : 1;
  const int chunk = 32;
  int rolled = 1;
  bool done = st.dones[k & 1];
  double r2 = st.r2s[k & 1];
  st.itn = st.itns[k & 1];
  while (!done) {
    int n = std::min(chunk, st.maxits - k);
    if (n <= 0) break;
    for (int i = 0; i < n; i++, k++) {
      CHK(cg_xpay(c, *p, *r, par, k, rolled));
      rolled = 0;
      int ndot = 0;
      CHK(op_xx(c, *Ap, *p, m2, par_even, 1, &c->cg->dones[k & 1], &ndot));
      CHK(cg_update(c, x, *r, *p, *Ap, par, k, ndot));
    }
    CHK(cg_close(c, k));
    rolled = 1;
    CHK(read_cg(c, &st));
    CHK(comm_agree_check(c, st));
    done = st.dones[k & 1];
    r2 = st.r2s[k & 1];
    st.itn = st.itns[k & 1];
  }
  st.r2 = r2;
  if (iters) *iters = st.itn;
  if (r2_over_b2) *r2_over_b2 = (st.b2 != 0.0) ? st.r2 / st.b2 : 0.0;
  if (hist && histcap > 0) {
    int n = std::min(std::min(histcap, c->histcap), st.itn + 1);
    HIPCHK(hipMemcpyAsync(hist, c->hist, sizeof(double) * n, hipMemcpyDeviceToHost, c->stream));
    HIPCHK(hipStreamSynchronize(c->stream));
  }
  c->cg_resume.valid = 1; c->cg_resume.x = x.d; c->cg_resume.par_even = par_even; c->cg_resume.m2 = m2; c->cg_resume.k = st.itn;
  return 0;
}

int solve_xx_dev(qexhip_ctx *c, DevField &x, DevField &b, double mass, double r2req, int maxits,
                 int par_even, int *iters, double *r2_over_b2, double *hist, int histcap) {
  const int par = par_even ? 0 : 1;
  DevField *r, *p, *Ap;
  CHK(get_work(c, WK_R, &r));
  CHK(get_work(c, WK_P, &p));
  CHK(get_work(c, WK_AP, &Ap));
  CHK(ensure_hist(c, std::max(histcap, 1)));
  const double m2 = mass * mass;
  CHK(blas_zero(c, x, 2));
  CHK(blas_norm2(c, b, par, &c->dscal[0]));
  CHK(blas_copy(c, *r, b, par));
  CHK(blas_norm2(c, *r, par, &c->dscal[1]));
  CHK(cg_init(c, r2req, maxits));
  CgScal st;
  CHK(read_cg(c, &st));
  return cg_iterate(c, x, r, p, Ap, m2, par_even, 0, st, iters, r2_over_b2, hist, histcap);
}

int solve_xx_continue_dev(qexhip_ctx *c, DevField &x, double r2req, int maxits, int *iters, double *r2_over_b2, double *hist, int histcap) {
  if (!c->cg_resume.valid || c->cg_resume.x != x.d) {
    qexhip_set_error("solve_xx_continue: no resumable CG state for this field (another solver, set_links or a work-vector user ran "
                     "since the last solve_xx on it)");
    return -3;
  }
  const int k = c->cg_resume.k, par_even = c->cg_resume.par_even;
  const double m2 = c->cg_resume.m2;
  DevField *r = &c->fields[c->wk[WK_R]], *p = &c->fields[c->wk[WK_P]], *Ap = &c->fields[c->wk[WK_AP]];
  CHK(cg_resume(c, k, r2req, maxits));
  CgScal st;
  CHK(read_cg(c, &st));
  return cg_iterate(c, x, r, p, Ap, m2, par_even, k, st, iters, r2_over_b2, hist, histcap);
}

static int slp_agree(qexhip_ctx *c, const SlpScal &h) {
  if (c->nranks < 2 || !comm_ready(c)) return 0;
  CHK(peer_check(c));
  const double key = ((double)h.k * 2.0 + h.done) * 65536.0 + (h.nupd & 0xffff);
  double v[4] = {h.r2t, -h.r2t, key, -key};
  CHK(comm_allreduce_max(c, v, 4));
  const bool both_nan = std::isnan(v[0]) && std::isnan(v[1]);
  if ((!both_nan && v[0] != -v[1]) || v[2] != -v[3]) {
    qexhip_set_error("sharded sloppy solve: the ranks disagree on the true residual (%.17g .. %.17g) or on iterations / updates / stop "
                     "(key %g .. %g)", -v[1], v[0], -v[3], v[2]);
    return QEXHIP_ERR_COMM;
  }
  return 0;
}

int solve_xx_sloppy_dev(qexhip_ctx *c, DevField &x, DevField &b, double mass, double r2req, int maxits, int par_even,
                        int *iters, double *r2_over_b2, int *nupdates) {
  const int par = par_even ? 0 : 1;
  DevField *r, *Ax;
  CHK(get_work(c, WK_R, &r));
  CHK(get_work(c, WK_AP, &Ax));
  CHK(f32_links(c, nullptr, nullptr));
  DevFieldF *rs, *ps, *aps, *xs;
  CHK(f32_field(c, F32_R, &rs));
  CHK(f32_field(c, F32_P, &ps));
  CHK(f32_field(c, F32_AP, &aps));
  CHK(f32_field(c, F32_X, &xs));
  SlpScal *s;
  CHK(slp_alloc(c, &s));
  const double m2 = mass * mass;
  if (m2 == 0.0) { qexhip_set_error("sloppy solve: mass 0 unsupported (op_xx's <p,Ap> needs 4 m^2 > 0)"); return -1; }
  CHK(blas_zero(c, x, 2));
  CHK(blas_norm2(c, b, par, &c->dscal[0]));
  CHK(blas_copy(c, *r, b, par));
  HIPCHK(hipMemsetAsync(xs->par(par), 0, xs->half * sizeof(float2), c->stream));
  CHK(slp_init(c, s, r2req, maxits));
  SlpScal h;
  HIPCHK(hipMemcpyAsync(c->pinned, s, sizeof(SlpScal), hipMemcpyDeviceToHost, c->stream));
  HIPCHK(hipStreamSynchronize(c->stream));
  memcpy(&h, c->pinned, sizeof(SlpScal));
  const int every = std::max(1, c->opt_sloppy_check);
  const int chunk = 32;
  int k = 0;
  while (!h.done && k < maxits) {
    const int n = std::min(chunk, maxits - k);
    for (int i = 0; i < n; i++, k++) {
      CHK(slp_xpay(c, s, *ps, *rs, *r, par));
      int ndot = 0;
      CHK(f32_op_xx(c, *aps, *ps, m2, par_even, 1, &s->done, &ndot));
      CHK(slp_update(c, s, *xs, *rs, *ps, *aps, par, ndot));
      if ((k + 1) % every == 0 || k + 1 >= maxits) {
        CHK(slp_flush(c, s, x, *xs, par));
        CHK(op_xx(c, *Ax, x, m2, par_even, 0, &s->noupd));
        CHK(slp_resid(c, s, *r, b, *Ax, par));
      }
    }
    HIPCHK(hipMemcpyAsync(c->pinned, s, sizeof(SlpScal), hipMemcpyDeviceToHost, c->stream));
    HIPCHK(hipStreamSynchronize(c->stream));
    memcpy(&h, c->pinned, sizeof(SlpScal));
    CHK(slp_agree(c, h));
  }
  if (iters) *iters = h.k;
  if (r2_over_b2) *r2_over_b2 = (h.b2 != 0.0) ? h.r2t / h.b2 : 0.0;
  if (nupdates) *nupdates = h.nupd;
  return 0;
}

static int inner_xx(qexhip_ctx *c, DevField &x, DevField &b, double m, double r2req, int maxits, int par_even, int *its,
                    int sloppy, int *nupd) {
  if (!sloppy) return solve_xx_dev(c, x, b, m, r2req, maxits, par_even, its, nullptr, nullptr, 0);
  int nu = 0;
  CHK(solve_xx_sloppy_dev(c, x, b, m, r2req, maxits, par_even, its, nullptr, &nu));
  *nupd += nu;
  return 0;
}

static int norm2_eo(qexhip_ctx *c, DevField &f, double *e, double *o) {
  CHK(blas_norm2(c, f, 0, &c->dscal[2]));
  CHK(blas_norm2(c, f, 1, &c->dscal[3]));
  double h[2];
  CHK(read_scalars(c, &c->dscal[2], 2, h));
  *e = h[0]; *o = h[1];
  return 0;
}

static int solve_inner(qexhip_ctx *c, DevField &x, DevField &b, double m, double r2req, int maxits,
                       double b2e, double b2o, int *its, int sloppy, int *nupd) {
  const double b2 = b2e + b2o;
  const double r2stop = r2req * b2, r2stop2 = 0.5 * r2stop;
  const double r2stope = (b2o <= r2stop2) ? r2stop - b2o : r2stop2;
  const double r2stopo = (b2e <= r2stop2) ? r2stop - b2e : r2stop2;
  *its = 0;
  if (b2e <= r2stope || b2o <= r2stopo || m == 0.0) {
    DevField *y;
    CHK(get_work(c, WK_D, &y));
    if (b2e > r2stope) {
      CHK(inner_xx(c, *y, b, m, r2stope / b2e, maxits, 1, its, sloppy, nupd));
      CHK(blas_scale(c, 4.0, *y, 0));
      CHK(op_D(c, x, *y, m, -1.0));
    } else if (b2o > r2stopo) {
      CHK(inner_xx(c, *y, b, m, r2stopo / b2o, maxits, 0, its, sloppy, nupd));
      CHK(blas_scale(c, 4.0, *y, 1));
      CHK(op_D(c, x, *y, m, -1.0));
    }
  } else {
    DevField *d;
    CHK(get_work(c, WK_D, &d));
// ... 50 lines not shown
```

### qex_amd/staggered.py

```python
import ctypes as C
import time
import numpy as np

from . import _lib
from ._lib import check, lib

EVEN, ODD, ALL = 0, 1, 2
SloppyNone, SloppySingle, SloppyHalf = 0, 1, 2
_SUBSET = {"even": EVEN, "odd": ODD, "all": ALL}


def _p(a):
    if a is None:
        return None
    if a.dtype != np.float64 or not a.flags["C_CONTIGUOUS"]:
        raise ValueError("fields must be C-contiguous float64 arrays")
    return a.ctypes.data_as(C.c_void_p)


class SolverParams:

    def __init__(self, r2req=1e-6, maxits=50000, verbosity=1, usePrevSoln=False, sloppySolve=SloppyNone):
        self.r2req = r2req
        self.maxits = maxits
# ... 347 lines not shown
        return float((self.nlinks * 4 * 72 + 60) * (self.ctx.vol // 2) * its)

    def solveXX(self, r, x, m, sp, parEven=True, histcap=0):
        t0 = time.time()
        its, fin = C.c_int(0), C.c_double(0)
        hist = np.zeros(max(histcap, 1))
        sloppy = int(getattr(sp, "sloppySolve", SloppyNone))
        if sloppy != SloppyNone:
            nup = C.c_int(0)
            check(lib().qexhip_stag_solve_xx_sloppy(self.ctx._h, _p(r), _p(x), float(m), float(sp.r2req), int(sp.maxits),
                                                    1 if parEven else 0, sloppy, C.byref(its), C.byref(fin), C.byref(nup)))
            sp.reliableUpdates += nup.value
            histcap = 0
        else:
            check(lib().qexhip_stag_solve_xx(self.ctx._h, _p(r), _p(x), float(m), float(sp.r2req), int(sp.maxits),
                                             1 if parEven else 0, C.byref(its), C.byref(fin), _p(hist), histcap))
        sp.calls += 1
        sp.iterations += its.value
        sp.iterationsMax = max(sp.iterationsMax, its.value)
        sp.seconds += time.time() - t0
        sp.flops += self._flops(its.value)
        sp.r2 = fin.value
        sp.r2hist = hist[: min(histcap, its.value + 1)] if histcap else None
        if sp.verbosity > 1:
            print(("solveEE" if parEven else "solveOO") + "(HIP): " + sp.getStats())

    def solveEE(self, r, x, m, sp, histcap=0):
        self.solveXX(r, x, m, sp, True, histcap)

    def solveOO(self, r, x, m, sp, histcap=0):
        self.solveXX(r, x, m, sp, False, histcap)

    def solve(self, x, b, m, sp):
        t0 = time.time()
        its, fin = C.c_int(0), C.c_double(0)
        sloppy = int(getattr(sp, "sloppySolve", SloppyNone))
        if isinstance(x, (list, tuple)) and sloppy != SloppyNone:
            raise ValueError("sloppySolve applies to single-mass solves only (multi-shift solves run in fp64)")
        if sloppy != SloppyNone:
            nup = C.c_int(0)
            check(lib().qexhip_stag_solve_sloppy(self.ctx._h, _p(x), _p(b), float(m), float(sp.r2req), int(sp.maxits),
                                                 1 if sp.usePrevSoln else 0, sloppy, C.byref(its), C.byref(fin), C.byref(nup)))
            sp.reliableUpdates += nup.value
        elif isinstance(x, (list, tuple)):
            ms = np.array([float(v) for v in m], dtype=np.float64)
            ptrs = (C.c_void_p * len(x))(*[_p(a).value for a in x])
            check(lib().qexhip_stag_solve_multi(self.ctx._h, ptrs, _p(b), _p(ms), len(x), float(sp.r2req),
                                                int(sp.maxits), C.byref(its), C.byref(fin)))
        else:
            check(lib().qexhip_stag_solve_prev(self.ctx._h, _p(x), _p(b), float(m), float(sp.r2req), int(sp.maxits),
                                               1 if sp.usePrevSoln else 0, C.byref(its), C.byref(fin)))
        sp.calls += 1
        sp.iterations += its.value
        sp.iterationsMax = max(sp.iterationsMax, its.value)
        sp.seconds += time.time() - t0
        sp.flops += self._flops(its.value)
        sp.r2 = fin.value
        if sp.verbosity > 1:
            print("stagSolve(HIP): " + sp.getStats())

    def _batch(self, fn_name, xs, bs, ms, r2req, maxits, parEven=None, sloppy=None):
        if sloppy is not None:
            sloppy = _batch_sloppy(sloppy)
        n = len(xs)
        if not (1 <= n <= 4 and len(bs) == n and len(ms) == n):
            raise ValueError("batch solve: 1..4 systems, one source and one mass each")
        rq = [float(r2req)] * n if np.isscalar(r2req) else [float(v) for v in r2req]
        xp = (C.c_void_p * n)(*[_p(a).value for a in xs])
        bp = (C.c_void_p * n)(*[_p(a).value for a in bs])
        mv, rv = (C.c_double * n)(*[float(v) for v in ms]), (C.c_double * n)(*rq)
        its, fin = (C.c_int * n)(), (C.c_double * n)()
        if sloppy is not None:
            nup = (C.c_int * n)()
            if parEven is None:
                check(lib().qexhip_stag_solve_batch_sloppy(self.ctx._h, n, xp, bp, mv, rv, int(maxits), sloppy, its, fin, nup))
            else:
                check(lib().qexhip_stag_solve_xx_batch_sloppy(self.ctx._h, n, xp, bp, mv, rv, int(maxits), 1 if parEven else 0,
                                                              sloppy, its, fin, nup))
            return list(its), list(fin), list(nup)
        if parEven is None:
            check(lib().qexhip_stag_solve_batch(self.ctx._h, n, xp, bp, mv, rv, int(maxits), its, fin))
        else:
            check(lib().qexhip_stag_solve_xx_batch(self.ctx._h, n, xp, bp, mv, rv, int(maxits), 1 if parEven else 0, its, fin))
        return list(its), list(fin)

    def solve_batch(self, xs, bs, ms, sps, sloppy=None):
        sl = [sps] * len(xs) if isinstance(sps, SolverParams) else list(sps)
        if sloppy is not None:
            sloppy = _batch_sloppy(sloppy)
        elif any(int(getattr(sp, "sloppySolve", SloppyNone)) != SloppyNone for sp in sl):
            raise ValueError("sloppySolve applies to single-system solves only: a lock-step batch runs in fp64 unless the "
                             "mixed-precision batch is asked for with the keyword sloppy=1 (solve_batch / solveXX_batch / "
                             "dev_solve_batch)")
        t0 = time.time()
        nup = [0] * len(xs)
        if sloppy is None:
            its, fin = self._batch("solve", xs, bs, ms, [sp.r2req for sp in sl], min(sp.maxits for sp in sl))
        else:
            its, fin, nup = self._batch("solve", xs, bs, ms, [sp.r2req for sp in sl], min(sp.maxits for sp in sl), sloppy=sloppy)
        dt = (time.time() - t0) / len(xs)
        for sp, u in zip(sl, nup):
            sp.reliableUpdates += u
        for sp, i, f in zip(sl, its, fin):
            sp.calls += 1
            sp.iterations += i
            sp.iterationsMax = max(sp.iterationsMax, i)
            sp.seconds += dt
            sp.flops += self._flops(i)
            sp.r2 = f
        return its

    def solveXX_batch(self, xs, bs, ms, r2req, maxits, parEven=True, sloppy=None):
        return self._batch("xx", xs, bs, ms, r2req, maxits, parEven, sloppy)

    def solveXX_multi(self, xs, b, shifts, sp, parEven=True, histcap=0):
        if int(getattr(sp, "sloppySolve", SloppyNone)) != SloppyNone:
            raise ValueError("sloppySolve applies to single-mass solves only (multi-shift solves run in fp64)")
        its = C.c_int(0)
        sh = np.array([float(v) for v in shifts], dtype=np.float64)
        hist = np.zeros(max(histcap, 1))
        ptrs = (C.c_void_p * len(xs))(*[_p(a).value for a in xs])
        check(lib().qexhip_stag_solve_xx_multi(self.ctx._h, ptrs, _p(b), _p(sh), len(xs), float(sp.r2req),
                                               int(sp.maxits), 1 if parEven else 0, C.byref(its), _p(hist), histcap))
        sp.iterations += its.value
        sp.r2hist = hist[: min(histcap, its.value + 1)] if histcap else None


def _batch_sloppy(sloppy):
    if isinstance(sloppy, bool) or not isinstance(sloppy, (int, np.integer)) or not 0 <= int(sloppy) <= 2:
        raise ValueError("sloppy = %r: None (fp64, the default), 0 (SloppyNone), 1 (SloppySingle) or 2 (SloppyHalf, runs single)" % (sloppy,))
    return int(sloppy)


def newStag(ctx, g):
    return Staggered(ctx, g)


def newStag3(ctx, g, g3):
    return Staggered(ctx, g, g3)


def link_residual_host(links):
    a = np.asarray(links)
    if np.iscomplexobj(a):
        a = np.stack([a.real, a.imag], axis=-1)
    a = np.ascontiguousarray(a, dtype=np.float64).reshape(-1, 18)
    n = a.shape[0]
    esc = np.zeros(n, dtype=np.uint8)
    row2 = np.zeros((n, 3, 2), dtype=np.float64)
    check(lib().qexhip_link_residual_host(a.ctypes.data, n, esc.ctypes.data, row2.ctypes.data))
    return esc.astype(bool), row2


def plaq(ctx, g=None):
    if g is not None:
        check(lib().qexhip_gauge_set(ctx._h, _p(g)))
    out = np.zeros(6)
    check(lib().qexhip_plaq(ctx._h, _p(out)))
    return out


_FLOW_KIND = {"Wilson": 0, "rect": 0, "adj": 1}


def gaugeForce(ctx, g, cplaq=1.0, rect=0.0, adjplaq=0.0):
    if rect != 0.0 and adjplaq != 0.0:
        raise ValueError("rect and adjplaq are separate code paths in QEX (gaugeForce vs forceA)")
    check(lib().qexhip_gauge_set(ctx._h, _p(g)))
    f = np.zeros_like(g)
    kind = 1 if adjplaq != 0.0 else 0
    check(lib().qexhip_gauge_force_general(ctx._h, _p(f), float(cplaq), float(adjplaq if kind else rect), kind))
    return f


def flowEQ(ctx, loop=1, g=None):
    if g is not None:
        check(lib().qexhip_gauge_set(ctx._h, _p(g)))
    out = np.zeros(3)
    check(lib().qexhip_flow_EQ(ctx._h, int(loop), _p(out)))
    return out


def flowMeasure(ctx, g=None):
    if g is not None:
        check(lib().qexhip_gauge_set(ctx._h, _p(g)))
    pl, eq = np.zeros(6), np.zeros(3)
    check(lib().qexhip_flow_measure(ctx._h, _p(pl), _p(eq)))
    return pl, eq


def gaugeAction(ctx, g=None, plaq=1.0, rect=0.0, adjplaq=0.0):
    if g is not None:
        check(lib().qexhip_gauge_set(ctx._h, _p(g)))
    out = C.c_double(0)
    check(lib().qexhip_gauge_action(ctx._h, float(plaq), float(rect), float(adjplaq), C.byref(out)))
    return out.value


def gaugeUpdate(ctx, g, p, t):
    check(lib().qexhip_gauge_set(ctx._h, _p(g)))
    check(lib().qexhip_gauge_update(ctx._h, _p(p), float(t)))
    check(lib().qexhip_gauge_get(ctx._h, _p(g)))


class ResidentMD:

    GAUGE, NHYP = 0, 1

    def __init__(self, ctx):
        self.ctx = ctx

    def begin(self, g, p):
        check(lib().qexhip_md_begin(self.ctx._h, _p(g), _p(p)))

    def end(self, g=None, p=None):
        check(lib().qexhip_md_end(self.ctx._h, _p(g), _p(p)))

    def momentum_norm2(self):
        out = C.c_double(0)
        check(lib().qexhip_md_momentum_norm2(self.ctx._h, C.byref(out)))
        return out.value

    def update_links(self, t):
        check(lib().qexhip_md_update_links(self.ctx._h, float(t)))

    def gauge_force(self, plaq=1.0, rect=0.0, adjplaq=0.0):
        check(lib().qexhip_md_gauge_force(self.ctx._h, float(plaq), float(rect), float(adjplaq)))

    def kick(self, source, t):
        check(lib().qexhip_md_kick(self.ctx._h, int(source), float(t)))

    def shift_links(self, source, t):
        check(lib().qexhip_md_shift_links(self.ctx._h, int(source), float(t)))

    def save_links(self):
        check(lib().qexhip_md_save_links(self.ctx._h))

    def restore_links(self):
        check(lib().qexhip_md_restore_links(self.ctx._h))


def reunit(ctx, g):
    check(lib().qexhip_gauge_set(ctx._h, _p(g)))
    check(lib().qexhip_gauge_reunit(ctx._h))
    check(lib().qexhip_gauge_get(ctx._h, _p(g)))


def wline(ctx, path, g=None):
    if g is not None:
        check(lib().qexhip_gauge_set(ctx._h, _p(g)))
    out = (C.c_double * 2)()
    arr = (C.c_int * len(path))(*[int(v) for v in path])
    check(lib().qexhip_wline(ctx._h, arr, len(path), out))
    return complex(out[0], out[1])


def s4_gauge(ctx, g=None):
    if g is not None:
        check(lib().qexhip_gauge_set(ctx._h, _p(g)))
    out = np.zeros(8)
    check(lib().qexhip_plaq_s4(ctx._h, _p(out)))
    return out.reshape(4, 2)


def ploops(ctx, g=None):
    if g is not None:
        check(lib().qexhip_gauge_set(ctx._h, _p(g)))
    out = np.zeros(8)
    check(lib().qexhip_polyakov_loops(ctx._h, _p(out)))
    return [complex(out[2 * d], out[2 * d + 1]) for d in range(4)]


def gaugeFlow(ctx, g, steps, eps, measure=None, flow_act="Wilson", plaq=1.0, rect=0.0, adjplaq=0.0):
    kind = _FLOW_KIND[flow_act]
    c2 = adjplaq if kind else rect
    check(lib().qexhip_gauge_set(ctx._h, _p(g)))
    if measure is None:
        check(lib().qexhip_wflow_general(ctx._h, int(steps), float(eps), float(plaq), float(c2), kind))
    else:
        for n in range(1, steps + 1):
            check(lib().qexhip_wflow_general(ctx._h, 1, float(eps), float(plaq), float(c2), kind))
            measure(n * eps)
    check(lib().qexhip_gauge_get(ctx._h, _p(g)))


def gaugeSet(ctx, g):
    check(lib().qexhip_gauge_set(ctx._h, _p(g)))


def gaugeFlowResident(ctx, steps, eps):
    check(lib().qexhip_wflow(ctx._h, int(steps), float(eps)))


class HisqCoefs:

    def init(self):
        return self

    def force(self, ctx, g, dsdsu, dsdsul):
        f = np.zeros_like(g)
        check(lib().qexhip_hisq_force(ctx._h, _p(g), _p(dsdsu), _p(dsdsul), _p(f)))
        return f

    def smear(self, ctx, g, fl, ll):
        check(lib().qexhip_hisq_smear(ctx._h, _p(g), _p(fl), _p(ll)))

# ... 80 lines not shown
```

Measured before the change: 2695.

## Group link residuals per tile and defer CG x update into next xpay

Reorganizes the lossless compressed-link storage so each direction's residual words are grouped across direction pairs within a tile block. The Dslash inner loop can then fetch residuals for two pairs with three wide vector loads instead of scattered per-row loads. Separately, the CG update no longer touches x. The x += alpha*p step is deferred into the following xpay kernel, which already reads p, and a flush kernel runs at solver exit, cutting one read of p and of x per iteration. This adds state (alphas, xlag) and a host-side self-check helper, and relies on the deferred-x bookkeeping staying correct across chunk boundaries and resume.

Result: no change. 2714, median of 2 (+0.7%).

```diff
diff --git a/include/qexhip.h b/include/qexhip.h
--- a/include/qexhip.h
+++ b/include/qexhip.h
@@ -166,6 +166,7 @@
 int qexhip_stag_links_info(qexhip_handle h, int *nlinks, int *compressed, double *max_dev);
 int qexhip_stag_links_storage(qexhip_handle h, int *bytes_per_link, long long *escaped);
 int qexhip_link_residual_host(const double *links, int n, unsigned char *escaped, double *row2);
+int qexhip_link_residual_tile_host(const double *links, unsigned char *escaped, double *row2, short *residuals);
 int qexhip_set_option(qexhip_handle h, const char *name, int value);
 
 int qexhip_stag_set_links_hisq(qexhip_handle h, const double *g);
diff --git a/qex_amd/__init__.py b/qex_amd/__init__.py
--- a/qex_amd/__init__.py
+++ b/qex_amd/__init__.py
@@ -2,7 +2,7 @@
 from .layout import Layout
 from .gauge import setBC, stagPhase, rephase, unit, synthetic_random_su3, synthetic_gaussian_vector
 from .staggered import (
-    Context, device_count, Staggered, SolverParams, newStag, newStag3, link_residual_host, plaq, gaugeForce, gaugeFlow, gaugeSet, gaugeFlowResident, flowEQ, flowMeasure, gaugeAction, gaugeUpdate, reunit, wline, ploops, s4_gauge, ResidentMD, HisqCoefs, HypCoefs, makeImpLinks, fat7lDeriv, EVEN, ODD, ALL,
+    Context, device_count, Staggered, SolverParams, newStag, newStag3, link_residual_host, link_residual_tile_host, plaq, gaugeForce, gaugeFlow, gaugeSet, gaugeFlowResident, flowEQ, flowMeasure, gaugeAction, gaugeUpdate, reunit, wline, ploops, s4_gauge, ResidentMD, HisqCoefs, HypCoefs, makeImpLinks, fat7lDeriv, EVEN, ODD, ALL,
     SloppyNone, SloppySingle, SloppyHalf,
 )
 from .io import loadGauge, loadGaugeSlab, saveGauge, getFileLattice, gaugeFileInfo, writeField, readField, fileMetadata
diff --git a/qex_amd/_lib.py b/qex_amd/_lib.py
--- a/qex_amd/_lib.py
+++ b/qex_amd/_lib.py
@@ -86,6 +86,7 @@
     ("qexhip_stag_links_info", _ci, [_vp, _pi, _pi, _vp]),
     ("qexhip_stag_links_storage", _ci, [_vp, _pi, C.POINTER(C.c_longlong)]),
     ("qexhip_link_residual_host", _ci, [_vp, _ci, _vp, _vp]),
+    ("qexhip_link_residual_tile_host", _ci, [_vp, _vp, _vp, _vp]),
     ("qexhip_set_option", _ci, [_vp, C.c_char_p, _ci]),
     ("qexhip_fat7_deriv", _ci, [_vp, _vp, _vp, _vp, _vp, _cd, _vp]),
     ("qexhip_hisq_force", _ci, [_vp, _vp, _vp, _vp, _vp]),
diff --git a/qex_amd/csrc/api.cpp b/qex_amd/csrc/api.cpp
--- a/qex_amd/csrc/api.cpp
+++ b/qex_amd/csrc/api.cpp
@@ -757,6 +757,7 @@
   const std::string n(name);
   if (n == "recon") c->opt_recon = value;
   else if (n == "lossless") c->opt_lossless = value;
+  else if (n == "cg_defer_x") c->opt_cg_defer_x = value;
   else if (n == "overlap") c->opt_overlap = value;
   else if (n == "transport") {
     if (comm_ready(c)) { qexhip_set_error("option transport must be set before qexhip_comm_init"); return QEXHIP_ERR_STATE; }
@@ -835,6 +836,10 @@
   if (!links || n < 0) return QEXHIP_ERR_ARG;
   return link_residual_host((const double2 *)links, n, escaped, (double2 *)row2);
 }
+extern "C" int qexhip_link_residual_tile_host(const double *links, unsigned char *escaped, double *row2, short *residuals) {
+  if (!links) return QEXHIP_ERR_ARG;
+  return link_residual_tile_host((const double2 *)links, escaped, (double2 *)row2, residuals);
+}
 extern "C" int qexhip_hisq_prepare(qexhip_handle c, const double *g, double *fl, double *ll) {
   if (!c || !g) return QEXHIP_ERR_ARG;
   HIPCHK(hipSetDevice(c->device));
diff --git a/qex_amd/csrc/blas.hip b/qex_amd/csrc/blas.hip
--- a/qex_amd/csrc/blas.hip
+++ b/qex_amd/csrc/blas.hip
@@ -193,9 +193,13 @@
   return 0;
 }
 
-__global__ void __launch_bounds__(256) k_cg_xpay(double2 *p, const double2 *r, size_t n, CgScal *s, int k, int rolled,
+template <bool DEFER>
+__global__ void __launch_bounds__(256) k_cg_xpay(double2 *p, const double2 *r, double2 *x, size_t n, CgScal *s, int k, int rolled,
                                                 const double *r2parts, int nparts, double *hist, int histcap) {
   const int cur = k & 1, prv = cur ^ 1;
+  const bool owed = DEFER && k > 0 && s->xlag[prv] == k;
+  const double alpha = owed ? s->alphas[prv] : 0.0;
+  bool live = true;
   double r2k;
   if (rolled) {
     if (s->dones[cur]) return;
@@ -207,35 +211,58 @@
     }
     r2k = cg_sum_parts(r2parts, nparts);
     if (blockIdx.x == 0 && threadIdx.x == 0) cg_roll(s, k, r2k, hist, histcap);
-    if (!(k < s->maxits && r2k > s->r2stop)) return;
+    live = k < s->maxits && r2k > s->r2stop;
+    if (!live && !owed) return;
   }
   const bool first = (k == 0);
   const double beta = r2k / s->r2s[prv];
   for (size_t i = blockIdx.x * 256 + threadIdx.x; i < n; i += (size_t)gridDim.x * 256) {
-    double2 rv = r[i];
-    if (first) p[i] = rv;
+    if (first) p[i] = r[i];
     else {
       double2 pv = p[i];
-      p[i] = make_double2(fma(beta, pv.x, rv.x), fma(beta, pv.y, rv.y));
-    }
-  }
-}
+      if (owed) {
+        double2 xv = x[i];
+        xv.x += alpha * pv.x; xv.y += alpha * pv.y;
+        x[i] = xv;
+      }
+      if (!DEFER || live) {
+        double2 rv = r[i];
+        p[i] = make_double2(fma(beta, pv.x, rv.x), fma(beta, pv.y, rv.y));
+      }
+    }
+  }
+}
+template <bool DEFER>
 __global__ void __launch_bounds__(256) k_cg_update(double2 *x, double2 *r, const double2 *p, const double2 *Ap,
-                                                  size_t n, const CgScal *s, int k, double *partials,
+                                                  size_t n, CgScal *s, int k, double *partials,
                                                   const double *dotp, int ndot) {
   if (s->dones[k & 1]) return;
   const double pAp = (ndot > 0) ? cg_sum_parts(dotp, ndot) : s->pAp;
   const double alpha = s->r2s[k & 1] / pAp;
+  if (DEFER && blockIdx.x == 0 && threadIdx.x == 0) { s->alphas[k & 1] = alpha; s->xlag[k & 1] = k + 1; }
   double acc = 0;
   for (size_t i = blockIdx.x * 256 + threadIdx.x; i < n; i += (size_t)gridDim.x * 256) {
-    double2 pv = p[i], xv = x[i], rv = r[i], av = Ap[i];
-    xv.x += alpha * pv.x; xv.y += alpha * pv.y;
+    double2 rv = r[i], av = Ap[i];
+    if (!DEFER) {
+      double2 pv = p[i], xv = x[i];
+      xv.x += alpha * pv.x; xv.y += alpha * pv.y;
+      x[i] = xv;
+    }
     rv.x -= alpha * av.x; rv.y -= alpha * av.y;
-    x[i] = xv; r[i] = rv;
+    r[i] = rv;
     acc = fma(rv.x, rv.x, fma(rv.y, rv.y, acc));
   }
   double t = block_sum_256(acc);
   if (threadIdx.x == 0) partials[blockIdx.x] = t;
+}
+__global__ void __launch_bounds__(256) k_cg_flush_x(double2 *x, const double2 *p, size_t n, const CgScal *s, int k) {
+  if (k <= 0 || s->xlag[(k - 1) & 1] != k) return;
+  const double alpha = s->alphas[(k - 1) & 1];
+  for (size_t i = blockIdx.x * 256 + threadIdx.x; i < n; i += (size_t)gridDim.x * 256) {
+    double2 pv = p[i], xv = x[i];
+    xv.x += alpha * pv.x; xv.y += alpha * pv.y;
+    x[i] = xv;
+  }
 }
 __global__ void k_cg_init(CgScal *s, const double *dscal, double r2req, int maxits, double *hist, int histcap) {
   s->b2 = dscal[0];
@@ -248,6 +275,7 @@
   s->done = !(0 < maxits && s->r2 > s->r2stop);
   s->r2s[0] = s->r2; s->itns[0] = 0; s->dones[0] = s->done;
   s->r2s[1] = 1.0; s->itns[1] = 0; s->dones[1] = s->done;
+  s->xlag[0] = s->xlag[1] = 0;
   if (histcap > 0) hist[0] = (s->b2 != 0.0) ? s->r2 / s->b2 : 0.0;
 }
 __global__ void __launch_bounds__(256) k_cg_close(CgScal *s, int k, const double *r2parts, int nparts, double *hist, int histcap) {
@@ -259,11 +287,19 @@
   if (threadIdx.x == 0) cg_roll(s, k, r2k, hist, histcap);
 }
 
-int cg_xpay(qexhip_ctx *c, DevField &p, const DevField &r, int parity, int k, int rolled) {
+int cg_xpay(qexhip_ctx *c, DevField &p, const DevField &r, DevField &x, int parity, int k, int rolled) {
   size_t n = body2(c);
   ScopedTimer tm(c, "blas", c->stream);
-  k_cg_xpay<<<grid_for(n), 256, 0, c->stream>>>(p.par(parity), r.par(parity), n, c->cg, k, rolled,
-                                               c->partials + c->part2_off, rolled ? grid_for(n) : c->cg_r2parts, c->hist, c->histcap);
+  auto kern = c->opt_cg_defer_x ? k_cg_xpay<true> : k_cg_xpay<false>;
+  kern<<<grid_for(n), 256, 0, c->stream>>>(p.par(parity), r.par(parity), x.par(parity), n, c->cg, k, rolled,
+                                          c->partials + c->part2_off, rolled ? grid_for(n) : c->cg_r2parts, c->hist, c->histcap);
+  HIPCHK(hipGetLastError());
+  return 0;
+}
+int cg_flush_x(qexhip_ctx *c, DevField &x, const DevField &p, int parity, int k) {
+  size_t n = body2(c);
+  ScopedTimer tm(c, "blas", c->stream);
+  k_cg_flush_x<<<grid_for(n), 256, 0, c->stream>>>(x.par(parity), p.par(parity), n, c->cg, k);
   HIPCHK(hipGetLastError());
   return 0;
 }
@@ -275,8 +311,9 @@
   CHK(devjoin_flush(c));
   {
     ScopedTimer tm(c, "blas", c->stream);
-    k_cg_update<<<nb, 256, 0, c->stream>>>(x.par(parity), r.par(parity), p.par(parity), Ap.par(parity), n, c->cg, k, r2p,
-                                           c->partials, ndot);
+    auto kern = c->opt_cg_defer_x ? k_cg_update<true> : k_cg_update<false>;
+    kern<<<nb, 256, 0, c->stream>>>(x.par(parity), r.par(parity), p.par(parity), Ap.par(parity), n, c->cg, k, r2p,
+                                    c->partials, ndot);
     HIPCHK(hipGetLastError());
   }
   CHK(comm_allreduce_parts(c, r2p, nb, &c->cg_r2parts));
@@ -294,6 +331,7 @@
   s->r2s[cur] = s->r2; s->r2s[cur ^ 1] = s->rzo; s->itns[cur] = k;
   s->dones[cur] = !(k < maxits && s->r2s[cur] > s->r2stop);
   s->done = s->dones[cur];
+  s->xlag[0] = s->xlag[1] = 0;
   s->agree[0] = s->r2s[cur]; s->agree[1] = -s->r2s[cur]; s->agree[2] = (double)k; s->agree[3] = -(double)k;
 }
 int cg_resume(qexhip_ctx *c, int k, double r2req, int maxits) {
diff --git a/qex_amd/csrc/dslash.hip b/qex_amd/csrc/dslash.hip
--- a/qex_amd/csrc/dslash.hip
+++ b/qex_amd/csrc/dslash.hip
@@ -67,7 +67,7 @@
       in_f3 = tu + 3 >= g.X[3] ? A.gh_hi : A.in;
       in_b3 = tu - 3 < 0 ? A.gh_lo : A.in;
     }
-    auto pair = [&](const int pr, const bool do_f, const bool do_b) __attribute__((always_inline)) {
+    auto pair = [&](const int pr, const bool do_f, const bool do_b, const LrRes *pre = nullptr) __attribute__((always_inline)) {
       const int mu = pr & 3;
       const int hop = pr >= 4 ? 3 : 1;
       const int pf = nbr_pos<HALO>(g, c, s, mu, hop);
@@ -94,8 +94,9 @@
         if (do_b) recon_row2<1>(W, (L.sm[2 * pr + 1] >> L.lane) & 1ull);
       } else if (RECON == 3) {
         const size_t fr = ((size_t)L.tile * NDIR + 2 * pr) * 576 + L.lane;
-        if (do_f) recon_row2_res(U, wp - L.lane, L.sm + 4 * pr, L.hdr, fr, L.lane);
-        if (do_b) recon_row2_res(W, wp - L.lane + LROW, L.sm + 4 * pr + 2, L.hdr, fr + 576, L.lane);
+        const LrRes rr = pre ? *pre : L.res_pair(pr);
+        if (do_f) recon_row2_res(U, rr.lo_f, (uint32_t)rr.hi, L.sm + 4 * pr, L.hdr, fr, L.lane);
+        if (do_b) recon_row2_res(W, rr.lo_b, (uint32_t)(rr.hi >> 32), L.sm + 4 * pr + 2, L.hdr, fr + 576, L.lane);
       } else if (RECON == 2) {
         if (do_f) recon_row2<2>(U, false);
         if (do_b) recon_row2<2>(W, false);
@@ -155,7 +156,15 @@
         for (int k = 0; k < 3; k++) acc[k] = make_double2(0.0, 0.0);
       }
       constexpr int UNR = (NDIR == 8) ? (RECON == 3 ? (FUSED ? 1 : 2) : (RECON ? 1 : 4)) : 2;
-      if (!edge) {
+      if (!edge && RECON == 3 && UNR == 2) {
+#pragma unroll 1
+        for (int gq = 0; gq < NDIR / 4; gq++) {
+          LrRes ra, rb;
+          L.res_group(gq, &ra, &rb);
+          pair(2 * gq, true, true, &ra);
+          pair(2 * gq + 1, true, true, &rb);
+        }
+      } else if (!edge) {
 #pragma unroll UNR
         for (int pr = 0; pr < NDIR / 2; pr++) pair(pr, true, true);
       } else if (!cleanup) {
@@ -396,7 +405,7 @@
     *W = c->Wc + rows * (c->recon == 1 ? LinkFormat<1>::LROW : LinkFormat<2>::LROW);
     *S = c->Ws + rows;
   } else if (lossless) {
-    *W = c->Wc + rows * LinkFormat<3>::LROW;
+    *W = c->Wc + rows * LinkFormat<3>::LDIR;
     *S = c->Wm + (size_t)parity * (2 + c->g.ntile * c->ndir * 2) + 2;
   } else {
     *W = c->W + rows * LinkFormat<0>::LROW;
diff --git a/qex_amd/csrc/dslash_core.h b/qex_amd/csrc/dslash_core.h
--- a/qex_amd/csrc/dslash_core.h
+++ b/qex_amd/csrc/dslash_core.h
@@ -47,10 +47,8 @@
   for (int k = 0; k < 3; k++) U[6 + k] = r2[k];
 }
 
-__device__ __forceinline__ void recon_row2_res(double2 U[9], const double2 *row, const unsigned long long *m, const unsigned long long *hdr,
-                                               size_t fr, int lane) {
-  const uint64_t lo = __builtin_nontemporal_load((const uint64_t *)(row + LR_RES) + lane);
-  const uint32_t hi = __builtin_nontemporal_load((const uint32_t *)(row + LR_RES + 32) + lane);
+__device__ __forceinline__ void recon_row2_res(double2 U[9], const uint64_t lo, const uint32_t hi, const unsigned long long *m,
+                                               const unsigned long long *hdr, size_t fr, int lane) {
   double2 r2[3];
   lr_decode(U, (m[0] >> lane) & 1ull, lo, hi, r2);
   if ((m[1] >> lane) & 1ull) {
@@ -64,20 +62,23 @@
 
 template <int RECON> struct LinkFormat {
   static constexpr int NLOAD = (RECON == 1 || RECON == 3) ? 6 : (RECON == 2 ? 7 : 9);
-  static constexpr int LROW = RECON == 3 ? LR_ROW : NLOAD * 64;
+  static constexpr int LROW = NLOAD * 64;
+  static constexpr int LDIR = RECON == 3 ? LR_ROW : LROW;
 };
 
 template <int NDIR, int RECON>
 struct LinkCursor {
-  static constexpr int NLOAD = LinkFormat<RECON>::NLOAD, LROW = LinkFormat<RECON>::LROW;
+  static constexpr int NLOAD = LinkFormat<RECON>::NLOAD, LROW = LinkFormat<RECON>::LROW, LDIR = LinkFormat<RECON>::LDIR;
   const double2 *w;
   const unsigned long long *sm;
   const unsigned long long *hdr;
   int tile, lane;
   __device__ __forceinline__ LinkCursor(const double2 *W, const unsigned long long *S, const int c)
-      : w(W + (size_t)(c >> 6) * (NDIR * LROW) + (c & 63)),
+      : w(W + (size_t)(c >> 6) * (NDIR * LDIR) + (c & 63)),
         sm(RECON == 1 ? S + (size_t)(c >> 6) * NDIR : (RECON == 3 ? S + (size_t)(c >> 6) * NDIR * 2 : nullptr)),
         hdr(RECON == 3 ? S - 2 : nullptr), tile(c >> 6), lane(c & 63) {}
+  __device__ __forceinline__ LrRes res_pair(const int pr) const { return lr_fetch_pair(w - lane, NDIR, pr, lane); }
+  __device__ __forceinline__ void res_group(const int g, LrRes *a, LrRes *b) const { lr_fetch_group(w - lane, NDIR, g, lane, a, b); }
   __device__ __forceinline__ void fetch(const int pr, const bool do_f, const bool do_b, double2 U[9], double2 Wb[9]) const {
     const double2 *wp = w + (size_t)pr * (2 * LROW);
     if (do_f) {
@@ -99,8 +100,9 @@
       if (do_b) recon_row2<1>(Wb, (sm[2 * pr + 1] >> lane) & 1ull);
     } else if (RECON == 3) {
       const size_t fr = ((size_t)tile * NDIR + 2 * pr) * 576 + lane;
-      if (do_f) recon_row2_res(U, wp - lane, sm + 4 * pr, hdr, fr, lane);
-      if (do_b) recon_row2_res(Wb, wp - lane + LROW, sm + 4 * pr + 2, hdr, fr + 576, lane);
+      const LrRes rr = res_pair(pr);
+      if (do_f) recon_row2_res(U, rr.lo_f, (uint32_t)rr.hi, sm + 4 * pr, hdr, fr, lane);
+      if (do_b) recon_row2_res(Wb, rr.lo_b, (uint32_t)(rr.hi >> 32), sm + 4 * pr + 2, hdr, fr + 576, lane);
     } else if (RECON == 2) {
       if (do_f) recon_row2<2>(U, false);
       if (do_b) recon_row2<2>(Wb, false);
diff --git a/qex_amd/csrc/layout.hip b/qex_amd/csrc/layout.hip
--- a/qex_amd/csrc/layout.hip
+++ b/qex_amd/csrc/layout.hip
@@ -213,7 +213,9 @@
   if (row >= nrows) return;
   const int l = j & 63;
   const double2 *w = W + row * 576 + l;
-  double2 *o = Wc + row * LR_ROW + l;
+  const int dir = (int)(row & 7);
+  double2 *blk = Wc + (row >> 3) * (8 * LR_ROW);
+  double2 *o = blk + lr_r01_off(dir) + l;
   double2 u[9];
 #pragma unroll
   for (int k = 0; k < 9; k++) u[k] = w[k * 64];
@@ -223,8 +225,7 @@
   uint64_t lo;
   uint32_t hi;
   const bool ok = lr_encode(u, &neg, &lo, &hi);
-  ((uint64_t *)(Wc + row * LR_ROW + LR_RES))[l] = lo;
-  ((uint32_t *)(Wc + row * LR_ROW + LR_RES + 32))[l] = hi;
+  lr_store_res(blk, 8, dir, l, lo, hi);
   const unsigned long long sgn = __ballot(neg), esc = __ballot(!ok);
   if (l == 0) {
     unsigned long long *m = Wm + 2 * (row + row / prows + 1);
@@ -243,6 +244,47 @@
     if (escaped) escaped[i] = !ok;
     if (row2) lr_decode(u + 9 * i, neg, lo, hi, row2 + 3 * i);
   }
+  return 0;
+}
+
+int link_residual_tile_host(const double2 *u, unsigned char *escaped, double2 *row2, short *res) {
+  std::vector<double2> blk((size_t)8 * LR_ROW, make_double2(0, 0));
+  unsigned long long m[8][2] = {};
+  for (int dir = 0; dir < 8; dir++)
+    for (int l = 0; l < 64; l++) {
+      const double2 *ul = u + 9 * (dir * 64 + l);
+      bool neg;
+      uint64_t lo;
+      uint32_t hi;
+      const bool ok = lr_encode(ul, &neg, &lo, &hi);
+      for (int k = 0; k < 6; k++) blk[lr_r01_off(dir) + k * 64 + l] = ul[k];
+      lr_store_res(blk.data(), 8, dir, l, lo, hi);
+      m[dir][0] |= (unsigned long long)neg << l;
+      m[dir][1] |= (unsigned long long)!ok << l;
+    }
+  for (int g = 0; g < 2; g++)
+    for (int l = 0; l < 64; l++) {
+      LrRes r[2];
+      lr_fetch_group(blk.data(), 8, g, l, &r[0], &r[1]);
+      for (int h = 0; h < 2; h++) {
+        const int pr = 2 * g + h;
+        const LrRes s = lr_fetch_pair(blk.data(), 8, pr, l);
+        if (s.lo_f != r[h].lo_f || s.lo_b != r[h].lo_b || s.hi != r[h].hi) { qexhip_set_error("link_residual_tile: the pair and group fetches disagree"); return -3; }
+        for (int fb = 0; fb < 2; fb++) {
+          const int dir = 2 * pr + fb, i = dir * 64 + l;
+          const uint64_t lo = fb ? s.lo_b : s.lo_f;
+          const uint32_t hi = (uint32_t)(fb ? s.hi >> 32 : s.hi);
+          double2 u01[6];
+          for (int k = 0; k < 6; k++) u01[k] = blk[lr_r01_off(dir) + k * 64 + l];
+          if (escaped) escaped[i] = (m[dir][1] >> l) & 1ull;
+          if (row2) lr_decode(u01, (m[dir][0] >> l) & 1ull, lo, hi, row2 + 3 * i);
+          if (res) {
+            for (int j = 0; j < 4; j++) res[6 * i + j] = (short)(lo >> (16 * j));
+            res[6 * i + 4] = (short)hi; res[6 * i + 5] = (short)(hi >> 16);
+          }
+        }
+      }
+    }
   return 0;
 }
 
diff --git a/qex_amd/csrc/link_residual.h b/qex_amd/csrc/link_residual.h
--- a/qex_amd/csrc/link_residual.h
+++ b/qex_amd/csrc/link_residual.h
@@ -4,7 +4,32 @@
 #include <cmath>
 
 #define LR_ROW 432
-#define LR_RES 384
+#define LR_R01 384
+#define LR_GRP 192
+
+typedef uint64_t lr_u2v __attribute__((ext_vector_type(2)));
+struct LrRes { uint64_t lo_f, lo_b, hi; };
+
+__host__ __device__ __forceinline__ size_t lr_r01_off(int dir) { return (size_t)dir * LR_R01; }
+__host__ __device__ __forceinline__ size_t lr_grp_off(int ndir, int g) { return (size_t)ndir * LR_R01 + (size_t)g * LR_GRP; }
+
+__host__ __device__ __forceinline__ void lr_store_res(double2 *blk, int ndir, int dir, int lane, uint64_t lo, uint32_t hi) {
+  double2 *q = blk + lr_grp_off(ndir, dir >> 2);
+  ((uint64_t *)(q + ((dir >> 1) & 1) * 64))[2 * lane + (dir & 1)] = lo;
+  ((uint32_t *)(q + 128))[4 * lane + (dir & 3)] = hi;
+}
+__host__ __device__ __forceinline__ LrRes lr_fetch_pair(const double2 *blk, int ndir, int pr, int lane) {
+  const double2 *q = blk + lr_grp_off(ndir, pr >> 1);
+  const lr_u2v lo = __builtin_nontemporal_load((const lr_u2v *)(q + (pr & 1) * 64) + lane);
+  const uint64_t hi = __builtin_nontemporal_load((const uint64_t *)(q + 128) + 2 * lane + (pr & 1));
+  return LrRes{lo.x, lo.y, hi};
+}
+__host__ __device__ __forceinline__ void lr_fetch_group(const double2 *blk, int ndir, int g, int lane, LrRes *a, LrRes *b) {
+  const lr_u2v *q = (const lr_u2v *)(blk + lr_grp_off(ndir, g)) + lane;
+  const lr_u2v q0 = __builtin_nontemporal_load(q), q1 = __builtin_nontemporal_load(q + 64), q2 = __builtin_nontemporal_load(q + 128);
+  *a = LrRes{q0.x, q0.y, q2.x};
+  *b = LrRes{q1.x, q1.y, q2.y};
+}
 
 __host__ __device__ __forceinline__ uint64_t lr_bits(double x) { return __builtin_bit_cast(uint64_t, x); }
 __host__ __device__ __forceinline__ double lr_double(uint64_t b) { return __builtin_bit_cast(double, b); }
diff --git a/qex_amd/csrc/qexhip_internal.h b/qex_amd/csrc/qexhip_internal.h
--- a/qex_amd/csrc/qexhip_internal.h
+++ b/qex_amd/csrc/qexhip_internal.h
@@ -51,6 +51,8 @@
   int itn, maxits, done, pad;
   double r2s[2];
   int itns[2], dones[2];
+  double alphas[2];
+  int xlag[2];
   double agree[4];
 };
 
@@ -107,6 +109,7 @@
   double2 *Wc = nullptr; unsigned long long *Ws = nullptr; size_t Wc_rows = 0; int recon = 0; double recon_dev = 0;
   unsigned long long *Wm = nullptr; size_t Wm_rows = 0; int lres = 0; long long lres_esc = 0;
   int opt_lossless = 1;
+  int opt_cg_defer_x = 1;
   int opt_batch_multi = 0;
   int opt_multi_reduce = 0;
   int opt_force_pair = 1;
@@ -176,6 +179,7 @@
 int links_from_natural(qexhip_ctx *c, const double2 *fat, const double2 *lng);
 int links_compress(qexhip_ctx *c);
 int link_residual_host(const double2 *u, long n, unsigned char *escaped, double2 *row2);
+int link_residual_tile_host(const double2 *u, unsigned char *escaped, double2 *row2, short *res);
 int op_eo_reconstruct_pub(qexhip_ctx *c, DevField &r, DevField &b, double m);
 int op_eo_reduce_pub(qexhip_ctx *c, DevField &r, DevField &b, double m);
 int op_stagD_pub(qexhip_ctx *c, DevField &r, DevField &x, int parity, double m, double sc, double a);
@@ -289,7 +293,8 @@
 int read_scalars(qexhip_ctx *c, const double *dev, int n, double *host);
 int blas_grid(const qexhip_ctx *c, int parity_count);
 int blas_delay(hipStream_t st, int us);
-int cg_xpay(qexhip_ctx *c, DevField &p, const DevField &r, int parity, int k, int rolled);
+int cg_xpay(qexhip_ctx *c, DevField &p, const DevField &r, DevField &x, int parity, int k, int rolled);
+int cg_flush_x(qexhip_ctx *c, DevField &x, const DevField &p, int parity, int k);
 int cg_update(qexhip_ctx *c, DevField &x, DevField &r, const DevField &p, const DevField &Ap, int parity, int k, int ndot);
 int cg_close(qexhip_ctx *c, int k);
 int cg_init(qexhip_ctx *c, double r2req, int maxits);
diff --git a/qex_amd/csrc/solver.cpp b/qex_amd/csrc/solver.cpp
--- a/qex_amd/csrc/solver.cpp
+++ b/qex_amd/csrc/solver.cpp
@@ -93,7 +93,7 @@
     int n = std::min(chunk, st.maxits - k);
     if (n <= 0) break;
     for (int i = 0; i < n; i++, k++) {
-      CHK(cg_xpay(c, *p, *r, par, k, rolled));
+      CHK(cg_xpay(c, *p, *r, x, par, k, rolled));
       rolled = 0;
       int ndot = 0;
       CHK(op_xx(c, *Ap, *p, m2, par_even, 1, &c->cg->dones[k & 1], &ndot));
@@ -107,6 +107,7 @@
     r2 = st.r2s[k & 1];
     st.itn = st.itns[k & 1];
   }
+  if (c->opt_cg_defer_x) CHK(cg_flush_x(c, x, *p, par, k));
   st.r2 = r2;
   if (iters) *iters = st.itn;
   if (r2_over_b2) *r2_over_b2 = (st.b2 != 0.0) ? st.r2 / st.b2 : 0.0;
diff --git a/qex_amd/staggered.py b/qex_amd/staggered.py
--- a/qex_amd/staggered.py
+++ b/qex_amd/staggered.py
@@ -523,6 +523,18 @@
     return esc.astype(bool), row2
 
 
+def link_residual_tile_host(links):
+    a = np.asarray(links)
+    if np.iscomplexobj(a):
+        a = np.stack([a.real, a.imag], axis=-1)
+    a = np.ascontiguousarray(a, dtype=np.float64).reshape(8, 64, 18)
+    esc = np.zeros((8, 64), dtype=np.uint8)
+    row2 = np.zeros((8, 64, 3, 2), dtype=np.float64)
+    res = np.zeros((8, 64, 6), dtype=np.int16)
+    check(lib().qexhip_link_residual_tile_host(a.ctypes.data, esc.ctypes.data, row2.ctypes.data, res.ctypes.data))
+    return esc.astype(bool), row2, res
+
+
 def plaq(ctx, g=None):
     if g is not None:
         check(lib().qexhip_gauge_set(ctx._h, _p(g)))
```
